# zju3dv/SMAP

Measured on AMD Instinct MI355X. Metric: frames/sec at 3x512x832 (SMAP backbone + depth-aware association + 3D lifting), higher is better.
Workload: dtype f16x3; 1 GPU; batch=8 x 3x512x832 per GPU, full SMAP + depth-aware PAF association + lifting (BASELINE configs[2]; configs[3] when n_gpus=8); records_in_run=4392, resident_batches_in_rotation=4, frames_per_launch=16, ranks_in_gather=1, full=False

## Files before the change

smap_amd/csrc/assoc.hip:

```cpp
#include <hip/hip_runtime.h>
#include <stdint.h>
#include <type_traits>
#include "smap_hip.h"
#include "hip_rc.h"
#include "prep_device.h"

namespace {

constexpr int NJ = SMAP_NJ, NL = SMAP_NL, MAXP = SMAP_MAXP, PSTRIDE = MAXP + 1;

__constant__ int c_pairs[2 * NL] = {0, 1, 0, 2, 0, 9, 9, 10, 10, 11, 0, 3, 3, 4,
                                    4, 5, 2, 12, 12, 13, 13, 14, 2, 6, 6, 7, 7, 8};
__constant__ float c_bone_length[NL] = {
    26.42178982f, 48.36980909f, 14.88291009f, 31.28002332f, 23.915707f,
    14.97674918f, 31.28002549f, 23.91570732f, 12.4644364f,  48.26604433f,
    39.03553194f, 12.4644364f,  48.19076948f, 39.03553252f};

__global__ void scale_hms_kernel(float* __restrict__ hms, int HW4, int total4)
{
    for (int i = blockIdx.x * blockDim.x + threadIdx.x; i < total4; i += gridDim.x * blockDim.x) {
        const int c = (i / HW4) % SMAP_HMS_C;
        const float d = c < NJ ? 255.f : 127.f;
        float4 v = reinterpret_cast<float4*>(hms)[i];
        v.x = v.x / d; v.y = v.y / d; v.z = v.z / d; v.w = v.w / d;
// ... 811 lines not shown
                       root_idx, dist_flag, bodys, counts);
    return hip_rc(hipGetLastError());
}

int smap_lift(const float* bodys, const int32_t* counts, const float* det_d, const float* root_d,
              const double* cams, int B, int H, int W, float* pred_2d, double* pred_3d, double* root_z,
              void* stream)
{
    if (!bodys || !counts || !det_d || !root_d || !cams || !pred_2d || !pred_3d || !root_z || B <= 0)
        return SMAP_E_ARG;
    hipLaunchKernelGGL(lift_kernel<false>, dim3(B), dim3(128), 0, (hipStream_t)stream, bodys, counts, det_d, root_d,
                       cams, H, W, pred_2d, pred_3d, root_z);
    return hip_rc(hipGetLastError());
}

int smap_lift_gt(const float* bodys, const int32_t* counts, const float* det_d, const float* root_d,
                 const double* cams, int B, int H, int W, double* pred_2d, double* pred_3d, double* root_z,
                 void* stream)
{
    if (!bodys || !counts || !det_d || !root_d || !cams || !pred_2d || !pred_3d || !root_z || B <= 0)
        return SMAP_E_ARG;
    hipLaunchKernelGGL(lift_kernel<true>, dim3(B), dim3(128), 0, (hipStream_t)stream, bodys, counts, det_d, root_d,
                       cams, H, W, pred_2d, pred_3d, root_z);
    return hip_rc(hipGetLastError());
}

int smap_lift_gt_bones(const float* bodys, const int32_t* counts, const float* det_d, const float* root_d,
                       const double* cams, int B, int H, int W, double* pred_2d, double* pred_3d, double* root_z,
                       double* depth_v, int32_t* bone_mask, void* stream)
{
    if (!bodys || !counts || !det_d || !root_d || !cams || !pred_2d || !pred_3d || !root_z || !depth_v || !bone_mask || B <= 0)
        return SMAP_E_ARG;
    hipLaunchKernelGGL((lift_kernel<true, true>), dim3(B), dim3(128), 0, (hipStream_t)stream, bodys, counts, det_d, root_d,
                       cams, H, W, pred_2d, pred_3d, root_z, depth_v, bone_mask);
    return hip_rc(hipGetLastError());
}

int smap_register_gt(const float* bodys, const int32_t* counts, const float* gt_roots, const int32_t* gt_counts,
                     int B, int G, float* matched, int32_t* matched_counts, void* stream)
{
    if (!bodys || !counts || !gt_roots || !gt_counts || !matched || !matched_counts || B <= 0 || G <= 0 ||
        G > REG_MAXG)
        return SMAP_E_ARG;
    hipLaunchKernelGGL(register_gt_kernel, dim3(B), dim3(64), 0, (hipStream_t)stream, bodys, counts, gt_roots,
                       gt_counts, G, matched, matched_counts);
    return hip_rc(hipGetLastError());
}

int smap_refine(const float* pred_2d, const double* pred_3d, const int32_t* counts, int B,
                const float* const* wt, const float* const* bs, double* refined, void* stream)
{
    if (!pred_2d || !pred_3d || !counts || !wt || !bs || !refined || B <= 0) return SMAP_E_ARG;
    RefineW w;
    for (int l = 0; l < 5; ++l) {
        if (!wt[l] || !bs[l]) return SMAP_E_ARG;
        w.wt[l] = wt[l];
        w.bs[l] = bs[l];
    }
    hipLaunchKernelGGL(refine_kernel<float>, dim3(MAXP, B), dim3(256), 0, (hipStream_t)stream, pred_2d, pred_3d,
                       counts, w, refined);
    return hip_rc(hipGetLastError());
}

int smap_refine_gt(const double* pred_2d, const double* pred_3d, const int32_t* counts, int B,
                   const float* const* wt, const float* const* bs, double* refined, void* stream)
{
    if (!pred_2d || !pred_3d || !counts || !wt || !bs || !refined || B <= 0) return SMAP_E_ARG;
    RefineW w;
    for (int l = 0; l < 5; ++l) {
        if (!wt[l] || !bs[l]) return SMAP_E_ARG;
        w.wt[l] = wt[l];
        w.bs[l] = bs[l];
    }
    hipLaunchKernelGGL(refine_kernel<double>, dim3(MAXP, B), dim3(256), 0, (hipStream_t)stream, pred_2d, pred_3d,
                       counts, w, refined);
    return hip_rc(hipGetLastError());
}

}

extern "C" int smap_refine_mlp(const float* x, int N, const float* const* wt, const float* const* bs, float* y,
                               void* stream)
{
    if (!wt || !bs || N < 0) return SMAP_E_ARG;
    if (N == 0) return 0;
    if (!x || !y) return SMAP_E_ARG;
    RefineW w;
    for (int l = 0; l < 5; ++l) {
        if (!wt[l] || !bs[l]) return SMAP_E_ARG;
        w.wt[l] = wt[l];
        w.bs[l] = bs[l];
    }
    hipLaunchKernelGGL(refine_mlp_kernel, dim3(N), dim3(256), 0, (hipStream_t)stream, x, w, y);
    return hip_rc(hipGetLastError());
}

extern "C" int smap_flip_merge(float* hms, const float* hms_flip, const int* pair43, int B, int H, int W, void* stream)
{
    if (!hms || !hms_flip || !pair43 || B <= 0 || H <= 0 || W <= 0) return SMAP_E_ARG;
    FlipTab tab;
    for (int c = 0; c < SMAP_HMS_C; ++c) {
        if (pair43[c] < 0 || pair43[c] >= SMAP_HMS_C) return SMAP_E_ARG;
        tab.pair[c] = pair43[c];
    }
    const long long total = (long long)B * SMAP_HMS_C * H * W;
    const int grid = (int)((total + 255) / 256 < 4096 ? (total + 255) / 256 : 4096);
    hipLaunchKernelGGL(flip_merge_kernel, dim3(grid), dim3(256), 0, (hipStream_t)stream, hms, hms_flip, tab, W, H * W,
                       total);
    return hip_rc(hipGetLastError());
}

extern "C" int smap_preprocess(const unsigned char* src, int h, int w, int nh, int nw, int top, int left, float* dst,
                               int net_h, int net_w, const float* mean3, const float* std3, double fx, double fy, void* stream)
{
    if (!src || !dst || !mean3 || !std3 || h <= 0 || w <= 0 || nh <= 0 || nw <= 0 || net_h <= 0 || net_w <= 0 || !(fx > 0) || !(fy > 0))
        return SMAP_E_ARG;
    const PrepFrame f{src, {h, w, nh, nw, top, left, 1.0 / fx, 1.0 / fy}};
    const PrepCanvas cv{net_h, net_w, {mean3[0], mean3[1], mean3[2]}, {std3[0], std3[1], std3[2]}};
    hipLaunchKernelGGL(preprocess_kernel, dim3((net_w + 255) / 256, net_h), dim3(256), 0, (hipStream_t)stream, f, dst, cv);
    return hip_rc(hipGetLastError());
}

extern "C" int smap_sizeof_prep_frame(void) { return (int)sizeof(smap_prep_frame); }

extern "C" int smap_preprocess_batch(const smap_prep_frame* frames, int B, float* dst, int net_h, int net_w, const float* mean3,
                                     const float* std3, void* stream)
{
    if (!frames || !dst || !mean3 || !std3 || B <= 0 || net_h <= 0 || net_w <= 0) return SMAP_E_ARG;
    for (int b = 0; b < B; ++b) {
        const smap_prep_frame& s = frames[b];
        if (!s.src || s.h <= 0 || s.w <= 0 || s.nh <= 0 || s.nw <= 0 || !(s.fx > 0) || !(s.fy > 0)) return SMAP_E_ARG;
    }
    const PrepCanvas cv{net_h, net_w, {mean3[0], mean3[1], mean3[2]}, {std3[0], std3[1], std3[2]}};
    const bool vec = net_w % 4 == 0 && ((uintptr_t)dst & 15) == 0;
    const int px = vec ? 4 : 1;
    const size_t frame_floats = (size_t)3 * net_h * net_w;
    for (int b0 = 0; b0 < B; b0 += SMAP_PREP_MAX_FRAMES) {
        const int n = B - b0 < SMAP_PREP_MAX_FRAMES ? B - b0 : SMAP_PREP_MAX_FRAMES;
        PrepTable t;
        for (int i = 0; i < SMAP_PREP_MAX_FRAMES; ++i) {
            const smap_prep_frame& s = frames[b0 + (i < n ? i : n - 1)];
            t.f[i] = PrepFrame{s.src, {s.h, s.w, s.nh, s.nw, s.top, s.left, 1.0 / s.fx, 1.0 / s.fy}};
        }
        const dim3 grid((net_w + 256 * px - 1) / (256 * px), net_h, n);
        float* out = dst + (size_t)b0 * frame_floats;
        if (vec) hipLaunchKernelGGL(preprocess_batch_kernel<4>, grid, dim3(256), 0, (hipStream_t)stream, t, out, cv);
        else hipLaunchKernelGGL(preprocess_batch_kernel<1>, grid, dim3(256), 0, (hipStream_t)stream, t, out, cv);
        const int rc = hip_rc(hipGetLastError());
        if (rc) return rc;
    }
    return 0;
}

extern "C" const char* smap_version(void) { return "smap_hip gfx950 r6 (assoc + backbone f16|x3 + flip-TTA + persistent conv + whole-Bottleneck launches + plan blob v2 + windowed arena + N segments + split K + lanes + two-input launches + tap-dot head + scaled head sum + two-launch peak search)"; }
```

smap_amd/csrc/conv.hip:

```cpp
#include <hip/hip_runtime.h>
#include <stdint.h>
#include "smap_hip.h"
#include "plan.h"
#include "conv_device.h"

namespace {

#ifndef SMAP_ABLATE
#define SMAP_ABLATE 0
#endif
template <int BM, int BN, int WM, int WN, int STAGES, int BK, bool FULL, bool X3, bool SPLITK = false, bool REGEPI = false, bool DUAL = false, bool TAPDOT = false,
          bool RELUSUM = false>
__global__ __launch_bounds__(WM * WN * 64) void conv_igemm_kernel(const ConvArgs a)
{
    static_assert(!TAPDOT || (!FULL && !SPLITK && !REGEPI && !DUAL), "tap-dot epilogue: plain instance only");
    static_assert(!RELUSUM || DUAL, "relu-sum: a second input");
    static_assert(!REGEPI || (X3 && !FULL && !SPLITK), "register epilogue: split precision, plain epilogue, no split K");
    static_assert(!DUAL || (!FULL && !SPLITK && !REGEPI), "second input: plain epilogue, no split K");
    constexpr int NPL = X3 ? 2 : 1;
    constexpr int NW = WM * WN, NT = NW * 64;
    static_assert(NW == 4 || NW == 8, "4 or 8 waves");
    static_assert(STAGES >= 2 && STAGES <= 4, "2..4 LDS stages");
    static_assert(BK == 32 || BK == 64, "BK = halves per K chunk");
    constexpr int ROWB = BK * 2;
    constexpr int SPR = ROWB / 16;
    constexpr int RPW = 64 / SPR;
    constexpr int RPR = NW * RPW;
    static_assert(BM % RPR == 0 && BN % RPR == 0, "tile must be a multiple of the DMA round");
    constexpr int LA = BM / RPR, LB = BN / RPR;
    constexpr int MI = BM / WM / 32, NI = BN / WN / 32;
    static_assert(MI >= 1 && NI >= 1, "tile too small for the wave grid");
    constexpr int STAGE = NPL * (BM + BN) * ROWB;
    constexpr int LPT = NPL * (LA + LB);
    static_assert((STAGES - 2) * LPT <= 63, "vmcnt is 6 bits");
    constexpr int CSS = TAPDOT ? BN + 8 : BN;
    constexpr int LDS_BYTES = REGEPI ? STAGES * STAGE : (STAGES * STAGE > BM * CSS * 4 ? STAGES * STAGE : BM * CSS * 4) + (SPLITK ? 16 : 0);
    static_assert(LDS_BYTES <= 160 * 1024, "LDS is 160 KiB per CU");
    __shared__ __attribute__((aligned(16))) char smem[LDS_BYTES];

    SMAP_TL_BEGIN
    const int tid = threadIdx.x, lane = tid & 63;
    const int wave = __builtin_amdgcn_readfirstlane(tid >> 6);
#ifdef SMAP_TRACE
    long long tr_t[8]; long long tr_wait = 0;
    tr_t[0] = __builtin_amdgcn_s_memtime();
#define TR(i) tr_t[i] = __builtin_amdgcn_s_memtime()
#else
#define TR(i)
#endif

    const int logical = xcd_logical_block();
    const int S = SPLITK ? a.ksplit : 1;
    const int tile_id = S > 1 ? logical / S : logical, ks = logical - tile_id * S;
    const int m_tile = tile_id / a.n_tiles, n_tile = tile_id - m_tile * a.n_tiles;
    const int m0 = m_tile * BM, n0 = n_tile * BN;
    const int seg = (n0 >= a.seg_n1 ? 1 : 0) + (n0 >= a.seg_n2 ? 1 : 0);
    const int nb = n0 - (seg == 0 ? 0 : seg == 1 ? a.seg_n1 : a.seg_n2);
    void* const o_out = seg == 0 ? a.out : seg == 1 ? a.seg_out1 : a.seg_out2;
    const int o_cout8 = seg == 0 ? a.Cout8 : seg == 1 ? a.seg_cout8_1 : a.seg_cout8_2;
    const int o_stride = seg == 0 ? a.out_stride_c : seg == 1 ? a.seg_stride1 : a.seg_stride2;
    const int o_c_off = seg == 0 ? a.out_c_off : 0;
    const int o_relu = seg == 0 ? a.relu : seg == 1 ? a.seg_relu1 : a.seg_relu2;
    const float o_scale = seg == 0 ? a.acc_scale : seg == 1 ? a.seg_scale1 : a.seg_scale2;
    const int o_lo = o_stride >> 1;
    const _Float16* const o_res = seg == 0 ? a.res : nullptr;
    const _Float16* const o_up = seg == 0 ? a.up : nullptr;
    const _Float16* const o_add1 = seg == 0 ? a.add1 : nullptr;
    const _Float16* const o_add2 = seg == 0 ? a.add2 : nullptr;

    const int lrow = lane / SPR, lslot = lane % SPR;
    const int srow = wave * RPW + lrow;
    const int gch = BK == 64 ? (lslot ^ ((srow >> 1) & 7)) : (lslot ^ ((srow >> 2) & 3));
    const char* __restrict__ arena = reinterpret_cast<const char*>(a.arena);
    const char* __restrict__ wt = reinterpret_cast<const char*>(a.w);
    const int HoWo = a.Ho * a.Wo;

    const bool wpair = BK == 32 && a.w_pairs;
    const int wrow = wpair ? 128 : ROWB;
    const int wblk = NPL * BN * wrow;
    unsigned w_off[NPL * LB];
#pragma unroll
    for (int j = 0; j < NPL * LB; ++j) w_off[j] = (unsigned)((j * RPR + wave * RPW + lrow) * wrow + lslot * 16);
    const char* __restrict__ wt_tile = wt + (long long)n_tile * (wpair ? a.K / 64 : a.K / BK) * wblk;
    auto issue_b = [&](int buf, int it) {
        char* sB = smem + buf * STAGE + NPL * BM * ROWB;
        const char* gB = wpair ? wt_tile + (long long)(it >> 1) * wblk + (it & 1) * 64 : wt_tile + (long long)it * wblk;
#pragma unroll
        for (int j = 0; j < NPL * LB; ++j)
            lds_dma16(gB + w_off[j], sB + (j * RPR + wave * RPW) * ROWB);
    };
    if (!(SMAP_ABLATE & 1) && !SPLITK) issue_b(0, 0);

    unsigned a_off[LA];
    unsigned a_mask[LA];
    {
        int m = m0 + srow;
        int b = m / HoWo, rem = m - b * HoWo;
        int oy = rem / a.Wo, ox = rem - oy * a.Wo;
#pragma unroll
        for (int i = 0; i < LA; ++i) {
            a_off[i] = 0;
            a_mask[i] = 0;
            if (m < a.M) {
                const int iy0 = oy * a.stride - a.pad, ix0 = ox * a.stride - a.pad;
                const long long e = ((long long)(b * a.H + iy0) * a.W + ix0) * a.in_stride_c + a.in_c_off + gch * 8;
                a_off[i] = (unsigned)(a.in_off + e * 2);
                unsigned vx = 0, mk = 0;
#pragma unroll
                for (int kw = 0; kw < 3; ++kw)
                    if (kw < a.ksize && (unsigned)(ix0 + kw) < (unsigned)a.W) vx |= 1u << kw;
#pragma unroll
                for (int kh = 0; kh < 3; ++kh)
                    if (kh < a.ksize && (unsigned)(iy0 + kh) < (unsigned)a.H) mk |= vx << (kh * a.ksize);
                a_mask[i] = mk;
            }
            m += RPR;
            ox += RPR;
            while (ox >= a.Wo) { ox -= a.Wo; ++oy; }
            while (oy >= a.Ho) { oy -= a.Ho; ++b; }
        }
    }
    unsigned a_off2[DUAL ? LA : 1];
    if (DUAL) {
        int m = m0 + srow;
        int b = m / HoWo, rem = m - b * HoWo;
        int oy = rem / a.Wo, ox = rem - oy * a.Wo;
#pragma unroll
        for (int i = 0; i < LA; ++i) {
            a_off2[i] = 0;
            if (m < a.M) {
                const long long e = ((long long)(b * a.H2 + oy * a.stride2) * a.W2 + ox * a.stride2) * a.in2_stride_c + gch * 8;
                a_off2[i] = (unsigned)(a.in2_off + e * 2);
            }
            m += RPR;
            ox += RPR;
            while (ox >= a.Wo) { ox -= a.Wo; ++oy; }
            while (oy >= a.Ho) { oy -= a.Ho; ++b; }
        }
    }
    const int cchunks = a.Cin / BK;
    const int cchunks2 = DUAL ? a.Cin2 / BK : 0;
    const int n_all = a.ksize * a.ksize * cchunks + cchunks2;
    const int it_lo = S > 1 ? ks * n_all / S : 0;
    const int n_iter = (S > 1 ? (ks + 1) * n_all / S : n_all) - it_lo;

    int s_kh = 0, s_kw = 0, s_cc = 0;
    int s_in2 = 0;
    int s_it = it_lo;
    if (S > 1) {
        const int tap = it_lo / cchunks;
        s_cc = it_lo - tap * cchunks;
        s_kh = tap / a.ksize;
        s_kw = tap - s_kh * a.ksize;
    }
    unsigned a_cur[LA];
    auto set_tap = [&]() {
        const unsigned tap_off = (unsigned)((s_kh * a.W + s_kw) * a.in_stride_c * 2);
        const unsigned bit = 1u << (s_kh * a.ksize + s_kw);
#pragma unroll
        for (int i = 0; i < LA; ++i) a_cur[i] = (a_mask[i] & bit) ? a_off[i] + tap_off : 0u;
    };
    set_tap();
    auto issue_a = [&](int buf) {
#pragma unroll
        for (int pl = 0; pl < NPL; ++pl) {
            char* sA = smem + buf * STAGE + pl * BM * ROWB;
            const char* gA = arena + (unsigned)(s_cc * ROWB + (X3 ? pl * ((DUAL && s_in2) ? a.in2_lo : a.in_lo) * 2 : 0));
#pragma unroll
            for (int i = 0; i < LA; ++i)
                lds_dma16(gA + a_cur[i], sA + (i * RPR + wave * RPW) * ROWB);
        }
    };
    auto advance = [&]() {
        ++s_it;
        if (DUAL && s_in2) { ++s_cc; return; }
        if (++s_cc == cchunks) {
            s_cc = 0;
            if (DUAL) {
                s_in2 = 1;
#pragma unroll
                for (int i = 0; i < LA; ++i) a_cur[i] = a_off2[i];
                return;
            }
            if (++s_kw == a.ksize) { s_kw = 0; ++s_kh; }
            set_tap();
        }
    };
    auto stage = [&](int buf) {
        issue_a(buf);
        issue_b(buf, s_it);
        advance();
    };
    if (!(SMAP_ABLATE & 1)) {
        if (SPLITK) issue_b(0, it_lo);
        issue_a(0);
        advance();
    }

    constexpr int CG = BN / 8;
    constexpr int PASSES = REGEPI ? 1 : BM * CG / NT;
    static_assert(BM * CG % NT == 0, "tile/thread mismatch");
    half8 rres[PASSES][NPL];
    auto load_res = [&]() {
#pragma unroll
        for (int p = 0; p < PASSES; ++p) {
            const int idx = p * NT + tid;
            const int row = idx / CG, cg = idx - row * CG;
            const int m = m0 + row, n = nb + cg * 8;
            const unsigned dense = (m < a.M && n < o_cout8) ? (unsigned)m * (unsigned)(NPL * o_cout8) + (unsigned)n : 0u;
#pragma unroll
            for (int pl = 0; pl < NPL; ++pl)
                rres[p][pl] = *reinterpret_cast<const half8*>(o_res + dense + pl * o_cout8);
        }
    };
    if (o_res && !SPLITK && !REGEPI) load_res();

    f32x16 acc[MI][NI];
#pragma unroll
    for (int mi = 0; mi < MI; ++mi)
#pragma unroll
        for (int ni = 0; ni < NI; ++ni)
#pragma unroll
            for (int r = 0; r < 16; ++r) acc[mi][ni][r] = 0.f;

    const int wm = wave / WN, wn = wave - wm * WN;
    const int l31 = lane & 31, lhi = lane >> 5;
    if (REGEPI) {
        const float inv = 1.f / o_scale;
#pragma unroll
        for (int ni = 0; ni < NI; ++ni)
#pragma unroll
            for (int q = 0; q < 4; ++q) {
                const float4 b4 = *reinterpret_cast<const float4*>(a.bias + n0 + wn * (BN / WN) + ni * 32 + 8 * q + 4 * lhi);
#pragma unroll
                for (int mi = 0; mi < MI; ++mi) {
                    acc[mi][ni][4 * q + 0] = b4.x * inv; acc[mi][ni][4 * q + 1] = b4.y * inv;
                    acc[mi][ni][4 * q + 2] = b4.z * inv; acc[mi][ni][4 * q + 3] = b4.w * inv;
                }
            }
    }
    const int rswz = BK == 64 ? ((l31 >> 1) & 7) : ((l31 >> 2) & 3);
    const int a_row0 = wm * (BM / WM) + l31;
    const int b_row0 = wn * (BN / WN) + l31;
    f32x16 park[RELUSUM ? MI : 1][RELUSUM ? NI : 1];
    float bias1[RELUSUM ? NI : 1];
    if (RELUSUM) {
#pragma unroll
        for (int ni = 0; ni < NI; ++ni) bias1[ni] = a.bias[n0 + wn * (BN / WN) + ni * 32 + l31];
    }

    TR(1);
#pragma unroll
    for (int st = 1; st < STAGES - 1; ++st)
        if (st < n_iter && !(SMAP_ABLATE & 1)) stage(st);
    int buf = 0, nbuf = STAGES - 1;
    for (int it = 0; it < n_iter; ++it) {
#ifdef SMAP_TRACE
        const long long tw0 = __builtin_amdgcn_s_memtime();
#endif
        if (it + STAGES - 1 <= n_iter) asm volatile("s_waitcnt vmcnt(%0)" ::"n"((STAGES - 2) * LPT) : "memory");
        else asm volatile("s_waitcnt vmcnt(0)" ::: "memory");
        __builtin_amdgcn_s_barrier();
        asm volatile("" ::: "memory");
#ifdef SMAP_TRACE
        tr_wait += __builtin_amdgcn_s_memtime() - tw0;
        if (it == 0) tr_t[2] = __builtin_amdgcn_s_memtime();
#endif
        if (it + STAGES - 1 < n_iter && !(SMAP_ABLATE & 1)) stage(nbuf);
        if (RELUSUM && it == cchunks) {
#pragma unroll
            for (int mi = 0; mi < MI; ++mi)
#pragma unroll
                for (int ni = 0; ni < NI; ++ni)
#pragma unroll
                    for (int r = 0; r < 16; ++r) {
                        const float v = X3 ? acc[mi][ni][r] * o_scale + bias1[ni] : acc[mi][ni][r] + bias1[ni];
                        park[mi][ni][r] = v < 0.f ? 0.f : v;
                        acc[mi][ni][r] = 0.f;
                    }
        }
        const char* sA = smem + buf * STAGE;
        const char* sB = sA + NPL * BM * ROWB;
#pragma unroll
        for (int kk = 0; kk < ((SMAP_ABLATE & 2) ? 0 : BK / 16); ++kk) {
            const int slot = ((kk * 2 + lhi) ^ rswz) * 16;
            half8 af[NPL][MI], bf[NPL][NI];
#pragma unroll
            for (int pl = 0; pl < NPL; ++pl) {
#pragma unroll
                for (int mi = 0; mi < MI; ++mi)
                    af[pl][mi] = *reinterpret_cast<const half8*>(sA + (pl * BM + a_row0 + mi * 32) * ROWB + slot);
#pragma unroll
                for (int ni = 0; ni < NI; ++ni)
                    bf[pl][ni] = *reinterpret_cast<const half8*>(sB + (pl * BN + b_row0 + ni * 32) * ROWB + slot);
            }
#pragma unroll
            for (int mi = 0; mi < MI; ++mi)
#pragma unroll
                for (int ni = 0; ni < NI; ++ni) {
                    if (REGEPI) {
                        acc[mi][ni] = __builtin_amdgcn_mfma_f32_32x32x16_f16(bf[0][ni], af[NPL - 1][mi], acc[mi][ni], 0, 0, 0);
                        acc[mi][ni] = __builtin_amdgcn_mfma_f32_32x32x16_f16(bf[NPL - 1][ni], af[0][mi], acc[mi][ni], 0, 0, 0);
                        acc[mi][ni] = __builtin_amdgcn_mfma_f32_32x32x16_f16(bf[0][ni], af[0][mi], acc[mi][ni], 0, 0, 0);
                        continue;
                    }
                    if (X3) {
                        acc[mi][ni] = __builtin_amdgcn_mfma_f32_32x32x16_f16(af[NPL - 1][mi], bf[0][ni], acc[mi][ni], 0, 0, 0);
                        acc[mi][ni] = __builtin_amdgcn_mfma_f32_32x32x16_f16(af[0][mi], bf[NPL - 1][ni], acc[mi][ni], 0, 0, 0);
                    }
                    acc[mi][ni] = __builtin_amdgcn_mfma_f32_32x32x16_f16(af[0][mi], bf[0][ni], acc[mi][ni], 0, 0, 0);
                }
        }
        buf = buf + 1 == STAGES ? 0 : buf + 1;
        nbuf = nbuf + 1 == STAGES ? 0 : nbuf + 1;
    }
    TR(3);
    __syncthreads();
    if (SMAP_ABLATE & 8) {
        if (acc[0][0][0] == 12345.678f) reinterpret_cast<float*>(a.out)[tid] = acc[0][0][1];
        return;
    }

    if constexpr (REGEPI) {
        _Float16* const outp = reinterpret_cast<_Float16*>(o_out);
        unsigned m_dense[MI], m_out[MI];
        bool m_ok[MI];
#pragma unroll
        for (int mi = 0; mi < MI; ++mi) {
            const int m = m0 + wm * (BM / WM) + mi * 32 + l31;
            m_ok[mi] = m < a.M;
            const unsigned ms = m_ok[mi] ? (unsigned)m : 0u;
            m_dense[mi] = ms * (unsigned)(NPL * o_cout8);
            m_out[mi] = ms * (unsigned)o_stride + (unsigned)o_c_off;
        }
        auto n_of = [&](int ni) { return nb + wn * (BN / WN) + ni * 32 + 8 * lhi; };
        auto load_rr = [&](int mi, int ni, half8 (&rr)[2][NPL]) {
#pragma unroll
            for (int j = 0; j < 2; ++j) {
                const int n = n_of(ni) + 16 * j;
                const unsigned d = n < o_cout8 ? m_dense[mi] + (unsigned)n : 0u;
#pragma unroll
                for (int pl = 0; pl < NPL; ++pl) rr[j][pl] = *reinterpret_cast<const half8*>(o_res + d + pl * o_cout8);
            }
        };
        half8 rr[2][2][NPL];
        if (o_res) load_rr(0, 0, rr[0]);
#pragma unroll
        for (int mi = 0; mi < MI; ++mi)
#pragma unroll
            for (int ni = 0; ni < NI; ++ni) {
                constexpr int NB = MI * NI;
                const int blk = mi * NI + ni;
                if (o_res && blk + 1 < NB) load_rr((blk + 1) / NI, (blk + 1) % NI, rr[(blk + 1) & 1]);
                f32x16& c = acc[mi][ni];
#pragma unroll
                for (int j = 0; j < 2; ++j)
#pragma unroll
                    for (int e = 0; e < 4; ++e) {
                        const float2 sw = halfwave_swap(c[8 * j + e], c[8 * j + 4 + e]);
                        c[8 * j + e] = o_scale * sw.x;
                        c[8 * j + 4 + e] = o_scale * sw.y;
                    }
                if (o_res) {
#pragma unroll
                    for (int j = 0; j < 2; ++j)
#pragma unroll
                        for (int e = 0; e < 8; ++e) c[8 * j + e] += (float)rr[blk & 1][j][0][e] + (float)rr[blk & 1][j][NPL - 1][e];
                }
                if (o_relu) relu16(c);
#pragma unroll
                for (int j = 0; j < 2; ++j) {
                    const int n = n_of(ni) + 16 * j;
                    if (!m_ok[mi] || n >= o_cout8 || ((SMAP_ABLATE & 4) && a.M != 7)) continue;
                    _Float16* op = outp + (m_out[mi] + (unsigned)n);
                    half8 h, l;
#pragma unroll
                    for (int e = 0; e < 8; ++e) {
                        h[e] = (_Float16)c[8 * j + e];
                        l[e] = (_Float16)(c[8 * j + e] - (float)h[e]);
                    }
                    *reinterpret_cast<half8*>(op) = h;
                    *reinterpret_cast<half8*>(op + o_lo) = l;
                }
            }
        SMAP_TL_END(a)
        return;
    }

    float* Cs = reinterpret_cast<float*>(smem);
#pragma unroll
    for (int ni = 0; ni < NI; ++ni) {
        const int col = wn * (BN / WN) + ni * 32 + l31;
        const float bias = RELUSUM ? a.bias_b[n0 + col] : a.bias[n0 + col];
#pragma unroll
        for (int mi = 0; mi < MI; ++mi)
#pragma unroll
            for (int r = 0; r < 16; ++r) {
                const int row = wm * (BM / WM) + mi * 32 + (r & 3) + 8 * (r >> 2) + 4 * lhi;
                if (RELUSUM) {
                    const float v = X3 ? acc[mi][ni][r] * a.acc_scale_b + bias : acc[mi][ni][r] + bias;
                    Cs[row * CSS + col] = (v < 0.f ? 0.f : v) + park[mi][ni][r];
                    continue;
                }
                Cs[row * CSS + col] = S > 1 ? acc[mi][ni][r] : (X3 ? acc[mi][ni][r] * o_scale + bias : acc[mi][ni][r] + bias);
            }
    }
    __syncthreads();
    if (SPLITK && S == 1 && o_res) load_res();
    if (SPLITK && S > 1) {
#ifndef SMAP_SPLITK_ACQREL
#define SMAP_SPLITK_ACQREL 1
#endif
#if !SMAP_SPLITK_ACQREL && !defined(__gfx942__) && !defined(__gfx950__) && defined(__HIP_DEVICE_COMPILE__)
#error "split K: the fence-free partial-tile hand-off is verified for gfx942 / gfx950 only; build with -DSMAP_SPLITK_ACQREL=1 elsewhere"
#endif
        float* part = a.kpart + (size_t)tile_id * S * (BM * BN);
        for (int i = tid; i < BM * BN; i += NT) __hip_atomic_store(part + (size_t)ks * (BM * BN) + i, Cs[i], __ATOMIC_RELAXED, __HIP_MEMORY_SCOPE_AGENT);
        asm volatile("s_waitcnt vmcnt(0)" ::: "memory");
        __syncthreads();
        volatile int* s_last = reinterpret_cast<volatile int*>(smem + LDS_BYTES - 16);
        if (tid == 0) {
#if SMAP_SPLITK_ACQREL
            const unsigned t = __hip_atomic_fetch_add(a.kcount + tile_id, 1u, __ATOMIC_RELEASE, __HIP_MEMORY_SCOPE_AGENT);
            if (t == (unsigned)(S - 1)) __builtin_amdgcn_fence(__ATOMIC_ACQUIRE, "agent");
#else
            const unsigned t = atomicAdd(a.kcount + tile_id, 1u);
#endif
            *s_last = t == (unsigned)(S - 1);
            if (t == (unsigned)(S - 1)) atomicExch(a.kcount + tile_id, 0u);
        }
        __syncthreads();
        if (!*s_last) return;
        if (o_res) load_res();
        for (int i = tid; i < BM * BN; i += NT) {
            float v = __hip_atomic_load(part + i, __ATOMIC_RELAXED, __HIP_MEMORY_SCOPE_AGENT);
            for (int q = 1; q < S; ++q) v += __hip_atomic_load(part + (size_t)q * (BM * BN) + i, __ATOMIC_RELAXED, __HIP_MEMORY_SCOPE_AGENT);
            const float bias = a.bias[n0 + i % BN];
            Cs[i] = X3 ? v * o_scale + bias : v + bias;
        }
        __syncthreads();
    }

    if constexpr (TAPDOT) {
        static_assert(BM == 128 && BN == 256 && NW == 8, "one 16-row MFMA tile per wave");
                const int prow = wave * 16 + (lane & 15), kq = lane >> 4;
        const half8* __restrict__ wfrag = reinterpret_cast<const half8*>(a.tap_w) + lane;
        f32x4 d = {0.f, 0.f, 0.f, 0.f};
#pragma unroll
        for (int ks = 0; ks < BN / 32; ++ks) {
            const half8 wh = wfrag[(ks * 2 + 0) * 64], wl = wfrag[(ks * 2 + 1) * 64];
            const float4 y0 = *reinterpret_cast<const float4*>(Cs + prow * CSS + ks * 32 + kq * 8);
            const float4 y1 = *reinterpret_cast<const float4*>(Cs + prow * CSS + ks * 32 + kq * 8 + 4);
            float y[8] = {y0.x, y0.y, y0.z, y0.w, y1.x, y1.y, y1.z, y1.w};
            half8 yh, yl;
#pragma unroll
            for (int e = 0; e < 8; ++e) {
                float v = y[e];
                if (o_relu) v = v < 0.f ? 0.f : v;
                yh[e] = (_Float16)v;
                yl[e] = (_Float16)(v - (float)yh[e]);
            }
            d = __builtin_amdgcn_mfma_f32_16x16x32_f16(yl, wh, d, 0, 0, 0);
            d = __builtin_amdgcn_mfma_f32_16x16x32_f16(yh, wl, d, 0, 0, 0);
            d = __builtin_amdgcn_mfma_f32_16x16x32_f16(yh, wh, d, 0, 0, 0);
        }
        float* const tout = reinterpret_cast<float*>(o_out);
#pragma unroll
        for (int i = 0; i < 4; ++i) {
            const int m = m0 + wave * 16 + kq * 4 + i;
            if (m < a.M) tout[(size_t)m * 16 + (lane & 15)] = d[i] * a.tap_scale;
        }
        SMAP_TL_END(a)
        return;
    }

    struct Extra { half8 t00[NPL], t01[NPL], t10[NPL], t11[NPL], a1[NPL], a2[NPL]; float ly0, ly1, lx0, lx1; bool ok; unsigned o; int row, cg; };
    constexpr int TS = NPL;
    auto val = [](const half8 (&h)[NPL], int e) -> float {
        return X3 ? (float)h[0][e] + (float)h[NPL - 1][e] : (float)h[0][e];
    };
    auto load_pass = [&](int p) -> Extra {
        Extra x;
        const int idx = p * NT + tid;
        x.row = idx / CG;
        x.cg = idx - x.row * CG;
        const int m = m0 + x.row, n = nb + x.cg * 8;
        x.ok = m < a.M && n < o_cout8 && !((SMAP_ABLATE & 4) && a.M != 7);
        const int ms = x.ok ? m : 0, ns = x.ok ? n : 0;
        const unsigned dense = (unsigned)ms * (unsigned)(TS * o_cout8) + (unsigned)ns;
        x.o = (unsigned)ms * (unsigned)o_stride + (unsigned)(o_c_off + ns);
        if (FULL && o_up) {
            const int b = (SMAP_ABLATE & 64) ? 0 : ms / HoWo, rem = ms - b * HoWo;
            const int oy = (SMAP_ABLATE & 64) ? (ms & 63) : rem / a.Wo, ox = (SMAP_ABLATE & 64) ? (ms & 127) : rem - oy * a.Wo;
            Lerp ly = lerp_index(oy, a.up_h, a.Ho), lx = lerp_index(ox, a.up_w, a.Wo);
            if (SMAP_ABLATE & 64) { ly.i0 = oy >> 1; ly.i1 = ly.i0; ly.l0 = 0.5f; ly.l1 = 0.5f; lx.i0 = ox >> 1; lx.i1 = lx.i0; lx.l0 = 0.5f; lx.l1 = 0.5f; }
            const int us = TS * o_cout8;
            const unsigned tb0 = (unsigned)b * (unsigned)(a.up_h * a.up_w) * (unsigned)us + (unsigned)ns;
            const _Float16* __restrict__ tb = o_up;
#pragma unroll
            for (int pl = 0; pl < ((SMAP_ABLATE & 32) ? 0 : NPL); ++pl) {
                x.t00[pl] = *reinterpret_cast<const half8*>(tb + (tb0 + (unsigned)(ly.i0 * a.up_w + lx.i0) * (unsigned)us + (unsigned)(pl * o_cout8)));
                x.t01[pl] = *reinterpret_cast<const half8*>(tb + (tb0 + (unsigned)(ly.i0 * a.up_w + lx.i1) * (unsigned)us + (unsigned)(pl * o_cout8)));
                x.t10[pl] = *reinterpret_cast<const half8*>(tb + (tb0 + (unsigned)(ly.i1 * a.up_w + lx.i0) * (unsigned)us + (unsigned)(pl * o_cout8)));
                x.t11[pl] = *reinterpret_cast<const half8*>(tb + (tb0 + (unsigned)(ly.i1 * a.up_w + lx.i1) * (unsigned)us + (unsigned)(pl * o_cout8)));
            }
            x.ly0 = ly.l0; x.ly1 = ly.l1; x.lx0 = lx.l0; x.lx1 = lx.l1;
        }
#pragma unroll
        for (int pl = 0; pl < NPL; ++pl) {
            if (FULL && o_add1) x.a1[pl] = *reinterpret_cast<const half8*>(o_add1 + dense + pl * o_cout8);
            if (FULL && o_add2) x.a2[pl] = *reinterpret_cast<const half8*>(o_add2 + dense + pl * o_cout8);
        }
        return x;
    };
    auto finish_pass = [&](int p, const Extra& x) {
        float v[8];
        {
            const float4 lo = *reinterpret_cast<const float4*>(Cs + x.row * BN + x.cg * 8);
            const float4 hi = *reinterpret_cast<const float4*>(Cs + x.row * BN + x.cg * 8 + 4);
            v[0] = lo.x; v[1] = lo.y; v[2] = lo.z; v[3] = lo.w;
            v[4] = hi.x; v[5] = hi.y; v[6] = hi.z; v[7] = hi.w;
        }
        if (o_res) {
#pragma unroll
            for (int e = 0; e < 8; ++e) v[e] += val(rres[p], e);
        }
        if (FULL && o_up) {
#pragma unroll
            for (int e = 0; e < 8; ++e)
                v[e] += x.ly0 * (x.lx0 * val(x.t00, e) + x.lx1 * val(x.t01, e)) +
                        x.ly1 * (x.lx0 * val(x.t10, e) + x.lx1 * val(x.t11, e));
        }
        if (o_relu) {
#pragma unroll
            for (int e = 0; e < 8; ++e) v[e] = v[e] < 0.f ? 0.f : v[e];
        }
        if (FULL && o_add1) {
#pragma unroll
            for (int e = 0; e < 8; ++e) v[e] += val(x.a1, e);
        }
        if (FULL && o_add2) {
#pragma unroll
            for (int e = 0; e < 8; ++e) v[e] += val(x.a2, e);
        }
        if (!x.ok) return;
        if (a.out_fp32) {
            float* op = reinterpret_cast<float*>(o_out) + x.o;
            *reinterpret_cast<float4*>(op) = make_float4(v[0], v[1], v[2], v[3]);
            *reinterpret_cast<float4*>(op + 4) = make_float4(v[4], v[5], v[6], v[7]);
        } else {
            half8 h;
#pragma unroll
            for (int e = 0; e < 8; ++e) h[e] = (_Float16)v[e];
            *reinterpret_cast<half8*>(reinterpret_cast<_Float16*>(o_out) + x.o) = h;
            if (X3) {
                half8 l;
#pragma unroll
                for (int e = 0; e < 8; ++e) l[e] = (_Float16)(v[e] - (float)h[e]);
                *reinterpret_cast<half8*>(reinterpret_cast<_Float16*>(o_out) + x.o + o_lo) = l;
            }
        }
    };
    TR(4);
#ifndef SMAP_EPI_DEPTH
#define SMAP_EPI_DEPTH 1
#endif
    constexpr int ED = (FULL && PASSES > 2) ? SMAP_EPI_DEPTH : 1;
    Extra ex[ED + 1];
#pragma unroll
    for (int p = 0; p < ED && p < PASSES; ++p) ex[p] = load_pass(p);
#pragma unroll
    for (int p = 0; p < PASSES; ++p) {
        if (p + ED < PASSES) ex[(p + ED) % (ED + 1)] = load_pass(p + ED);
        finish_pass(p, ex[p % (ED + 1)]);
    }
#ifdef SMAP_TRACE
    asm volatile("s_waitcnt vmcnt(0)" ::: "memory");
    TR(5);
    if (a.dbg && tid == 0) {
        long long* d = a.dbg + (long long)blockIdx.x * 8;
        unsigned hwid;
        asm volatile("s_getreg_b32 %0, hwreg(HW_REG_HW_ID)" : "=s"(hwid));
        d[0] = tr_t[0]; d[1] = tr_t[1]; d[2] = tr_t[2]; d[3] = tr_t[3]; d[4] = tr_t[4]; d[5] = tr_t[5]; d[6] = tr_wait; d[7] = hwid;
    }
#endif
    SMAP_TL_END(a)
}

#define SMAP_IGEMM_ROW(cap)                                                                                      \
    constexpr TileRow t = tile_row(TILE);                                                                        \
    static_assert(t.family == TF_IGEMM && tile_has(t, X3, cap),                                                  \
                  "csrc/tiles.h: the row of this tile id does not list this instance");                          \
    constexpr int BM = t.bm, BN = t.bn, BK = tile_bk(t, X3)

template <int TILE, bool X3, int WM, int WN, int STAGES>
hipError_t launch_splitk(const ConvArgs& a, hipStream_t st)
{
    SMAP_IGEMM_ROW(TC_SPLITK);
    const dim3 grid(a.m_tiles * a.n_tiles * a.ksplit);
    if (a.up || a.add1 || a.add2)
        hipLaunchKernelGGL((conv_igemm_kernel<BM, BN, WM, WN, STAGES, BK, true, X3, true>), grid, dim3(WM * WN * 64), 0, st, a);
    else
        hipLaunchKernelGGL((conv_igemm_kernel<BM, BN, WM, WN, STAGES, BK, false, X3, true>), grid, dim3(WM * WN * 64), 0, st, a);
    return hipGetLastError();
}

template <int TILE, bool X3, int WM, int WN, int STAGES>
hipError_t launch(const ConvArgs& a, hipStream_t st)
{
    SMAP_IGEMM_ROW(0);
    static_assert(!(t.caps & TC_REGEPI), "register-epilogue tiles go through launch_regepi");
    if (a.up || a.add1 || a.add2)
        hipLaunchKernelGGL((conv_igemm_kernel<BM, BN, WM, WN, STAGES, BK, true, X3>), dim3(a.m_tiles * a.n_tiles), dim3(WM * WN * 64), 0, st, a);
    else
        hipLaunchKernelGGL((conv_igemm_kernel<BM, BN, WM, WN, STAGES, BK, false, X3>), dim3(a.m_tiles * a.n_tiles), dim3(WM * WN * 64), 0, st, a);
    return hipGetLastError();
}

template <int TILE, bool X3, int WM, int WN, int STAGES>
hipError_t launch_regepi(const ConvArgs& a, hipStream_t st)
{
    SMAP_IGEMM_ROW(TC_REGEPI);
    if (a.up || a.add1 || a.add2 || a.out_fp32 || a.ksplit > 1) return hipErrorInvalidValue;
    hipLaunchKernelGGL((conv_igemm_kernel<BM, BN, WM, WN, STAGES, BK, false, X3, false, true>), dim3(a.m_tiles * a.n_tiles), dim3(WM * WN * 64), 0, st, a);
    return hipGetLastError();
}

template <int TILE, bool X3, int WM, int WN, int STAGES>
hipError_t launch_dual(const ConvArgs& a, hipStream_t st)
{
    SMAP_IGEMM_ROW(TC_DUAL);
    if (a.up || a.add1 || a.add2 || a.ksplit > 1 || a.ksize != 1) return hipErrorInvalidValue;
    hipLaunchKernelGGL((conv_igemm_kernel<BM, BN, WM, WN, STAGES, BK, false, X3, false, false, true>), dim3(a.m_tiles * a.n_tiles), dim3(WM * WN * 64), 0, st, a);
    return hipGetLastError();
}

template <int TILE, bool X3, int WM, int WN, int STAGES>
hipError_t launch_relusum(const ConvArgs& a, hipStream_t st)
{
    SMAP_IGEMM_ROW(TC_DUAL | TC_RELUSUM);
    if (a.up || a.add1 || a.add2 || a.res || a.ksplit > 1 || a.ksize != 1 || a.relu || !a.bias_b) return hipErrorInvalidValue;
    hipLaunchKernelGGL((conv_igemm_kernel<BM, BN, WM, WN, STAGES, BK, false, X3, false, false, true, false, true>), dim3(a.m_tiles * a.n_tiles), dim3(WM * WN * 64), 0, st, a);
    return hipGetLastError();
}

template <int TILE, bool X3, int WM, int WN, int STAGES>
hipError_t launch_tapdot(const ConvArgs& a, hipStream_t st)
{
    SMAP_IGEMM_ROW(TC_TAPDOT);
    if (a.up || a.add1 || a.add2 || a.res || a.ksplit > 1 || a.Cin2 > 0 || a.n_tiles != 1 || a.tap_n != 9 || !a.tap_w) return hipErrorInvalidValue;
    hipLaunchKernelGGL((conv_igemm_kernel<BM, BN, WM, WN, STAGES, BK, false, X3, false, false, false, true>), dim3(a.m_tiles), dim3(WM * WN * 64), 0, st, a);
    return hipGetLastError();
}
#undef SMAP_IGEMM_ROW

#define SMAP_BOTH(HELPER, TILE, ...) (a.x3 ? HELPER<TILE, true, __VA_ARGS__>(a, st) : HELPER<TILE, false, __VA_ARGS__>(a, st))

}

hipError_t smap_launch_conv(const ConvArgs& a, int tile, hipStream_t st)
{
    const TileRow* t = tile_find(tile);
    if (!t || !tile_has(*t, a.x3)) return hipErrorInvalidValue;
    switch (t->family) {
        case TF_HALO: return smap_launch_conv3(a, tile, st);
        case TF_PERSIST: return smap_launch_convp(a, tile, st);
        case TF_TAIL: return smap_launch_convf(a, tile, st);
        case TF_BLOCK: return smap_launch_convb(a, tile, st);
        case TF_IGEMM: break;
    }
    if (a.tap_n > 0) {
        switch (tile) {
            case 54: return SMAP_BOTH(launch_tapdot, 54, 2, 4, 2);
            default: return hipErrorInvalidValue;
        }
    }
    if (a.Cin2 > 0 && a.bias_b) {
        switch (tile) {
            case 50: return SMAP_BOTH(launch_relusum, 50, 2, 4, 2);
            case 51: return SMAP_BOTH(launch_relusum, 51, 4, 2, 2);
            case 53: return SMAP_BOTH(launch_relusum, 53, 4, 2, 2);
            case 54: return SMAP_BOTH(launch_relusum, 54, 2, 4, 2);
            default: return hipErrorInvalidValue;
        }
    }
    if (a.Cin2 > 0) {
        switch (tile) {
            case 20: return SMAP_BOTH(launch_dual, 20, 2, 2, 2);
            case 50: return SMAP_BOTH(launch_dual, 50, 2, 4, 2);
            case 51: return SMAP_BOTH(launch_dual, 51, 4, 2, 2);
            case 53: return SMAP_BOTH(launch_dual, 53, 4, 2, 2);
            case 54: return SMAP_BOTH(launch_dual, 54, 2, 4, 2);
            default: return hipErrorInvalidValue;
        }
    }
    if (a.ksplit > 1) {
        switch (tile) {
            case 2: return SMAP_BOTH(launch_splitk, 2, 2, 2, 2);
            case 22: return SMAP_BOTH(launch_splitk, 22, 2, 2, 2);
            case 7: return SMAP_BOTH(launch_splitk, 7, 2, 2, 4);
            case 20: return SMAP_BOTH(launch_splitk, 20, 2, 2, 2);
            default: return hipErrorInvalidValue;
        }
    }
    if (a.x3) {
        switch (tile) {
            case 0: return launch<0, true, 2, 2, 2>(a, st);
            case 1: return launch<1, true, 2, 2, 2>(a, st);
            case 2: return launch<2, true, 2, 2, 2>(a, st);
            case 4: return launch<4, true, 2, 2, 2>(a, st);
            case 3: return launch<3, true, 4, 1, 2>(a, st);
            case 20: return launch<20, true, 2, 2, 2>(a, st);
            case 21: return launch<21, true, 2, 2, 2>(a, st);
            case 22: return launch<22, true, 2, 2, 2>(a, st);
            case 23: return launch<23, true, 2, 2, 2>(a, st);
            case 24: return launch<24, true, 2, 2, 3>(a, st);
            case 25: return launch<25, true, 2, 2, 3>(a, st);
            case 26: return launch<26, true, 2, 2, 4>(a, st);
            case 7: return launch<7, true, 2, 2, 4>(a, st);
            case 27: return launch<27, true, 2, 2, 3>(a, st);
            case 50: return launch<50, true, 2, 4, 2>(a, st);
            case 51: return launch<51, true, 4, 2, 2>(a, st);
            case 52: return launch<52, true, 2, 4, 2>(a, st);
            case 53: return launch<53, true, 4, 2, 2>(a, st);
            case 54: return launch<54, true, 2, 4, 2>(a, st);
            case 55: return launch<55, true, 2, 4, 4>(a, st);
            case 56: return launch_regepi<56, true, 2, 4, 2>(a, st);
            default: return hipErrorInvalidValue;
        }
    }
    switch (tile) {
        case 20: return launch<20, false, 2, 2, 2>(a, st);
        case 21: return launch<21, false, 2, 2, 2>(a, st);
        case 22: return launch<22, false, 2, 2, 2>(a, st);
        case 23: return launch<23, false, 2, 2, 2>(a, st);
        case 24: return launch<24, false, 2, 2, 4>(a, st);
        case 25: return launch<25, false, 2, 2, 3>(a, st);
        case 26: return launch<26, false, 2, 2, 4>(a, st);
        case 27: return launch<27, false, 2, 2, 3>(a, st);
        case 0: return launch<0, false, 2, 2, 2>(a, st);
        case 1: return launch<1, false, 2, 2, 2>(a, st);
        case 2: return launch<2, false, 2, 2, 2>(a, st);
        case 3: return launch<3, false, 4, 1, 2>(a, st);
        case 4: return launch<4, false, 2, 2, 2>(a, st);
        case 5: return launch<5, false, 2, 2, 4>(a, st);
        case 6: return launch<6, false, 2, 2, 3>(a, st);
        case 7: return launch<7, false, 2, 2, 4>(a, st);
        case 8: return launch<8, false, 4, 1, 3>(a, st);
        case 9: return launch<9, false, 2, 2, 3>(a, st);
        case 50: return launch<50, false, 2, 4, 2>(a, st);
        case 51: return launch<51, false, 4, 2, 2>(a, st);
        case 52: return launch<52, false, 2, 4, 2>(a, st);
        case 53: return launch<53, false, 4, 2, 2>(a, st);
        case 54: return launch<54, false, 2, 4, 2>(a, st);
        case 55: return launch<55, false, 2, 4, 4>(a, st);
        default: return hipErrorInvalidValue;
    }
}
```

smap_amd/csrc/plan.h:

```cpp
#pragma once
#include <hip/hip_runtime.h>
#include <stdint.h>
#include "tiles.h"

struct ConvArgs {
    const void* arena;
    long long in_off;
    const _Float16* w;
    const float* bias;
    void* out;
    const _Float16* res;
    const _Float16* add1;
    const _Float16* add2;
    const _Float16* up;
    int up_h, up_w;
    int H, W, Cin, in_stride_c, in_c_off;
    int Ho, Wo, Cout8;
    int ksize, stride, pad, relu;
    int out_stride_c, out_c_off, out_fp32;
    int M, K, m_tiles, n_tiles;
    int x3;
    int in_lo;
    int out_lo;
    long long w_lo;
    float acc_scale;
    int w_pairs;
    const _Float16* w2;
    const float* bias2;
    int tail_cout8;
    int tail_chunks;
    float tail_acc_scale;
    const _Float16* w0;
    const float* bias0;
    int head_cin;
    float acc_scale0;
    const _Float16* wd;
    float acc_scale_d;
    int ksplit;
    float* kpart;
    unsigned* kcount;
    long long in2_off;
    int H2, W2, Cin2, in2_stride_c, stride2, in2_lo;
    const float* bias_b;
    float acc_scale_b;
    const _Float16* tap_w;
    int tap_n;
    float tap_scale;
    int seg_n1, seg_n2;
    void* seg_out1; void* seg_out2;
    int seg_cout8_1, seg_cout8_2, seg_stride1, seg_stride2, seg_relu1, seg_relu2;
    float seg_scale1, seg_scale2;
#ifdef SMAP_TRACE
    long long* dbg;
#endif
#ifdef SMAP_TIMELINE
    long long* tl;
    long long tl_meta[4];
#endif
};

struct Lerp { int i0, i1; float l0, l1; };
__device__ __forceinline__ Lerp lerp_index(int dst, int in_size, int out_size)
{
    Lerp r;
    if (in_size == out_size) { r.i0 = dst; r.i1 = dst; r.l0 = 1.f; r.l1 = 0.f; return r; }
    const float scale = out_size > 1 ? (float)(in_size - 1) / (float)(out_size - 1) : 0.f;
    const float src = scale * (float)dst;
    r.i0 = (int)src;
    r.i1 = r.i0 + (r.i0 < in_size - 1 ? 1 : 0);
    float l1 = src - (float)r.i0;
    l1 = l1 < 0.f ? 0.f : (l1 > 1.f ? 1.f : l1);
    r.l1 = l1;
    r.l0 = 1.f - l1;
    return r;
}

hipError_t smap_launch_conv(const ConvArgs& a, int tile, hipStream_t st);
hipError_t smap_launch_conv3(const ConvArgs& a, int tile, hipStream_t st);
hipError_t smap_launch_convp(const ConvArgs& a, int tile, hipStream_t st);
hipError_t smap_launch_convf(const ConvArgs& a, int tile, hipStream_t st);
hipError_t smap_launch_convb(const ConvArgs& a, int tile, hipStream_t st);
hipError_t smap_launch_convc(const ConvArgs& a, hipStream_t st);

#ifdef SMAP_TIMELINE
#define SMAP_TL_BEGIN const long long tl_t0 = __builtin_amdgcn_s_memrealtime();
#define SMAP_TL_END(a)                                                                                        \
    if ((a).tl && threadIdx.x == 0) {                                                                         \
        unsigned hw_, xcc_;                                                                                   \
        asm volatile("s_getreg_b32 %0, hwreg(HW_REG_HW_ID)" : "=s"(hw_));                                     \
        asm volatile("s_getreg_b32 %0, hwreg(HW_REG_XCC_ID)" : "=s"(xcc_));                                   \
        long long* d_ = (a).tl + 4 * (1 + (long long)blockIdx.x);                                             \
        d_[0] = tl_t0; d_[1] = __builtin_amdgcn_s_memrealtime(); d_[2] = hw_; d_[3] = xcc_;                   \
        if (blockIdx.x == 0) { (a).tl[0] = (a).tl_meta[0]; (a).tl[1] = (a).tl_meta[1]; (a).tl[2] = (a).tl_meta[2]; (a).tl[3] = (a).tl_meta[3]; } \
    }
#else
#define SMAP_TL_BEGIN
#define SMAP_TL_END(a)
#endif
```

smap_amd/csrc/plan.hip:

```cpp
#include <hip/hip_runtime.h>
#include <stdint.h>
#include <new>
#include <memory>
#include <cstdlib>
#include <cstring>
#include <climits>
#include <vector>
#include <type_traits>
#include "smap_hip.h"
#include "plan.h"
#include "plan_check.h"
#include "conv_device.h"
#include "hip_rc.h"

namespace {

#ifndef SMAP_STEM_STORE16
#define SMAP_STEM_STORE16 1
#endif
constexpr int ST_T = 16, ST_PH = ST_T * 2 + 5, ST_PW = 40;
constexpr int ST_K = SMAP_STEM_K;

struct StemIn {
    const float* p[SMAP_MAX_INPUTS];
// ... 428 lines not shown
    }
    __syncthreads();
    for (int idx = tid; idx < C * HS_PX; idx += 256) {
        const int c = idx / HS_PX, px = idx - c * HS_PX;
        const int x = x0 + px;
        if (x >= Wo) continue;
        float v = tile[c * (HS_PX + 1) + px];
        if (FLIP) {
            const float f = tile2[pair[c] * (HS_PX + 1) + px];
            const bool neg = c >= n_kpt && ((c - n_kpt) & 1) == 0;
            v = v + (neg ? f * -1.f : f);
            if (c >= n_kpt) v = v * 0.5f;
        }
        if (scale) v = v / (c < n_kpt ? 255.f : 127.f);
        out[(((size_t)b * C + c) * Ho + y) * Wo + x] = v;
        if (status && !(fabsf(v) <= 3.4028234e38f)) {
            atomicOr(reinterpret_cast<unsigned*>(status) + b / 31, 1u | (2u << (b % 31)));
            if (b >= 31) atomicOr(reinterpret_cast<unsigned*>(status), 1u);
        }
    }
}

__global__ __launch_bounds__(256) void tapsum_kernel(const float* __restrict__ t, const float* __restrict__ bias, float* __restrict__ out,
                                                     int B, int H, int W, int ts, int* __restrict__ status)
{
    const long long total = (long long)B * H * W;
    const long long i = (long long)blockIdx.x * 256 + threadIdx.x;
    if (i >= total) return;
    const int x = (int)(i % W), y = (int)((i / W) % H), b = (int)(i / ((long long)W * H));
    float v = bias[0];
#pragma unroll
    for (int kh = 0; kh < 3; ++kh)
#pragma unroll
        for (int kw = 0; kw < 3; ++kw) {
            const int yy = y + kh - 1, xx = x + kw - 1;
            if ((unsigned)yy < (unsigned)H && (unsigned)xx < (unsigned)W) v += t[(((size_t)b * H + yy) * W + xx) * ts + kh * 3 + kw];
        }
    out[i] = v;
    if (status && !(fabsf(v) <= 3.4028234e38f)) {
        atomicOr(reinterpret_cast<unsigned*>(status) + b / 31, 1u | (2u << (b % 31)));
        if (b >= 31) atomicOr(reinterpret_cast<unsigned*>(status), 1u);
    }
}

inline int grid_for(long long total, int block)
{
    long long g = (total + block - 1) / block;
    return (int)(g < 1 ? 1 : (g > 8192 ? 8192 : g));
}

}

struct smap_plan : PlanCheck {
    bool lanes_on = false, lanes_ready = false;
    hipStream_t side[SMAP_MAX_LANES] = {};
    std::vector<hipEvent_t> ev;
    hipEvent_t join_ev[SMAP_MAX_LANES] = {};
};

#ifdef SMAP_TIMELINE
constexpr long long TL_SLICE = 4LL * (1 + 16384);
static int tl_next = 0;
static long long* tl_base() { const char* e = getenv("SMAP_TIMELINE_PTR"); return e ? reinterpret_cast<long long*>(strtoull(e, nullptr, 0)) : nullptr; }
static int tl_cap() { const char* e = getenv("SMAP_TIMELINE_CAP"); return e ? atoi(e) : 0; }
extern "C" __attribute__((visibility("default"))) void smap_timeline_reset(void) { tl_next = 0; }
extern "C" __attribute__((visibility("default"))) int smap_timeline_count(void) { return tl_next; }
#endif

extern "C" {

int smap_plan_create(const smap_op* ops, int n_ops, smap_plan** plan)
{
    std::unique_ptr<smap_plan> p(new (std::nothrow) smap_plan());
    if (!plan || !p) return SMAP_E_ARG;
    if (int rc = plan_check(ops, n_ops, p.get())) return rc;
    *plan = p.release();
    return 0;
}

int smap_plan_create_from_blob(const void* blob, size_t blob_bytes, smap_plan** plan, smap_blob_info* info)
{
    std::unique_ptr<smap_plan> p(new (std::nothrow) smap_plan());
    if (!plan || !p) return SMAP_E_ARG;
    if (int rc = plan_check_blob(blob, blob_bytes, p.get(), info)) return rc;
    *plan = p.release();
    return 0;
}

static void lanes_release(smap_plan* p)
{
    for (hipEvent_t& e : p->ev) if (e) { (void)hipEventDestroy(e); e = nullptr; }
    for (int l = 0; l < SMAP_MAX_LANES; ++l) {
        if (p->join_ev[l]) { (void)hipEventDestroy(p->join_ev[l]); p->join_ev[l] = nullptr; }
        if (p->side[l]) { (void)hipStreamDestroy(p->side[l]); p->side[l] = nullptr; }
    }
    p->lanes_ready = false;
}

void smap_plan_destroy(smap_plan* plan)
{
    if (!plan) return;
    lanes_release(plan);
    delete plan;
}

static int lanes_setup(smap_plan* p)
{
    if (p->lanes_ready) return 0;
    hipError_t e = hipSuccess;
    for (int l = 1; l < p->n_lanes && e == hipSuccess; ++l) e = hipStreamCreateWithFlags(&p->side[l], hipStreamNonBlocking);
    for (int l = 0; l < p->n_lanes && e == hipSuccess; ++l) e = hipEventCreateWithFlags(&p->join_ev[l], hipEventDisableTiming);
    p->ev.assign(p->ops.size(), nullptr);
    for (size_t i = 0; i < p->ops.size() && e == hipSuccess; ++i)
        if (p->signalled[i]) e = hipEventCreateWithFlags(&p->ev[i], hipEventDisableTiming);
    if (e != hipSuccess) { lanes_release(p); return hip_rc(e); }
    p->lanes_ready = true;
    return 0;
}

int smap_plan_set_lanes(smap_plan* plan, int on)
{
    if (!plan) return SMAP_E_ARG;
    if (on && plan->n_lanes > 1)
        if (int rc = lanes_setup(plan)) return rc;
    plan->lanes_on = on != 0;
    return 0;
}

static ConvArgs conv_args(const smap_op& o, char* ar, const char* wb)
{
    auto A = [&](int64_t off) -> _Float16* { return off < 0 ? nullptr : reinterpret_cast<_Float16*>(ar + off); };
    const TileRow& t = *tile_find(o.tile);
    ConvArgs a;
    a.arena = ar + window_of(o.in_off);
    a.in_off = o.in_off - window_of(o.in_off);
    a.w = reinterpret_cast<const _Float16*>(wb + o.w_off);
    a.bias = reinterpret_cast<const float*>(wb + o.bias_off);
    a.out = ar + o.out_off;
    a.res = A(o.res_off);
    a.add1 = A(o.add1_off);
    a.add2 = A(o.add2_off);
    a.up = A(o.aux_off[0]);
    a.up_h = o.aux_h[0];
    a.up_w = o.aux_w[0];
    a.H = o.H; a.W = o.W; a.Cin = o.Cin; a.in_stride_c = o.in_stride_c; a.in_c_off = o.in_c_off;
    a.Ho = o.Ho; a.Wo = o.Wo; a.Cout8 = (o.Cout + 7) & ~7;
    a.ksize = o.ksize; a.stride = o.stride; a.pad = o.pad; a.relu = o.relu;
    a.out_stride_c = o.out_stride_c; a.out_c_off = o.out_c_off; a.out_fp32 = o.out_fp32;
    a.M = o.B * o.Ho * o.Wo;
    a.K = o.ksize * o.ksize * o.Cin + (o.in2_C > 0 ? o.in2_C : 0);
    a.Cin2 = o.in2_C > 0 ? o.in2_C : 0;
    a.in2_off = o.in2_C > 0 ? o.in2_off - window_of(o.in_off) : 0;
    a.H2 = o.in2_H; a.W2 = o.in2_W; a.in2_stride_c = o.in2_stride_c; a.stride2 = o.in2_stride; a.in2_lo = o.in2_stride_c / 2;
    a.bias_b = (o.in2_C > 0 && o.in2_mode == 1) ? reinterpret_cast<const float*>(wb + o.in2_bias_off) : nullptr;
    a.acc_scale_b = o.in2_acc_scale;
    a.x3 = o.precision;
    a.in_lo = o.in_stride_c / 2;
    a.out_lo = o.out_stride_c / 2;
    a.w_lo = (long long)o.cout_pad * a.K * 2;
    a.acc_scale = o.acc_scale;
    a.w_pairs = o.w_pairs;
    a.w2 = o.tail_cout > 0 ? reinterpret_cast<const _Float16*>(wb + o.tail_w_off) : nullptr;
    a.bias2 = o.tail_cout > 0 ? reinterpret_cast<const float*>(wb + o.tail_bias_off) : nullptr;
    a.tail_cout8 = o.tail_cout;
    a.tail_chunks = o.tail_cout > 0 ? o.tail_cout_pad / t.tail_bn : 0;
    a.tail_acc_scale = o.tail_acc_scale;
    a.w0 = o.head_cin > 0 ? reinterpret_cast<const _Float16*>(wb + o.head_w_off) : nullptr;
    a.bias0 = o.head_cin > 0 ? reinterpret_cast<const float*>(wb + o.head_bias_off) : nullptr;
    a.head_cin = o.head_cin;
    a.acc_scale0 = o.head_acc_scale;
    a.wd = o.head_cin > 0 && o.short_acc_scale > 0.f ? reinterpret_cast<const _Float16*>(wb + o.short_w_off) : nullptr;
    a.acc_scale_d = o.short_acc_scale;
    a.tap_n = o.tap_n;
    a.tap_w = o.tap_n > 0 ? reinterpret_cast<const _Float16*>(wb + o.tap_w_off) : nullptr;
    a.tap_scale = o.tap_scale;
    a.ksplit = o.ksplit > 1 ? o.ksplit : 1;
    a.kpart = o.ksplit > 1 ? reinterpret_cast<float*>(ar + o.kpart_off) : nullptr;
    a.kcount = o.ksplit > 1 ? reinterpret_cast<unsigned*>(ar + o.kcount_off) : nullptr;
    a.seg_n1 = o.seg_n[0] > 0 ? o.seg_n[0] : INT32_MAX;
    a.seg_n2 = o.seg_n[1] > 0 ? o.seg_n[1] : INT32_MAX;
    a.seg_out1 = o.seg_n[0] > 0 ? ar + o.seg_out_off[0] : nullptr;
    a.seg_out2 = o.seg_n[1] > 0 ? ar + o.seg_out_off[1] : nullptr;
    a.seg_cout8_1 = o.seg_cout[0]; a.seg_cout8_2 = o.seg_cout[1];
    a.seg_stride1 = o.seg_out_stride_c[0]; a.seg_stride2 = o.seg_out_stride_c[1];
    a.seg_relu1 = o.seg_relu[0]; a.seg_relu2 = o.seg_relu[1];
    a.seg_scale1 = o.seg_acc_scale[0]; a.seg_scale2 = o.seg_acc_scale[1];
    a.m_tiles = (a.M + t.bm - 1) / t.bm;
    a.n_tiles = o.cout_pad / t.bn;
    return a;
}

static int run_ops(const smap_plan* plan, int first, int count, const float* const* inputs, int n_inputs, void* arena,
                   const void* weights, float* out, void* stream)
{
    if (!plan || !arena || !weights || first < 0 || count < 0 || first + count > (int)plan->ops.size())
        return SMAP_E_ARG;
    if (n_inputs < 0 || n_inputs > SMAP_MAX_INPUTS || (n_inputs > 0 && !inputs)) return SMAP_E_ARG;
    hipStream_t st = (hipStream_t)stream;
    char* ar = static_cast<char*>(arena);
    const char* wb = static_cast<const char*>(weights);
    auto A = [&](int64_t off) -> _Float16* { return off < 0 ? nullptr : reinterpret_cast<_Float16*>(ar + off); };
    StemIn sin;
    for (int j = 0; j < SMAP_MAX_INPUTS; ++j) sin.p[j] = j < n_inputs ? inputs[j] : nullptr;
    sin.frames_per = 1;
    const bool have_input = n_inputs > 0 && inputs[0];
    for (int64_t w : plan->windows)
        if (hipError_t e = hipMemsetAsync(ar + w, 0, SMAP_ZERO_PAGE, st); e != hipSuccess) return hip_rc(e);
    for (size_t t = 0; t < plan->tickets.size();) {
        if (plan->tickets[t].op < first || plan->tickets[t].op >= first + count) { ++t; continue; }
        int64_t lo = plan->tickets[t].off, hi = lo + plan->tickets[t].bytes;
        size_t u = t + 1;
        while (u < plan->tickets.size() && plan->tickets[u].off == hi && plan->tickets[u].op < first + count) hi += plan->tickets[u++].bytes;
        if (hipError_t e = hipMemsetAsync(ar + lo, 0, (size_t)(hi - lo), st); e != hipSuccess) return hip_rc(e);
        t = u;
    }
    for (int i = first; i < first + count; ++i)
        if ((plan->ops[i].kind == SMAP_OP_HEADSUM || plan->ops[i].kind == SMAP_OP_TAPSUM) && plan->ops[i].status_off > 0 && out) {
            if (hipError_t e = hipMemsetAsync(reinterpret_cast<char*>(out) + plan->ops[i].status_off, 0, 4 * (size_t)SMAP_STATUS_WORDS(plan->ops[i].B), st); e != hipSuccess) return hip_rc(e);
            break;
        }
    const bool lanes = plan->lanes_on && plan->lanes_ready && plan->n_lanes > 1 && first == 0 && count == (int)plan->ops.size();
    hipStream_t const st0 = st;
    auto join = [&]() -> int {
        for (int l = 1; l < plan->n_lanes; ++l) {
            if (hipError_t e = hipEventRecord(plan->join_ev[l], plan->side[l]); e != hipSuccess) return hip_rc(e);
            if (hipError_t e = hipStreamWaitEvent(st0, plan->join_ev[l], 0); e != hipSuccess) return hip_rc(e);
        }
        return 0;
    };
    auto fail = [&](int rc) -> int { if (lanes) (void)join(); return rc; };
    if (lanes) {
        if (hipError_t e = hipEventRecord(plan->join_ev[0], st0); e != hipSuccess) return hip_rc(e);
        for (int l = 1; l < plan->n_lanes; ++l)
            if (hipError_t e = hipStreamWaitEvent(plan->side[l], plan->join_ev[0], 0); e != hipSuccess) return hip_rc(e);
    }
    for (int i = first; i < first + count; ++i) {
        const smap_op& o = plan->ops[i];
        hipError_t e = hipSuccess;
        if (lanes) {
            st = o.lane > 0 ? plan->side[o.lane] : st0;
            for (int k = 0; k < o.n_wait; ++k)
                if (hipError_t e2 = hipStreamWaitEvent(st, plan->ev[o.wait_op[k]], 0); e2 != hipSuccess) return fail(hip_rc(e2));
        }
        switch (o.kind) {
            case SMAP_OP_CONV: {
                ConvArgs a = conv_args(o, ar, wb);
#ifdef SMAP_TIMELINE
                a.tl = nullptr;
                if (tl_base() && tl_next < tl_cap()) {
                    a.tl = tl_base() + (long long)tl_next++ * TL_SLICE;
                    a.tl_meta[0] = i; a.tl_meta[1] = 0; a.tl_meta[2] = (long long)(uintptr_t)stream; a.tl_meta[3] = o.tile;
                }
#endif
#ifdef SMAP_TRACE
                a.dbg = getenv("SMAP_TRACE_PTR") ? reinterpret_cast<long long*>(strtoull(getenv("SMAP_TRACE_PTR"), nullptr, 0)) : nullptr;
#endif
                e = smap_launch_conv(a, o.tile, st);
                break;
            }
            case SMAP_OP_STEM: {
                const int frames = o.flip_from > 0 ? o.flip_from : o.B;
                if (!have_input || frames % n_inputs) return fail(SMAP_E_ARG);
                for (int j = 0; j < n_inputs; ++j) if (!inputs[j]) return fail(SMAP_E_ARG);
                sin.frames_per = frames / n_inputs;
                dim3 grid((o.Wo + ST_T - 1) / ST_T, (o.Ho + ST_T - 1) / ST_T, o.B);
                if (o.precision)
                    hipLaunchKernelGGL(stem_kernel<true>, grid, dim3(256), 0, st, sin,
                                       reinterpret_cast<const _Float16*>(wb + o.w_off),
                                       reinterpret_cast<const float*>(wb + o.bias_off), A(o.out_off), o.H, o.W, o.Ho,
                                       o.Wo, o.acc_scale, o.flip_from);
                else
                    hipLaunchKernelGGL(stem_kernel<false>, grid, dim3(256), 0, st, sin,
                                       reinterpret_cast<const _Float16*>(wb + o.w_off),
                                       reinterpret_cast<const float*>(wb + o.bias_off), A(o.out_off), o.H, o.W, o.Ho,
                                       o.Wo, 1.f, o.flip_from);
                e = hipGetLastError();
                break;
            }
            case SMAP_OP_STEMPOOL: {
                const int frames = o.flip_from > 0 ? o.flip_from : o.B;
                if (!have_input || frames % n_inputs) return fail(SMAP_E_ARG);
                for (int j = 0; j < n_inputs; ++j) if (!inputs[j]) return fail(SMAP_E_ARG);
                sin.frames_per = frames / n_inputs;
                const int hs = (o.H + 6 - 7) / 2 + 1, ws = (o.W + 6 - 7) / 2 + 1;
                dim3 grid((o.Wo + SP_PX - 1) / SP_PX, (o.Ho + SP_PY - 1) / SP_PY, o.B);
                if (o.precision)
                    hipLaunchKernelGGL(stem_pool_kernel<true>, grid, dim3(256), 0, st, sin,
                                       reinterpret_cast<const _Float16*>(wb + o.w_off),
                                       reinterpret_cast<const float*>(wb + o.bias_off), A(o.out_off), o.H, o.W, hs, ws,
                                       o.Ho, o.Wo, o.acc_scale, o.flip_from);
                else
                    hipLaunchKernelGGL(stem_pool_kernel<false>, grid, dim3(256), 0, st, sin,
                                       reinterpret_cast<const _Float16*>(wb + o.w_off),
                                       reinterpret_cast<const float*>(wb + o.bias_off), A(o.out_off), o.H, o.W, hs, ws,
                                       o.Ho, o.Wo, 1.f, o.flip_from);
                e = hipGetLastError();
                break;
            }
            case SMAP_OP_MAXPOOL: {
                const long long total = (long long)o.B * o.Ho * o.Wo * (o.Cin / 8);
                if (o.precision)
                    hipLaunchKernelGGL(maxpool_kernel<true>, dim3(grid_for(total, 256)), dim3(256), 0, st, A(o.in_off),
                                       A(o.out_off), o.B, o.H, o.W, o.Cin, o.Ho, o.Wo);
                else
                    hipLaunchKernelGGL(maxpool_kernel<false>, dim3(grid_for(total, 256)), dim3(256), 0, st, A(o.in_off),
                                       A(o.out_off), o.B, o.H, o.W, o.Cin, o.Ho, o.Wo);
                e = hipGetLastError();
                break;
            }
            case SMAP_OP_UPADD: {
                const long long total = (long long)o.B * o.Ho * o.Wo * (o.Cout / 8);
                hipLaunchKernelGGL(upadd_kernel, dim3(grid_for(total, 256)), dim3(256), 0, st, A(o.in_off),
                                   A(o.aux_off[0]), A(o.out_off), o.B, o.Ho, o.Wo, o.Cout, o.aux_h[0], o.aux_w[0],
                                   o.relu);
                e = hipGetLastError();
                break;
            }
            case SMAP_OP_TAPSUM: {
                if (!out) return fail(SMAP_E_ARG);
                const long long total = (long long)o.B * o.H * o.W;
                int* status = o.status_off > 0 ? reinterpret_cast<int*>(reinterpret_cast<char*>(out) + o.status_off) : nullptr;
                hipLaunchKernelGGL(tapsum_kernel, dim3((unsigned)((total + 255) / 256)), dim3(256), 0, st, reinterpret_cast<const float*>(ar + o.aux_off[0]),
                                   reinterpret_cast<const float*>(wb + o.bias_off), reinterpret_cast<float*>(reinterpret_cast<char*>(out) + o.ext_off),
                                   o.B, o.H, o.W, o.Cin, status);
                e = hipGetLastError();
                break;
            }
            case SMAP_OP_HEADSUM: {
                if (!out) return fail(SMAP_E_ARG);
                HeadSrc s;
                s.n = o.n_aux;
                for (int k = 0; k < 3; ++k) {
                    s.p[k] = k < o.n_aux ? reinterpret_cast<const float*>(ar + o.aux_off[k]) : nullptr;
                    s.h[k] = o.aux_h[k];
                    s.w[k] = o.aux_w[k];
                }
                dim3 grid((o.Wo + HS_PX - 1) / HS_PX, o.Ho, o.B);
                float* dst = reinterpret_cast<float*>(reinterpret_cast<char*>(out) + o.ext_off);
                int* status = o.status_off > 0 ? reinterpret_cast<int*>(reinterpret_cast<char*>(out) + o.status_off) : nullptr;
                if (o.flip_from > 0)
                    hipLaunchKernelGGL(headsum_kernel<true>, grid, dim3(256), 0, st, s, dst, o.Ho, o.Wo, o.Cout, o.Cin,
                                       o.flip_from, reinterpret_cast<const int*>(wb + o.w_off), o.in_c_off, status, o.scale_hms);
                else
                    hipLaunchKernelGGL(headsum_kernel<false>, grid, dim3(256), 0, st, s, dst, o.Ho, o.Wo, o.Cout, o.Cin,
                                       0, nullptr, o.in_c_off, status, o.scale_hms);
                e = hipGetLastError();
                break;
            }
            default:
                return fail(SMAP_E_ARG);
        }
        if (e != hipSuccess) return fail(hip_rc(e));
        if (lanes && plan->signalled[i])
            if (hipError_t e2 = hipEventRecord(plan->ev[i], st); e2 != hipSuccess) return fail(hip_rc(e2));
    }
    if (lanes) return join();
    return 0;
}

int smap_workspace_bytes(const smap_plan* plan, int64_t* arena_bytes, int64_t* out_bytes)
{
    if (!plan) return SMAP_E_ARG;
    plan_workspace_bytes(plan->ops, arena_bytes, out_bytes);
    return 0;
}

int smap_plan_run_range(const smap_plan* plan, int first, int count, const float* input, void* arena,
                        const void* weights, float* out, void* stream)
{
    return run_ops(plan, first, count, &input, input ? 1 : 0, arena, weights, out, stream);
}

int smap_plan_run(const smap_plan* plan, const float* input, void* arena, const void* weights, float* out,
                  void* stream)
{
    if (!plan) return SMAP_E_ARG;
    return run_ops(plan, 0, (int)plan->ops.size(), &input, input ? 1 : 0, arena, weights, out, stream);
}

int smap_plan_run_inputs(const smap_plan* plan, const float* const* inputs, int n_inputs, void* arena, const void* weights,
                         float* out, void* stream)
{
    if (!plan || n_inputs < 1) return SMAP_E_ARG;
    return run_ops(plan, 0, (int)plan->ops.size(), inputs, n_inputs, arena, weights, out, stream);
}

}
```

smap_amd/csrc/plan_check.cpp:

```cpp
#include <algorithm>
#include <climits>
#include <cstring>
#include <initializer_list>
#include "plan_check.h"
#include "tiles.h"

namespace {

bool product(int64_t* r, std::initializer_list<int64_t> factors)
{
    int64_t n = 1;
    for (int64_t x : factors)
        if (x < 0 || __builtin_mul_overflow(n, x, &n)) return false;
    *r = n;
    return true;
}
bool within(int64_t limit, std::initializer_list<int64_t> factors)
{
    int64_t n;
    return product(&n, factors) && n <= limit;
}
inline int64_t cout8(const smap_op& o) { return (o.Cout + 7LL) & ~7LL; }

enum SpanBuf { ARENA, OUTPUT, WEIGHTS };
enum SpanRole { READ, WRITTEN, PARTIALS, TICKETS };
struct Span { SpanBuf buf; SpanRole role; int64_t off, bytes; };

template <class F>
bool for_each_span(const smap_op& o, F&& f)
{
    bool ok = true;
    auto span = [&](SpanBuf buf, SpanRole role, int64_t off, std::initializer_list<int64_t> factors) {
        int64_t bytes;
        if (product(&bytes, factors)) f(Span{buf, role, off, bytes});
        else ok = false;
    };
    const int64_t pl = o.precision == 1 ? 2 : 1;
    int64_t M;
    if (!product(&M, {o.B, o.Ho, o.Wo})) return false;
    auto status = [&] { if (o.status_off > 0) span(OUTPUT, WRITTEN, o.status_off, {SMAP_STATUS_WORDS((int64_t)o.B), 4}); };
    switch (o.kind) {
        case SMAP_OP_CONV: {
            const TileRow* t = tile_find(o.tile);
            int64_t K;
            if (!t || !product(&K, {o.ksize, o.ksize, o.Cin}) || __builtin_add_overflow(K, o.in2_C > 0 ? o.in2_C : 0, &K)) return false;
            const int64_t c8 = o.tail_cout > 0 ? o.tail_cout : cout8(o);
            span(ARENA, READ, o.in_off, {o.B, o.H, o.W, o.in_stride_c, 2});
            if (o.in2_C > 0) span(ARENA, READ, o.in2_off, {o.B, o.in2_H, o.in2_W, o.in2_stride_c, 2});
            span(ARENA, WRITTEN, o.out_off, {M, o.out_stride_c, o.out_fp32 ? 4 : 2});
            for (int64_t off : {o.res_off, o.add1_off, o.add2_off})
                if (off >= 0) span(ARENA, READ, off, {M, c8, 2, pl});
            if (o.aux_off[0] >= 0) span(ARENA, READ, o.aux_off[0], {o.B, o.aux_h[0], o.aux_w[0], c8, 2, pl});
            for (int j = 0; j < 2; ++j)
                if (o.seg_n[j] > 0) span(ARENA, WRITTEN, o.seg_out_off[j], {M, o.seg_out_stride_c[j], 2});
            if (o.ksplit > 1) {
                const int64_t m_tiles = M / t->bm + (M % t->bm != 0), n_tiles = o.cout_pad / t->bn;
                span(ARENA, PARTIALS, o.kpart_off, {m_tiles, n_tiles, o.ksplit, t->bm, t->bn, 4});
                span(ARENA, TICKETS, o.kcount_off, {m_tiles, n_tiles, 4});
            }
            span(WEIGHTS, READ, o.w_off, {o.cout_pad, K, 2, pl});
            span(WEIGHTS, READ, o.bias_off, {o.cout_pad, 4});
            if (o.tail_cout > 0) {
                span(WEIGHTS, READ, o.tail_w_off, {o.tail_cout_pad, o.Cout, 2, pl});
                span(WEIGHTS, READ, o.tail_bias_off, {o.tail_cout_pad, 4});
            }
            if (o.head_cin > 0) {
                span(WEIGHTS, READ, o.head_w_off, {o.head_cin, o.Cin, 2, pl});
                span(WEIGHTS, READ, o.head_bias_off, {o.Cin, 4});
                if (o.short_acc_scale > 0.f) span(WEIGHTS, READ, o.short_w_off, {o.tail_cout, o.head_cin, 2, pl});
            }
            if (o.in2_C > 0 && o.in2_mode == 1) span(WEIGHTS, READ, o.in2_bias_off, {o.cout_pad, 4});
            if (o.tap_n > 0) span(WEIGHTS, READ, o.tap_w_off, {o.cout_pad / 32, 2 * 64 * 8 * 2});
            break;
        }
        case SMAP_OP_STEM: case SMAP_OP_STEMPOOL:
            span(ARENA, WRITTEN, o.out_off, {M, 64, 2, pl});
            span(WEIGHTS, READ, o.w_off, {64, SMAP_STEM_K, 2, pl});
            span(WEIGHTS, READ, o.bias_off, {64, 4});
            break;
        case SMAP_OP_MAXPOOL:
            span(ARENA, READ, o.in_off, {o.B, o.H, o.W, o.Cin, 2, pl});
            span(ARENA, WRITTEN, o.out_off, {M, o.Cout, 2, pl});
            break;
        case SMAP_OP_UPADD:
            span(ARENA, READ, o.in_off, {M, o.Cout, 2});
            span(ARENA, READ, o.aux_off[0], {o.B, o.aux_h[0], o.aux_w[0], o.Cout, 2});
            span(ARENA, WRITTEN, o.out_off, {M, o.Cout, 2});
            break;
        case SMAP_OP_TAPSUM:
            span(ARENA, READ, o.aux_off[0], {M, o.Cin, 4});
            span(WEIGHTS, READ, o.bias_off, {4});
            span(OUTPUT, WRITTEN, o.ext_off, {M, 4});
            status();
            break;
        case SMAP_OP_HEADSUM:
            for (int k = 0; k < o.n_aux && k < 3; ++k)
                span(ARENA, READ, o.aux_off[k], {o.flip_from > 0 ? 2 : 1, o.B, o.aux_h[k], o.aux_w[k], o.Cin, 4});
            if (o.flip_from > 0) span(WEIGHTS, READ, o.w_off, {o.Cout, 4});
            span(OUTPUT, WRITTEN, o.ext_off, {M, o.Cout, 4});
            status();
            break;
        default:
            return false;
    }
    return ok;
}

inline bool clear_of_zero_pages(int64_t off, int64_t bytes)
{
    const int64_t in_window = off & (SMAP_WINDOW - 1);
    return off >= 0 && in_window >= SMAP_ZERO_PAGE && bytes <= SMAP_WINDOW - in_window;
}

inline bool inside(int64_t off, int64_t size, int64_t total) { return off >= 0 && size >= 0 && size <= total && off <= total - size; }

int geometry(const smap_op& o)
{
    if (o.B <= 0 || o.H <= 0 || o.W <= 0 || o.Ho <= 0 || o.Wo <= 0 || o.Cout <= 0) return SMAP_E_ARG;
    if (o.precision != 0 && o.precision != 1) return SMAP_E_ARG;
    if (o.precision == 1 && o.kind == SMAP_OP_UPADD) return SMAP_E_ARG;
    const int64_t pl = 1 + o.precision, i31 = ((int64_t)1 << 31) - 1, i32 = (int64_t)1 << 32;
    switch (o.kind) {
        case SMAP_OP_CONV: {
            const TileRow* t = tile_find(o.tile);
            if (!t || !tile_has(*t, o.precision == 1)) return SMAP_E_ARG;
            const int bn = t->bn;
            if (o.Cin <= 0 || o.Cin % 64 || o.Cin * 2LL + 16 > SMAP_ZERO_PAGE || o.cout_pad % bn || o.cout_pad < o.Cout) return SMAP_E_ARG;
            if (o.precision == 1) {
                if (o.in_stride_c % 16 || (!o.out_fp32 && o.out_stride_c % 16)) return SMAP_E_ARG;
                if (o.Cin * 2LL + o.in_stride_c + 16 > SMAP_ZERO_PAGE || !(o.acc_scale > 0.f)) return SMAP_E_ARG;
                if ((int64_t)o.in_c_off + o.Cin > o.in_stride_c / 2) return SMAP_E_ARG;
            }
            if ((o.ksize != 1 && o.ksize != 3) || o.stride < 1) return SMAP_E_ARG;
            if (o.w_pairs != 0 && o.w_pairs != 1) return SMAP_E_ARG;
            if (t->family == TF_HALO && (o.ksize != 3 || o.stride != 1 || o.pad != 1 || o.res_off >= 0 || o.add1_off >= 0 ||
                                 o.add2_off >= 0 || o.aux_off[0] >= 0))
                return SMAP_E_ARG;
            if ((t->tail_bn > 0) != (o.tail_cout > 0)) return SMAP_E_ARG;
            if ((t->family == TF_BLOCK) != (o.head_cin > 0)) return SMAP_E_ARG;
            if (t->family == TF_BLOCK) {
                const bool first = t->first;
                if (o.ksize != 3 || o.stride != 1 || o.pad != 1 || o.out_fp32 || o.aux_off[0] >= 0) return SMAP_E_ARG;
                const int planes = t->planes;
                if (o.Cin != planes || o.Cout != planes || o.cout_pad != planes || o.head_cin != (first ? planes : 4 * planes) || o.tail_cout != 4 * planes ||
                    o.tail_cout_pad != 4 * planes)
                    return SMAP_E_ARG;
                if (o.in_stride_c != 2 * o.head_cin || o.in_c_off != 0) return SMAP_E_ARG;
                if (first ? (o.res_off >= 0 || o.add1_off >= 0 || o.add2_off >= 0 || !(o.short_acc_scale > 0.f))
                          : (o.res_off != o.in_off || o.short_acc_scale != 0.f))
                    return SMAP_E_ARG;
                if (!(o.head_acc_scale > 0.f) || !(o.tail_acc_scale > 0.f) || o.out_stride_c < o.tail_cout) return SMAP_E_ARG;
                if (!within(i31, {o.B, o.Ho, o.Wo, o.tail_cout, 2})) return SMAP_E_ARG;
            } else if (o.short_acc_scale != 0.f) return SMAP_E_ARG;
            if (t->family == TF_TAIL) {
                const int bn2 = t->tail_bn;
                if (o.ksize != 3 || o.stride != 1 || o.pad != 1 || o.out_fp32 || o.aux_off[0] >= 0 || o.Cout != bn || o.cout_pad != bn)
                    return SMAP_E_ARG;
                if (o.tail_cout % 8 || o.tail_cout_pad % bn2 || o.tail_cout_pad < o.tail_cout) return SMAP_E_ARG;
                if (o.precision == 1 && !(o.tail_acc_scale > 0.f)) return SMAP_E_ARG;
                if (o.out_stride_c < o.tail_cout) return SMAP_E_ARG;
                if (!within(i31, {o.B, o.Ho, o.Wo, o.tail_cout, pl})) return SMAP_E_ARG;
            }
            if ((t->caps & TC_REGEPI) && (o.out_fp32 || o.aux_off[0] >= 0 || o.add1_off >= 0 || o.add2_off >= 0 || o.Cout % 8 || o.ksplit > 1))
                return SMAP_E_ARG;
            if (t->family == TF_PERSIST && (o.out_fp32 || o.aux_off[0] >= 0 || o.Cout % 8 || o.cout_pad > 2048))
                return SMAP_E_ARG;
            if (o.in_stride_c % 8 || o.in_c_off % 8 || o.out_stride_c % 8 || o.out_c_off % 8) return SMAP_E_ARG;
            if (o.out_stride_c < cout8(o) && o.tap_n == 0) return SMAP_E_ARG;
            if ((o.res_off >= 0 || o.add1_off >= 0 || o.add2_off >= 0 || o.aux_off[0] >= 0) && o.Cout % 8) return SMAP_E_ARG;
            if (o.aux_off[0] >= 0 && (o.aux_h[0] <= 0 || o.aux_w[0] <= 0)) return SMAP_E_ARG;
            if (!within(i32, {o.cout_pad, o.ksize, o.ksize, o.Cin, 2, pl})) return SMAP_E_ARG;
            if (o.ksplit < 0 || o.ksplit > 16) return SMAP_E_ARG;
            if (o.ksplit > 1 && (!(t->caps & TC_SPLITK) || o.ksplit > o.ksize * o.ksize * o.Cin / tile_bk(*t, o.precision == 1)))
                return SMAP_E_ARG;
            if (o.tap_n != 0) {
                if (o.tap_n != 9 || !(t->caps & TC_TAPDOT) || o.cout_pad != 256 || o.Cout != 256 || o.ksize != 1 || o.stride != 1 || !o.out_fp32 || o.out_stride_c != 16 ||
                    o.out_c_off != 0 || o.res_off >= 0 || o.add1_off >= 0 || o.add2_off >= 0 || o.aux_off[0] >= 0 || o.seg_n[0] != 0 || o.ksplit > 1 || o.in2_C != 0 ||
                    !(o.tap_scale > 0.f))
                    return SMAP_E_ARG;
            }
            if (o.in2_C < 0) return SMAP_E_ARG;
            if (o.in2_C > 0) {
                if (!(t->caps & TC_DUAL) || o.ksize != 1 || o.stride != 1 || o.pad != 0 || o.ksplit > 1 || o.seg_n[0] != 0 || o.aux_off[0] >= 0 ||
                    o.add1_off >= 0 || o.add2_off >= 0 || o.out_fp32 || o.in_c_off != 0)
                    return SMAP_E_ARG;
                if (o.in2_C % 64 || o.in2_stride < 1 || o.in2_stride > 2 || o.in2_H <= 0 || o.in2_W <= 0) return SMAP_E_ARG;
                if (o.Ho != (o.in2_H - 1) / o.in2_stride + 1 || o.Wo != (o.in2_W - 1) / o.in2_stride + 1) return SMAP_E_ARG;
                if (o.in2_stride_c % 8 || o.in2_stride_c < o.in2_C * pl || (o.precision == 1 && o.in2_stride_c % 16)) return SMAP_E_ARG;
                if (o.in2_C * 2LL + (o.precision ? o.in2_stride_c : 0) + 16 > SMAP_ZERO_PAGE) return SMAP_E_ARG;
                if (window_of(o.in2_off) != window_of(o.in_off)) return SMAP_E_ARG;
                if (!within(i32, {o.cout_pad, (int64_t)o.Cin + o.in2_C, 2, pl})) return SMAP_E_ARG;
                if (o.in2_mode != 0 && o.in2_mode != 1) return SMAP_E_ARG;
                if (o.in2_mode == 1 && (!(t->caps & TC_RELUSUM) || o.in2_stride != 1 || o.res_off >= 0 || o.relu != 0 || (o.precision == 1 && !(o.in2_acc_scale > 0.f))))
                    return SMAP_E_ARG;
            } else if (o.in2_mode != 0) return SMAP_E_ARG;
            if (o.seg_n[0] == 0 && o.seg_n[1] != 0) return SMAP_E_ARG;
            if (o.seg_n[0] != 0) {
                if (t->family != TF_IGEMM || o.ksize != 1 || o.out_fp32 || o.out_c_off != 0) return SMAP_E_ARG;
                int prev = 0;
                for (int j = 0; j < 2 && o.seg_n[j] != 0; ++j) {
                    if (o.seg_n[j] <= prev || o.seg_n[j] % bn || o.seg_n[j] >= o.cout_pad) return SMAP_E_ARG;
                    const int end = (j == 0 && o.seg_n[1] != 0) ? o.seg_n[1] : o.cout_pad;
                    if (o.seg_cout[j] <= 0 || o.seg_cout[j] % 8 || (int64_t)o.seg_n[j] + o.seg_cout[j] > end) return SMAP_E_ARG;
                    if (o.seg_out_stride_c[j] % 8 || (o.precision == 1 && o.seg_out_stride_c[j] % 16)) return SMAP_E_ARG;
                    if (o.seg_out_stride_c[j] < o.seg_cout[j] * pl) return SMAP_E_ARG;
                    if (o.precision == 1 && !(o.seg_acc_scale[j] > 0.f)) return SMAP_E_ARG;
                    if (!within(i31, {o.B, o.Ho, o.Wo, o.seg_out_stride_c[j]})) return SMAP_E_ARG;
                    prev = o.seg_n[j];
                }
                if (cout8(o) > o.seg_n[0]) return SMAP_E_ARG;
            }
            if (!within(i31, {o.B, o.Ho, o.Wo, o.out_stride_c}) || !within(i31, {o.B, o.Ho, o.Wo, cout8(o), pl})) return SMAP_E_ARG;
            if (o.Ho != (o.H + 2LL * o.pad - o.ksize) / o.stride + 1 || o.Wo != (o.W + 2LL * o.pad - o.ksize) / o.stride + 1) return SMAP_E_ARG;
            return 0;
        }
        case SMAP_OP_STEM: case SMAP_OP_STEMPOOL: {
            int64_t h = (o.H + 6LL - 7) / 2 + 1, w = (o.W + 6LL - 7) / 2 + 1;
            if (o.kind == SMAP_OP_STEMPOOL) h = (h + 2 - 3) / 2 + 1, w = (w + 2 - 3) / 2 + 1;
            if (o.Cin != 3 || o.Cout != 64 || o.Ho != h || o.Wo != w) return SMAP_E_ARG;
            if (o.flip_from < 0 || (o.flip_from > 0 && o.B != 2LL * o.flip_from)) return SMAP_E_ARG;
            return 0;
        }
        case SMAP_OP_MAXPOOL:
            if (o.Cin % 8 || o.Cin != o.Cout || o.Ho != (o.H + 2LL - 3) / 2 + 1 || o.Wo != (o.W + 2LL - 3) / 2 + 1)
                return SMAP_E_ARG;
            return 0;
        case SMAP_OP_UPADD:
            if (o.Cout % 8 || o.aux_h[0] <= 0 || o.aux_w[0] <= 0) return SMAP_E_ARG;
            return 0;
        case SMAP_OP_TAPSUM:
            if (o.Cout != 1 || o.Cin < 9 || o.Cin % 4 || o.Ho != o.H || o.Wo != o.W) return SMAP_E_ARG;
            if (o.status_off < 0 || o.status_off % 4) return SMAP_E_ARG;
            return 0;
        case SMAP_OP_HEADSUM:
            if (o.n_aux < 1 || o.n_aux > 3 || o.Cout > 48 || o.Cin < o.Cout || o.Cin % 4) return SMAP_E_ARG;
            for (int k = 0; k < o.n_aux; ++k)
                if (o.aux_h[k] <= 0 || o.aux_w[k] <= 0) return SMAP_E_ARG;
            if (o.flip_from < 0 || (o.flip_from > 0 && (o.in_c_off < 0 || o.in_c_off > o.Cout))) return SMAP_E_ARG;
            if (o.flip_from > 0 && o.flip_from != o.B) return SMAP_E_ARG;
            if (o.status_off < 0 || o.status_off % 4) return SMAP_E_ARG;
            if ((o.scale_hms != 0 && o.scale_hms != 1) || (o.scale_hms && (o.in_c_off < 0 || o.in_c_off > o.Cout))) return SMAP_E_ARG;
            return 0;
        default:
            return SMAP_E_ARG;
    }
}

int validate(const smap_op& o)
{
    if (int rc = geometry(o)) return rc;
    bool bad = false;
    const bool sized = for_each_span(o, [&](const Span& s) {
        if (s.buf == ARENA)
            bad = bad || !clear_of_zero_pages(s.off, s.bytes) || (s.role == PARTIALS && s.off % 16) || (s.role == TICKETS && s.off % 4);
        else
            bad = bad || s.off < 0 || s.off > INT64_MAX - s.bytes;
    });
    return sized && !bad ? 0 : SMAP_E_ARG;
}

}

int plan_check(const smap_op* ops, int n_ops, PlanCheck* out)
{
    if (!ops || !out || n_ops <= 0 || n_ops > 4096) return SMAP_E_ARG;
    for (int i = 0; i < n_ops; ++i)
        if (int rc = validate(ops[i])) return rc;
    *out = PlanCheck();
    out->ops.assign(ops, ops + n_ops);
    out->signalled.assign(n_ops, 0);
    for (int i = 0; i < n_ops; ++i) {
        const smap_op& o = ops[i];
        if (o.lane < 0 || o.lane >= SMAP_MAX_LANES || o.n_wait < 0 || o.n_wait > 4) return SMAP_E_ARG;
        if (o.lane + 1 > out->n_lanes) out->n_lanes = o.lane + 1;
        for (int k = 0; k < o.n_wait; ++k) {
            const int w = o.wait_op[k];
            if (w < 0 || w >= i || ops[w].lane == o.lane) return SMAP_E_ARG;
            out->signalled[w] = 1;
        }
    }
    out->windows.assign(1, 0);
    for (int i = 0; i < n_ops; ++i) {
        const int64_t w = window_of(ops[i].in_off);
        if (ops[i].kind == SMAP_OP_CONV && std::find(out->windows.begin(), out->windows.end(), w) == out->windows.end()) out->windows.push_back(w);
        for_each_span(ops[i], [&](const Span& s) { if (s.role == TICKETS) out->tickets.push_back({s.off, s.bytes, i}); });
    }
    for (int i = 0; i < n_ops; ++i) {
        bool hit = false;
        for_each_span(ops[i], [&](const Span& s) {
            for (const PlanCheck::Ticket& t : out->tickets)
                hit = hit || (s.buf == ARENA && !(s.role == TICKETS && i == t.op) && s.off < t.off + t.bytes && t.off < s.off + s.bytes);
        });
        if (hit) return SMAP_E_ARG;
    }
    return 0;
}

void plan_workspace_bytes(const std::vector<smap_op>& ops, int64_t* arena_bytes, int64_t* out_bytes)
{
    int64_t ar = SMAP_ZERO_PAGE, ob = 0;
    for (const smap_op& o : ops)
        for_each_span(o, [&](const Span& s) {
            int64_t& m = s.buf == ARENA ? ar : ob;
            if (s.buf != WEIGHTS && s.off + s.bytes > m) m = s.off + s.bytes;
        });
    if (arena_bytes) *arena_bytes = ar;
    if (out_bytes) *out_bytes = ob;
}

int plan_check_blob(const void* blob, size_t blob_bytes, PlanCheck* out, smap_blob_info* info)
{
    if (!blob || !out || blob_bytes < sizeof(smap_blob_header)) return SMAP_E_ARG;
    smap_blob_header h;
    memcpy(&h, blob, sizeof(h));
    if (memcmp(h.magic, "SMAPPLN1", 8) || h.version != SMAP_BLOB_VERSION || h.sizeof_op != sizeof(smap_op) || h.header_bytes != sizeof(smap_blob_header))
        return SMAP_E_ARG;
    const int64_t total = (int64_t)blob_bytes;
    if (h.n_ops <= 0 || h.n_ops > 4096 || h.ops_offset < (int64_t)sizeof(h)) return SMAP_E_ARG;
    if (!inside(h.ops_offset, (int64_t)h.n_ops * (int64_t)sizeof(smap_op), total) || !inside(h.weights_offset, h.weights_bytes, total)) return SMAP_E_ARG;
    std::vector<smap_op> ops(h.n_ops);
    memcpy(ops.data(), static_cast<const char*>(blob) + h.ops_offset, (size_t)h.n_ops * sizeof(smap_op));
    if (int rc = plan_check(ops.data(), h.n_ops, out)) return rc;
    bool held = true;
    for (const smap_op& o : ops)
        for_each_span(o, [&](const Span& s) { held = held && (s.buf != WEIGHTS || inside(s.off, s.bytes, h.weights_bytes)); });
    int64_t ar = 0, ob = 0;
    plan_workspace_bytes(ops, &ar, &ob);
    if (!held || ar > h.arena_bytes || ob > h.out_bytes || ar > h.info.arena_bytes || ob > h.info.out_bytes ||
        h.info.weights_offset != h.weights_offset || h.info.weights_bytes != h.weights_bytes)
        return SMAP_E_ARG;
    if (info) *info = h.info;
    return 0;
}

extern "C" {

int smap_sizeof_op(void) { return (int)sizeof(smap_op); }

int smap_conv_tile_dims(int tile, int* bm, int* bn)
{
    const TileRow* t = tile_find(tile);
    if (t) { *bm = t->bm; *bn = t->bn; }
    return t ? 0 : -1;
}
int smap_conv_tile_bk(int tile, int precision) { const TileRow* t = tile_find(tile); return t ? tile_bk(*t, precision != 0) : 0; }
int smap_conv_tile_tail_bn(int tile) { const TileRow* t = tile_find(tile); return t ? t->tail_bn : 0; }

}
```

smap_amd/csrc/tiles.h:

```cpp
#pragma once

enum TileFamily {
    TF_IGEMM,
    TF_HALO,
    TF_PERSIST,
    TF_TAIL,
    TF_BLOCK
};

enum TileCap : unsigned {
    TC_F16 = 1,
    TC_X3 = 2,
    TC_BOTH = TC_F16 | TC_X3,
    TC_SPLITK = 4,
    TC_DUAL = 8,
    TC_RELUSUM = 16,
    TC_REGEPI = 32,
    TC_TAPDOT = 64
};

struct TileRow {
    int id;
    TileFamily family;
    int bm, bn;
    int bk16, bkx3;
    int tail_bn;
    int planes;
    bool first;
    unsigned caps;
};

constexpr TileRow SMAP_TILES[] = {
    {0, TF_IGEMM, 128, 128, 64, 64, 0, 0, false, TC_BOTH},
    {1, TF_IGEMM, 128, 64, 64, 64, 0, 0, false, TC_BOTH},
    {2, TF_IGEMM, 64, 64, 64, 64, 0, 0, false, TC_BOTH | TC_SPLITK},
    {3, TF_IGEMM, 128, 32, 64, 64, 0, 0, false, TC_BOTH},
    {4, TF_IGEMM, 64, 128, 64, 64, 0, 0, false, TC_BOTH},
    {5, TF_IGEMM, 128, 128, 64, 32, 0, 0, false, TC_F16},
    {6, TF_IGEMM, 128, 64, 64, 32, 0, 0, false, TC_F16},
    {7, TF_IGEMM, 64, 64, 64, 64, 0, 0, false, TC_BOTH | TC_SPLITK},
    {8, TF_IGEMM, 128, 32, 64, 32, 0, 0, false, TC_F16},
    {9, TF_IGEMM, 64, 128, 64, 32, 0, 0, false, TC_F16},
    {20, TF_IGEMM, 128, 128, 32, 32, 0, 0, false, TC_BOTH | TC_SPLITK | TC_DUAL},
    {21, TF_IGEMM, 128, 64, 32, 32, 0, 0, false, TC_BOTH},
    {22, TF_IGEMM, 64, 64, 32, 32, 0, 0, false, TC_BOTH | TC_SPLITK},
    {23, TF_IGEMM, 64, 128, 32, 32, 0, 0, false, TC_BOTH},
    {24, TF_IGEMM, 128, 128, 32, 32, 0, 0, false, TC_BOTH},
    {25, TF_IGEMM, 128, 64, 32, 32, 0, 0, false, TC_BOTH},
    {26, TF_IGEMM, 64, 64, 32, 32, 0, 0, false, TC_BOTH},
    {27, TF_IGEMM, 64, 128, 32, 32, 0, 0, false, TC_BOTH},
    {30, TF_HALO, 128, 64, 64, 32, 0, 0, false, TC_BOTH},
    {31, TF_HALO, 128, 128, 64, 32, 0, 0, false, TC_BOTH},
    {32, TF_HALO, 128, 64, 64, 32, 0, 0, false, TC_BOTH},
    {33, TF_HALO, 128, 128, 64, 32, 0, 0, false, TC_BOTH},
    {34, TF_HALO, 128, 64, 64, 32, 0, 0, false, TC_BOTH},
    {35, TF_HALO, 128, 128, 64, 32, 0, 0, false, TC_BOTH},
    {36, TF_HALO, 128, 64, 64, 32, 0, 0, false, TC_BOTH},
    {37, TF_HALO, 128, 128, 64, 32, 0, 0, false, TC_BOTH},
    {38, TF_HALO, 128, 32, 64, 32, 0, 0, false, TC_BOTH},
    {39, TF_HALO, 128, 32, 64, 32, 0, 0, false, TC_BOTH},
    {40, TF_HALO, 128, 128, 64, 32, 0, 0, false, TC_BOTH},
    {41, TF_HALO, 256, 128, 64, 32, 0, 0, false, TC_BOTH},
    {42, TF_HALO, 256, 64, 64, 32, 0, 0, false, TC_BOTH},
    {43, TF_HALO, 256, 128, 64, 32, 0, 0, false, TC_BOTH},
    {44, TF_HALO, 256, 128, 64, 32, 0, 0, false, TC_BOTH},
    {45, TF_HALO, 256, 128, 64, 32, 0, 0, false, TC_BOTH},
    {50, TF_IGEMM, 128, 128, 32, 32, 0, 0, false, TC_BOTH | TC_DUAL | TC_RELUSUM},
    {51, TF_IGEMM, 128, 128, 32, 32, 0, 0, false, TC_BOTH | TC_DUAL | TC_RELUSUM},
    {52, TF_IGEMM, 128, 128, 64, 64, 0, 0, false, TC_BOTH},
    {53, TF_IGEMM, 256, 128, 32, 32, 0, 0, false, TC_BOTH | TC_DUAL | TC_RELUSUM},
    {54, TF_IGEMM, 128, 256, 32, 32, 0, 0, false, TC_BOTH | TC_DUAL | TC_RELUSUM | TC_TAPDOT},
    {55, TF_IGEMM, 128, 128, 32, 32, 0, 0, false, TC_BOTH},
    {56, TF_IGEMM, 256, 256, 64, 32, 0, 0, false, TC_X3 | TC_REGEPI},
    {60, TF_PERSIST, 128, 256, 32, 32, 0, 0, false, TC_BOTH},
    {61, TF_PERSIST, 256, 128, 32, 32, 0, 0, false, TC_BOTH},
    {62, TF_PERSIST, 128, 128, 32, 32, 0, 0, false, TC_BOTH},
    {63, TF_PERSIST, 128, 64, 32, 32, 0, 0, false, TC_BOTH},
    {64, TF_PERSIST, 128, 64, 32, 32, 0, 0, false, TC_BOTH},
    {65, TF_PERSIST, 128, 64, 32, 32, 0, 0, false, TC_BOTH},
    {80, TF_TAIL, 128, 64, 64, 32, 64, 0, false, TC_BOTH},
    {81, TF_TAIL, 128, 64, 64, 32, 128, 0, false, TC_BOTH},
    {82, TF_TAIL, 128, 128, 64, 32, 64, 0, false, TC_BOTH},
    {90, TF_BLOCK, 64, 64, 64, 32, 64, 64, false, TC_X3},
    {91, TF_BLOCK, 128, 64, 64, 32, 64, 64, false, TC_X3},
    {92, TF_BLOCK, 64, 64, 64, 32, 64, 64, true, TC_X3},
    {93, TF_BLOCK, 128, 64, 64, 32, 64, 64, true, TC_X3},
    {94, TF_BLOCK, 128, 128, 64, 32, 128, 128, false, TC_X3},
};

constexpr int SMAP_N_TILES = sizeof(SMAP_TILES) / sizeof(SMAP_TILES[0]);

constexpr const TileRow* tile_find(int id)
{
    for (int i = 0; i < SMAP_N_TILES; ++i)
        if (SMAP_TILES[i].id == id) return &SMAP_TILES[i];
    return nullptr;
}

constexpr TileRow tile_row(int id) { return *tile_find(id); }

constexpr int tile_bk(const TileRow& t, bool x3) { return x3 ? t.bkx3 : t.bk16; }
constexpr bool tile_has(const TileRow& t, bool x3, unsigned caps = 0) { return (t.caps & ((x3 ? TC_X3 : TC_F16) | caps)) == ((x3 ? TC_X3 : TC_F16) | caps); }
```

smap_amd/engine.py:

```python
import ctypes as C
import os
from collections import namedtuple
from dataclasses import dataclass, field, fields

import torch

from . import lib as _L

OP_CONV, OP_STEM, OP_MAXPOOL, OP_UPADD, OP_HEADSUM, OP_STEMPOOL, OP_TAPSUM = range(7)

Tile = namedtuple("Tile", "family bm bn bk16 bkx3 caps tail_bn planes first prec", defaults=("", 0, 0, False, "f16 x3"))
TILE_TABLE = {
    0: Tile("igemm", 128, 128, 64, 64), 1: Tile("igemm", 128, 64, 64, 64), 2: Tile("igemm", 64, 64, 64, 64, "splitk"),
    3: Tile("igemm", 128, 32, 64, 64), 4: Tile("igemm", 64, 128, 64, 64),
    5: Tile("igemm", 128, 128, 64, 32, prec="f16"), 6: Tile("igemm", 128, 64, 64, 32, prec="f16"), 7: Tile("igemm", 64, 64, 64, 64, "splitk"),
    8: Tile("igemm", 128, 32, 64, 32, prec="f16"), 9: Tile("igemm", 64, 128, 64, 32, prec="f16"),
    20: Tile("igemm", 128, 128, 32, 32, "splitk dual"), 21: Tile("igemm", 128, 64, 32, 32), 22: Tile("igemm", 64, 64, 32, 32, "splitk"),
    23: Tile("igemm", 64, 128, 32, 32), 24: Tile("igemm", 128, 128, 32, 32), 25: Tile("igemm", 128, 64, 32, 32),
    26: Tile("igemm", 64, 64, 32, 32), 27: Tile("igemm", 64, 128, 32, 32),
    30: Tile("halo", 128, 64, 64, 32), 31: Tile("halo", 128, 128, 64, 32), 32: Tile("halo", 128, 64, 64, 32), 33: Tile("halo", 128, 128, 64, 32),
    34: Tile("halo", 128, 64, 64, 32), 35: Tile("halo", 128, 128, 64, 32), 36: Tile("halo", 128, 64, 64, 32), 37: Tile("halo", 128, 128, 64, 32),
    38: Tile("halo", 128, 32, 64, 32), 39: Tile("halo", 128, 32, 64, 32),
    40: Tile("halo", 128, 128, 64, 32), 41: Tile("halo", 256, 128, 64, 32), 42: Tile("halo", 256, 64, 64, 32), 43: Tile("halo", 256, 128, 64, 32),
    44: Tile("halo", 256, 128, 64, 32), 45: Tile("halo", 256, 128, 64, 32),
    50: Tile("igemm", 128, 128, 32, 32, "dual relusum"), 51: Tile("igemm", 128, 128, 32, 32, "dual relusum"), 52: Tile("igemm", 128, 128, 64, 64),
    53: Tile("igemm", 256, 128, 32, 32, "dual relusum"), 54: Tile("igemm", 128, 256, 32, 32, "dual relusum tapdot"), 55: Tile("igemm", 128, 128, 32, 32),
    56: Tile("igemm", 256, 256, 64, 32, "regepi", prec="x3"),
    60: Tile("persist", 128, 256, 32, 32), 61: Tile("persist", 256, 128, 32, 32), 62: Tile("persist", 128, 128, 32, 32),
    63: Tile("persist", 128, 64, 32, 32), 64: Tile("persist", 128, 64, 32, 32), 65: Tile("persist", 128, 64, 32, 32),
    80: Tile("tail", 128, 64, 64, 32, tail_bn=64), 81: Tile("tail", 128, 64, 64, 32, tail_bn=128), 82: Tile("tail", 128, 128, 64, 32, tail_bn=64),
    90: Tile("block", 64, 64, 64, 32, tail_bn=64, planes=64, prec="x3"), 91: Tile("block", 128, 64, 64, 32, tail_bn=64, planes=64, prec="x3"),
    92: Tile("block", 64, 64, 64, 32, tail_bn=64, planes=64, first=True, prec="x3"), 93: Tile("block", 128, 64, 64, 32, tail_bn=64, planes=64, first=True, prec="x3"),
    94: Tile("block", 128, 128, 64, 32, tail_bn=128, planes=128, prec="x3")}


def tile_family(tile):
    return TILE_TABLE[tile].family


def tile_bk(tile, x3):
    return TILE_TABLE[tile].bkx3 if x3 else TILE_TABLE[tile].bk16


def tile_has(tile, cap=None, x3=False):
    row = TILE_TABLE.get(tile)
    return row is not None and ("x3" if x3 else "f16") in row.prec.split() and (cap is None or cap in row.caps.split())


def tile_ids(family=None, cap=None, x3=None):
    fams = None if family is None else (family,) if isinstance(family, str) else tuple(family)
    return tuple(t for t, r in sorted(TILE_TABLE.items()) if (fams is None or r.family in fams)
                 and (tile_has(t, cap, x3) if x3 is not None else tile_has(t, cap, False) or tile_has(t, cap, True)))


X3_TILES = tuple(t for t in tile_ids(("igemm", "persist"), x3=True) if TILE_TABLE[t].bn >= 64)
REGEPI_TILES = tile_ids(cap="regepi")
TILES = {t: (r.bm, r.bn) for t, r in TILE_TABLE.items()}
TAIL_BN = {t: r.tail_bn for t, r in TILE_TABLE.items() if r.tail_bn}
HALO_ROWS = ("halo", "tail", "block")
TAIL_DEFAULT = {}
BLOCK_DEFAULT = {64: 91, 128: 94}
BLOCK_FIRST_DEFAULT = {64: 93}


_HERE = os.path.dirname(os.path.abspath(__file__))
_TABLE_FILES = {}


def _load_table(path):
    if not os.path.exists(path):
        return {}
    st = os.stat(path)
    key = (path, st.st_mtime_ns, st.st_size)
    if key not in _TABLE_FILES:
        import json
        _TABLE_FILES[key] = json.load(open(path))
    return _TABLE_FILES[key]


@dataclass(frozen=True)
class SchedulePolicy:
    block: tuple = None
    """SMAP_BLOCK="64:91,128:94": (Bottleneck planes, tile id) of the whole-block launches; () = none; None (unset) = the rule of Graph.block_tile."""
    block_first: tuple = None
    """SMAP_BLOCK_FIRST="64:93": the same for layer1's first block; None (unset) = BLOCK_FIRST_DEFAULT, 92 for 93 in small schedules."""
    tail: tuple = None
    """SMAP_TAIL="64:80,128:82": (planes, tile id) pairs of the fused 3x3 + 1x1 launches (Graph.conv_tail); None (unset) = TAIL_DEFAULT."""
    cat: bool = None
    """SMAP_CAT=0|1: a Bottleneck's last 1x1 and its shortcut conv as one launch (Graph.conv_cat) never / in small schedules too; None = in all but those."""
    skipsum: bool = None
    """SMAP_SKIPSUM=0|1: skip1 + skip2 of an Upsample_unit as one launch and one tensor (Graph.conv_relusum), the same way."""
    taphead: bool = None
    """SMAP_TAPHEAD=0|1: the root-depth head as tap-dot launch + stencil (Graph.conv_tapdot / tapsum), the same way."""
    merge_1x1: int = 1
    """SMAP_MERGE_1X1: shared-input 1x1s of an Upsample_unit as one launch (Graph.conv_seg): 1 = the merges that pay, 2 = all of them, 0 = one launch per conv."""
    splitk: str = ""
    """SMAP_SPLITK: "" (unset or "1") = the measured rule of Graph.split_k, "0" = off, "<n>" = n parts wherever a launch qualifies, "t<n>" = aim at n workgroups."""
    splitk_mink: int = 2048
    """SMAP_SPLITK_MINK: shortest K loop the measured split-K rule shares out (re-measured with the release / acquire ticket: EXPERIMENTS R6.5)."""
    deep_tile: bool = True
    """SMAP_DEEP_TILE=0 switches Graph.deep_pipeline_tile (tile 2 -> 7 for launches of <= 256 workgroups, profiles/r5_v9_*) off."""
    lanes: bool = False
    """SMAP_LANES=1: the independent head chains on forked streams (use_lanes; profiles/r5_v3_ab_b1.log)."""
    wpairs: int = None
    """SMAP_WPAIRS=0|1 forces one layout of the packed 32-half weight tiles; None = pairs in small schedules (use_w_pairs; profiles/r3_ab_wpairs*.log)."""
    x3_tile: int = None
    """SMAP_X3_TILE: one split-precision tile id put before the table's candidates wherever it fits (Graph._pick)."""
    cat_tile: int = None
    """SMAP_CAT_TILE: tile id of every Graph.conv_cat launch."""
    relusum_tile: int = None
    """SMAP_RELUSUM_TILE: tile id of every Graph.conv_relusum launch (profiles/r6_v14_ab_two_input_tiles.log)."""
    halo3: tuple = None
    """SMAP_HALO3="16" | "32" [":64" | ":128"]: (pixel-tile width, BN or None) -- every plain 3x3 with Cout > 32 on that halo tile (csrc/conv3.hip)."""
    halo3_deep: bool = False
    """SMAP_HALO3_DEEP: ... on its variant with the deeper weight pipeline (tile id + 4)."""
    tile_remap: tuple = ()
    """SMAP_TILE_REMAP="0:5,1:6": (tile id, tile id) pairs that swap variants of one tile shape (other pipeline depth) without touching the schedule."""
    tile_policy: str = ""
    """SMAP_TILE_POLICY="traffic[:min blocks]": experiment of pick_tile -- fewest L2 -> LDS bytes subject to a minimum block count (fp16)."""
    stempool: bool = False
    """SMAP_STEMPOOL: ResNet_top as one kernel that writes the pooled tensor only (bit-identical, no faster inside the two-batch pipeline)."""
    no_upadd_fusion: bool = False
    """SMAP_NO_UPADD_FUSION: fp16 with SMAP_MERGE_1X1=0 -- the bilinear add as a launch of its own (SMAP_OP_UPADD) instead of the u_skip conv's epilogue."""
    tile_table: dict = field(default_factory=dict, repr=False)
    """The measured fp16 table (pick_tile): SMAP_TILE_TABLE=<json>, default smap_amd/tile_table.json; {} under SMAP_NO_TILE_TABLE."""
    tile_table_x3: dict = field(default_factory=dict, repr=False)
    """The measured split-precision table (pick_tile_x3): SMAP_TILE_TABLE_X3=<json>, default smap_amd/tile_table_x3.json; {} under SMAP_NO_TILE_TABLE."""

    @classmethod
    def from_env(cls, environ=os.environ):
        get = lambda name, default="": environ.get("SMAP_" + name, default)
        pairs = lambda spec: None if spec is None else tuple((int(a), int(b)) for a, b in (kv.split(":") for kv in spec.split(",") if ":" in kv))
        tri = lambda name: {"0": False, "1": True}.get(get(name))
        num = lambda name: int(get(name)) if get(name) else None
        remap = pairs(get("TILE_REMAP"))
        assert all(TILES[a] == TILES[b] for a, b in remap), "remap must keep the tile shape"
        tw, _, bn = get("HALO3").partition(":")
        table = lambda name, shipped: {} if get("NO_TILE_TABLE") else _load_table(get(name) or os.path.join(_HERE, shipped))
        return cls(block=pairs(get("BLOCK", None)), block_first=pairs(get("BLOCK_FIRST", None)), tail=pairs(get("TAIL", None)),
                   cat=tri("CAT"), skipsum=tri("SKIPSUM"), taphead=tri("TAPHEAD"), merge_1x1={"0": 0, "2": 2}.get(get("MERGE_1X1"), 1),
                   splitk="" if get("SPLITK") == "1" else get("SPLITK"), splitk_mink=int(get("SPLITK_MINK", "2048")),
                   deep_tile=get("DEEP_TILE") != "0", lanes=get("LANES") == "1", wpairs={"0": 0, "1": 1}.get(get("WPAIRS")),
                   x3_tile=num("X3_TILE"), cat_tile=num("CAT_TILE"), relusum_tile=num("RELUSUM_TILE"),
                   halo3=(int(tw), int(bn) if bn else None) if tw else None, halo3_deep=bool(get("HALO3_DEEP")), tile_remap=remap,
                   tile_policy=get("TILE_POLICY"), stempool=bool(get("STEMPOOL")), no_upadd_fusion=bool(get("NO_UPADD_FUSION")),
                   tile_table=table("TILE_TABLE", "tile_table.json"), tile_table_x3=table("TILE_TABLE_X3", "tile_table_x3.json"))

    def cache_token(self):
        import hashlib
        import json
        digest = lambda t: hashlib.blake2b(json.dumps(t, sort_keys=True).encode(), digest_size=16).hexdigest()
        return tuple((f.name, digest(v) if isinstance(v, dict) else v) for f in fields(self) for v in (getattr(self, f.name),))


LAYERS = (3, 4, 6, 3)
PLANES = (64, 128, 256, 512)
ALIGN = 256
ZERO_PAGE = 16384
WINDOW = 1 << 32
PRECISIONS = ("f16", "x3")


def split_f16(w, scaled=True):
    import math
    m = float(w.abs().max())
    s = (13 - math.frexp(m)[1] + 1) if (scaled and m > 0) else 0
    ws = w.double() * (2.0 ** s)
    hi = ws.to(torch.float16)
    lo = (ws - hi.double()).to(torch.float16)
    assert torch.isfinite(hi).all()
    return hi, lo, 2.0 ** -s


def pack_stem_weights(w, x3):
    if x3:
        hi, lo, scale = split_f16(w.permute(0, 2, 1, 3).reshape(64, 21, 7))
        wk = torch.zeros((2, 64, 22, 8), dtype=torch.float16)
        wk[0, :, :21, :7], wk[1, :, :21, :7] = hi, lo
        return wk.reshape(2, 64, 176), scale
    wk = torch.zeros((64, 22, 8), dtype=torch.float16)
    wk[:, :21, :7] = w.permute(0, 2, 1, 3).reshape(64, 21, 7).to(torch.float16)
    return wk.reshape(64, 176), 1.0


def _table_entry(v):
    return [int(t) for t in v] if isinstance(v, (list, tuple)) else [int(v)]


def tile_legal(tile, *, cout, cout_pad=None, plain3=True, up=False, out_fp32=False, adds=False, x3=True):
    fam = tile_family(tile)
    if tile_has(tile, "regepi", True):
        return x3 and not up and not out_fp32 and not adds and cout % 8 == 0
    if fam == "halo":
        return plain3
    if fam in ("tail", "block"):
        return False
    if fam == "persist":
        cp = cout_pad if cout_pad is not None else _rup(cout, TILES[tile][1])
        return not up and not out_fp32 and cout % 8 == 0 and cp <= 2048
    return True


def pick_tile_x3(M, cout, key=None, policy=None):
    table = (policy or SchedulePolicy.from_env()).tile_table_x3
    keys = [key] if isinstance(key, str) else list(key or [])
    tuned = sorted({int(k.split(",")[0]) for k in table})
    if keys and tuned:
        f = int(keys[0].split(",")[0])
        if f not in tuned:
            import math
            near = min(tuned, key=lambda b: abs(math.log(b / f)))
            keys = keys + [",".join([str(near)] + k.split(",")[1:]) for k in keys]
    cands = [t for k in keys if k in table for t in _table_entry(table[k])]
    if cout <= 32:
        return cands + [3]
    best, best_blocks = None, -1
    for t in ((21, 22) if cout <= 64 else (20, 23, 21, 22)):
        bm, bn = TILES[t]
        blocks = -(-M // bm) * (-(-cout // bn))
        if blocks >= 512:
            return cands + [t]
        if blocks > best_blocks:
            best, best_blocks = t, blocks
    return cands + [best]


def use_lanes(frames, H, W, policy=None):
    return int((policy or SchedulePolicy.from_env()).lanes)


def use_w_pairs(small, policy=None):
    forced = (policy or SchedulePolicy.from_env()).wpairs
    return int(small) if forced is None else forced


def pack_conv_weights(w2, tile, x3, ksize, cin, pairs=True):
    planes, cout_pad, K = w2.shape
    assert planes == (2 if x3 else 1) and K == ksize * ksize * cin
    bn = TILES[tile][1]
    nt = cout_pad // bn
    assert nt * bn == cout_pad
    r = torch.arange(bn)
    if tile_family(tile) in HALO_ROWS:
        assert ksize == 3
        return pack_halo_rows(w2, bn, 9, cin, x3)
    bk = tile_bk(tile, x3)
    spr = bk // 8
    kt = K // bk
    assert kt * bk == K
    rows = w2.reshape(planes, nt, bn, kt, spr, 8).permute(1, 3, 0, 2, 4, 5)
    swz = ((r >> 1) & 7) if bk == 64 else ((r >> 2) & 3)
    idx = torch.arange(spr)[None, :] ^ swz[:, None]
    tiles = rows[:, :, :, r[:, None], idx, :]
    if bk == 32 and pairs:
        assert kt % 2 == 0
        tiles = tiles.reshape(nt, kt // 2, 2, planes, bn, spr, 8).permute(0, 1, 3, 4, 2, 5, 6)
    return tiles.contiguous()


def pack_halo_rows(w2, bn, taps, cin, x3):
    planes, cout_pad, K = w2.shape
    assert K == taps * cin and cout_pad % bn == 0
    nt = cout_pad // bn
    ch = 32 if x3 else 64
    cch = cin // ch
    assert cch * ch == cin
    r = torch.arange(bn)
    w = w2.reshape(planes, nt, bn, taps, cch, ch // 8, 8)
    if x3:
        rows = w.permute(1, 4, 3, 2, 0, 5, 6).reshape(nt, cch, taps, bn, 8, 8)
    else:
        rows = w[0].permute(0, 3, 2, 1, 4, 5)
    idx = torch.arange(8)[None, :] ^ ((r[:, None] >> 1) & 7)
    return rows[:, :, :, r[:, None], idx, :].contiguous()


def pack_rows16(w2):
    planes, rows, K = w2.shape
    assert planes == 2 and K % 16 == 0
    w = w2.reshape(2, rows, K // 16, 2, 8).permute(2, 1, 0, 3, 4).reshape(K // 16, rows, 4, 8)
    r = torch.arange(rows)
    idx = torch.arange(4)[None, :] ^ ((r[:, None] >> 2) & 3)
    return w[:, r[:, None], idx, :].contiguous()


def unpack_halo_rows(packed, bn, taps, cin, cout_pad, x3):
    planes, K = (2 if x3 else 1), taps * cin
    perm = pack_halo_rows(torch.arange(planes * cout_pad * K, dtype=torch.int64).reshape(planes, cout_pad, K), bn, taps, cin, x3).reshape(-1)
    out = torch.empty(planes * cout_pad * K, dtype=packed.dtype)
    out[perm] = packed.reshape(-1)
    return out.reshape(planes, cout_pad, K)


# ... 189 lines not shown
        if tiles >= 128 or n_k < 8:
            return 1
        if env.startswith("t"):
            s = min(8, int(env[1:]) // tiles, n_k // 4)
        elif env:
            s = min(int(env), 16, n_k)
        else:
            if K < self.policy.splitk_mink:
                return 1
            s = min(4, 256 // tiles, n_k // 8)
        return s if s >= 2 else 1

    def _split_k_fields(self, name, tile, M, cout_pad, ks):
        if ks <= 1:
            return {}, []
        bm, bn = TILES[tile]
        tiles = -(-M // bm) * (cout_pad // bn)
        part = Tensor(name + ".kpart", 1, 1, 1, tiles * ks * bm * bn, 4, 1)
        self.scratch_tensors.append(part)
        if self.kcount is None:
            self.kcount = Tensor("split_k.tickets", 1, 1, 1, 0, 4, 1)
        first_ticket = self.kcount_tiles
        self.kcount_tiles += tiles
        self.kcount.C = self.kcount_tiles
        return dict(ksplit=ks, kcount_first=first_ticket), [part]

    def _add_w(self, t):
        t = t.contiguous()
        raw = t.view(torch.uint8).reshape(-1) if t.dtype != torch.uint8 else t.reshape(-1)
        off = self.woff
        self.wchunks.append((off, raw))
        self.woff = _rup(off + raw.numel(), ALIGN)
        return off

    @property
    def small(self):
        return self.B * self.H * self.W <= 2 * 512 * 832

    @property
    def one_window(self):
        return self.B * self.H * self.W <= 20 * 512 * 832

    def _weights(self, name, rows, cout_pad=None):
        cout, K = rows.shape
        wk = torch.zeros((2 if self.x3 else 1, cout_pad or cout, K), dtype=torch.float16)
        acc_scale = 1.0
        if self.x3:
            wk[0, :cout], wk[1, :cout], acc_scale = split_f16(rows)
        else:
            wk[0, :cout] = rows.to(torch.float16)
            self._check_fp16(name, wk, rows)
        return wk, acc_scale

    def _check_fp16(self, name, wk, *folded):
        if not torch.isfinite(wk).all():
            raise ValueError(f"{name}: folded weights exceed the fp16 range (max |w| = {max(float(w.abs().max()) for w in folded):.3g})")

    def _bias(self, b, cout_pad=None):
        bk = torch.zeros((cout_pad or b.numel(),), dtype=torch.float32)
        bk[:b.numel()] = b.to(torch.float32)
        return bk

    def _ref(self, **folded):
        return {k + "_ref": v if self.keep_ref else None for k, v in folded.items()}

    def _forced_or_first(self, forced, cands, cap):
        return forced if forced is not None else next(t for t in cands if tile_has(t, cap, self.x3))

    def _pick(self, keys, legal, M, cout, K, *, key16, deep_pad, remap, remap16, x3_tile_fits=lambda t: True, tile=None):
        pol = self.policy
        if tile is not None:
            assert legal(tile), tile
        elif self.x3:
            cands = pick_tile_x3(M, cout, keys, pol)
            if pol.x3_tile is not None and x3_tile_fits(pol.x3_tile):
                cands = [pol.x3_tile] + cands
            tile = next(t for t in cands if legal(t))
            tile = remap.get(tile, tile)
        else:
            tile = pick_tile(M, cout, key16, pol)
            if remap16:
                tile = remap.get(tile, tile)
            if not legal(tile):
                tile = pick_tile_heuristic(M, cout)
        return self.deep_pipeline_tile(tile, M, deep_pad, K)

    def _conv_op(self, out, x, wk, bias, *, flops, alg_bytes, kinds, Cin, Cout, cout_pad, tile, acc_scale, ref, relu=1, ksize=1, stride=1,
                 in_c_off=0, out_fp32=0, frames=None, w_pairs=None, split_k=None, sub=None, **tensors):
        self.flops += flops
        self.alg_bytes += alg_bytes
        skf, scratch = {}, []
        if split_k:
            M, K = split_k
            skf, scratch = self._split_k_fields(out.name, tile, M, cout_pad, self.split_k(tile, M, cout_pad, K))
        p = dict(flops=flops, alg_bytes=alg_bytes, kinds=kinds, **skf,
                 Cin=Cin, in_c_off=in_c_off, Cout=Cout, ksize=ksize, stride=stride, pad=ksize // 2, relu=int(relu),
                 cout_pad=cout_pad, tile=tile, out_fp32=int(out_fp32), w_off=self._add_w(wk), bias_off=self._add_w(bias),
                 acc_scale=acc_scale, frames=self.B if frames is None else frames, w_pairs=self.w_pairs if w_pairs is None else w_pairs)
        p.update(sub() if sub else {}, **ref)
        self.ops.append(Op(OP_CONV, out=out, inp=x, scratch=scratch, p=p, **tensors))
        return out

    def conv(self, name, prefixes, x, ksize=1, stride=1, relu=True, res=None, add1=None, add2=None,
             in_c_off=0, cin=None, out_fp32=False, up=None, frames=None):
        ws, bs = zip(*[self._fold(p) for p in prefixes])
        w, b = torch.cat(ws, 0), torch.cat(bs, 0)
        cout, cin_w = w.shape[0], w.shape[1]
        cin = cin or x.C
        assert cin_w == cin and w.shape[2] == ksize, (name, w.shape, cin, ksize)
        pad = ksize // 2
        Ho = (x.H + 2 * pad - ksize) // stride + 1
        Wo = (x.W + 2 * pad - ksize) // stride + 1
        nfr = self.B if frames is None else frames
        M, K = nfr * Ho * Wo, ksize * ksize * cin
        key = f"{nfr},{x.H},{x.W},{cin},{cout},{ksize},{stride}"
        plain3 = ksize == 3 and stride == 1 and res is None and add1 is None and add2 is None and up is None
        legal = lambda t: tile_legal(t, cout=cout, plain3=plain3, up=up is not None, out_fp32=out_fp32,
                                     adds=add1 is not None or add2 is not None, x3=self.x3)
        tile = self._pick([key + ",up", key] if up is not None else [key], legal, M, cout, K, key16=key, deep_pad=_rup(cout, 64),
                          remap=dict(self.policy.tile_remap), remap16=True, x3_tile_fits=lambda t: cout > 32 and not (cout <= 64 and TILES[t][1] > 64))
        if self.policy.halo3 and plain3 and cout > 32:
            tw, hbn = self.policy.halo3
            hbn = hbn or min(TILES[tile][1], 128 if cout > 64 else 64)
            tile = {(16, 64): 30, (16, 128): 31, (32, 64): 32, (32, 128): 33}[(tw, max(hbn, 64))] + (4 if self.policy.halo3_deep else 0)
        cout_pad = _rup(cout, TILES[tile][1])
        wk, acc_scale = self._weights(name, w.permute(0, 2, 3, 1).reshape(cout, K), cout_pad)
        wk = pack_conv_weights(wk, tile, self.x3, ksize, cin, pairs=self.w_pairs)
        out = self.tensor(name, Ho, Wo, _rup(cout, 8), 4 if out_fp32 else 2)
        by = (nfr * x.H * x.W * cin * 2 * x.planes + nfr * Ho * Wo * out.C * out.esize * out.planes
              + wk.numel() * 2 + sum(t.nbytes * nfr // self.B for t in (res, add1, add2, up) if t is not None))
        return self._conv_op(out, x, wk, self._bias(b, cout_pad), flops=2 * M * cout * K, alg_bytes=by, kinds="1x1" if ksize == 1 else "3x3",
                             Cin=cin, Cout=cout, cout_pad=cout_pad, tile=tile, acc_scale=acc_scale, ref=self._ref(w=w, b=b), relu=relu,
                             ksize=ksize, stride=stride, in_c_off=in_c_off, out_fp32=out_fp32, frames=nfr, split_k=(M, K),
                             res=res, add1=add1, add2=add2, aux=[up] if up is not None else [])

    def conv_relusum(self, name, pre1, x, pre2, x2, tile=None):
        (w1, b1), (w2, b2) = self._fold(pre1), self._fold(pre2)
        cout, c1, c2 = w1.shape[0], w1.shape[1], w2.shape[1]
        assert w2.shape[0] == cout and w1.shape[2] == 1 == w2.shape[2] and c1 == x.C and c2 == x2.C and cout % 8 == 0 and (x.H, x.W) == (x2.H, x2.W)
        M, K = self.B * x.H * x.W, c1 + c2
        if tile is None:
            key = f"{self.B},{x.H},{x.W},{c1}+{c2}relusum,{cout},1,1"
            tile = self._forced_or_first(self.policy.relusum_tile, (pick_tile_x3(M, cout, key, self.policy) if self.x3 else []) + [54, 53, 50, 51], "relusum")
        assert tile_has(tile, "relusum", self.x3), tile
        cout_pad = _rup(cout, TILES[tile][1])
        wk1, sc1 = self._weights(name, w1.reshape(cout, c1), cout_pad)
        wk2, sc2 = self._weights(name, w2.reshape(cout, c2), cout_pad)
        wk = pack_conv_weights(torch.cat([wk1, wk2], 2), tile, self.x3, 1, K, pairs=self.w_pairs)
        out = self.tensor(name, x.H, x.W, cout)
        return self._conv_op(out, x, wk, self._bias(b1, cout_pad), flops=2 * M * cout * K, alg_bytes=x.nbytes + x2.nbytes + out.nbytes + wk.numel() * 2,
                             kinds="1x1", Cin=c1, Cout=cout, cout_pad=cout_pad, tile=tile, acc_scale=sc1, ref=self._ref(w=w1, b=b1), relu=0, aux2=x2,
                             sub=lambda: dict(cat=dict(cin=c2, stride=1, relusum=True, acc_scale=sc2, bias_off=self._add_w(self._bias(b2, cout_pad)),
                                                       **self._ref(w=w2, b=b2))))

    def conv_tapdot(self, name, pre1, pre3, x, frames=None):
        w1, b1 = self._fold(pre1)
        w3, b3 = self._fold(pre3)
        cout, cin = w1.shape[0], w1.shape[1]
        assert cout == 256 == w3.shape[1] and w3.shape[0] == 1 and w3.shape[2] == 3 and cin == x.C and w1.shape[2] == 1
        tile = tile_ids(cap="tapdot", x3=self.x3)[0]
        nfr = self.B if frames is None else frames
        M = nfr * x.H * x.W
        wk, acc_scale = self._weights(name, w1.reshape(cout, cin))
        wk = pack_conv_weights(wk, tile, self.x3, 1, cin, pairs=self.w_pairs)
        tw = torch.zeros((16, cout), dtype=torch.float64)
        tw[:9] = w3[0].permute(1, 2, 0).reshape(9, cout)
        thi, tlo, tap_scale = split_f16(tw)
        lane = torch.arange(64)
        kidx = (torch.arange(cout // 32)[:, None, None] * 32 + (lane // 16)[None, :, None] * 8 + torch.arange(8)[None, None, :])
        tapw = torch.stack([thi[(lane % 16)[None, :, None], kidx], tlo[(lane % 16)[None, :, None], kidx]], 1).contiguous()
        t = Tensor(name, self.B, x.H, x.W, 16, 4, 1)
        self.tensors.append(t)
        by = nfr * x.H * x.W * cin * 2 * x.planes + nfr * x.H * x.W * 16 * 4 + wk.numel() * 2
        self._conv_op(t, x, wk, self._bias(b1), flops=2 * M * cout * cin + 2 * M * 9 * cout, alg_bytes=by, kinds="1x1", Cin=cin, Cout=cout,
                      cout_pad=cout, tile=tile, acc_scale=acc_scale, ref=self._ref(w=w1, b=b1), out_fp32=1, frames=nfr,
                      sub=lambda: dict(tap=dict(w_off=self._add_w(tapw), scale=tap_scale, **self._ref(w=w3))))
        return t, b3

    def tapsum(self, t, b3, ext_off):
        self.ops.append(Op(OP_TAPSUM, aux=[t], p=dict(Cout=1, ext_off=ext_off, bias_off=self._add_w(b3.to(torch.float32).reshape(1)),
                                                       **self._ref(b=b3))))

    def conv_cat(self, name, pre1, x, pre2, x2, stride2, relu=True, tile=None):
        (w1, b1), (w2, b2) = self._fold(pre1), self._fold(pre2)
        cout, c1, c2 = w1.shape[0], w1.shape[1], w2.shape[1]
        assert w2.shape[0] == cout and w1.shape[2] == 1 == w2.shape[2] and c1 == x.C and c2 == x2.C and cout % 8 == 0
        Ho, Wo = x.H, x.W
        assert (x2.H - 1) // stride2 + 1 == Ho and (x2.W - 1) // stride2 + 1 == Wo
        M, K = self.B * Ho * Wo, c1 + c2
        if tile is None:
            key = f"{self.B},{Ho},{Wo},{c1}+{c2}cat,{cout},1,1"
            tile = self._forced_or_first(self.policy.cat_tile, (pick_tile_x3(M, cout, key, self.policy) if self.x3 else []) + [50, 51, 20], "dual")
        assert tile_has(tile, "dual", self.x3), tile
        cout_pad = _rup(cout, TILES[tile][1])
        wk, acc_scale = self._weights(name, torch.cat([w1.reshape(cout, c1), w2.reshape(cout, c2)], 1), cout_pad)
        wk = pack_conv_weights(wk, tile, self.x3, 1, K, pairs=self.w_pairs)
        out = self.tensor(name, Ho, Wo, cout)
        by = x.nbytes + self.B * Ho * Wo * c2 * 2 * x2.planes + out.nbytes + wk.numel() * 2
        return self._conv_op(out, x, wk, self._bias(b1 + b2, cout_pad), flops=2 * M * cout * K, alg_bytes=by, kinds="1x1", Cin=c1, Cout=cout,
                             cout_pad=cout_pad, tile=tile, acc_scale=acc_scale, ref=self._ref(w=w1, b=b1), relu=relu, aux2=x2,
                             sub=lambda: dict(cat=dict(cin=c2, stride=stride2, **self._ref(w=w2, b=b2))))

    def conv_seg(self, segs, x, up=None, tile=None):
        assert 2 <= len(segs) <= 3
        folded = [self._fold(pre) for _, pre, _ in segs]
        cin = x.C
        couts = [w.shape[0] for w, _ in folded]
        assert all(w.shape[1] == cin and w.shape[2] == 1 for w, _ in folded) and all(c % 8 == 0 for c in couts)
        M = self.B * x.H * x.W
        key = f"{self.B},{x.H},{x.W},{cin},{'+'.join(map(str, couts))},1,1"
        wide = f"{self.B},{x.H},{x.W},{cin},{max(couts)},1,1"
        legal = lambda t: (tile_family(t) == "igemm" and tile_has(t, None, self.x3) and TILES[t][1] >= 64
                           and (not tile_has(t, "regepi", True) or (self.x3 and up is None)))
        keys = ([key + ",up"] if up is not None else []) + [key] + ([wide + ",up"] if up is not None else []) + [wide]
        tile = self._pick(keys, legal, M, sum(couts), cin, key16=key, deep_pad=sum(_rup(c, 64) for c in couts),
                          remap={a: b for a, b in self.policy.tile_remap if b}, remap16=False, tile=tile)
        bn = TILES[tile][1]
        starts, n = [], 0
        for c in couts:
            starts.append(n)
            n = _rup(n + c, bn)
        cout_pad = n
        wk = torch.zeros((2 if self.x3 else 1, cout_pad, cin), dtype=torch.float16)
        bk = torch.zeros((cout_pad,), dtype=torch.float32)
        scales = []
        for (w, b), st, c in zip(folded, starts, couts):
            wk[:, st:st + c], sc = self._weights(segs[0][0], w.reshape(c, cin))
            bk[st:st + c] = b.to(torch.float32)
            scales.append(sc)
        self._check_fp16(segs[0][0], wk, *[w for w, _ in folded])
        wk = pack_conv_weights(wk, tile, self.x3, 1, cin, pairs=self.w_pairs)
        outs = [self.tensor(nm, x.H, x.W, c) for (nm, _, _), c in zip(segs, couts)]
        by = x.nbytes + sum(t.nbytes for t in outs) + wk.numel() * 2 + (up.nbytes if up is not None else 0)
        self._conv_op(outs[0], x, wk, bk, flops=2 * M * sum(couts) * cin, alg_bytes=by, kinds="1x1", Cin=cin, Cout=couts[0], cout_pad=cout_pad,
                      tile=tile, acc_scale=scales[0], ref=self._ref(w=folded[0][0], b=folded[0][1]), relu=segs[0][2], split_k=(M, cin),
                      aux=[up] if up is not None else [], outs=outs[1:],
                      sub=lambda: dict(segs=[dict(n0=st, cout=c, relu=int(r), acc_scale=sc, **self._ref(w=w, b=b))
                                             for st, c, (_, _, r), sc, (w, b) in list(zip(starts, couts, segs, scales, folded))[1:]]))
        return outs

    def conv_tail(self, name, pre3, pre1, x, tile, res=None, add1=None, add2=None):
        w3, b3 = self._fold(pre3)
        w1, b1 = self._fold(pre1)
        P, cin = w3.shape[0], w3.shape[1]
        cout = w1.shape[0]
        bn2 = TAIL_BN[tile]
        assert TILES[tile][1] == P == w1.shape[1] and cin == x.C and w3.shape[2] == 3 and w1.shape[2] == 1 and cout % 8 == 0
        cout_pad = _rup(cout, bn2)
        M = self.B * x.H * x.W
        K3 = 9 * cin
        wk3, sc3 = self._weights(name, w3.permute(0, 2, 3, 1).reshape(P, K3))
        wk1, sc1 = self._weights(name, w1.reshape(cout, P), cout_pad)
        wk3 = pack_halo_rows(wk3, P, 9, cin, self.x3)
        wk1 = pack_halo_rows(wk1, bn2, 1, P, self.x3)
        out = self.tensor(name, x.H, x.W, cout)
        by = (x.nbytes + out.nbytes + (wk3.numel() + wk1.numel()) * 2
              + sum(t.nbytes for t in (res, add1, add2) if t is not None))
        return self._conv_op(out, x, wk3, self._bias(b3), flops=2 * M * (P * K3 + cout * P), alg_bytes=by, kinds="3x3+1x1", Cin=cin, Cout=P, cout_pad=P,
                             tile=tile, acc_scale=sc3, ref=self._ref(w=w3, b=b3), ksize=3, w_pairs=0, res=res, add1=add1, add2=add2,
                             sub=lambda: dict(tail=dict(cout=cout, cout_pad=cout_pad, w_off=self._add_w(wk1), bias_off=self._add_w(self._bias(b1, cout_pad)),
                                                        acc_scale=sc1, **self._ref(w=w1, b=b1))))

    def conv_block_first(self, name, pre, x, tile):
        assert self.x3
        w1, b1 = self._fold(pre + ".conv_bn_relu1")
        w3, b3 = self._fold(pre + ".conv_bn_relu2")
        wt, bt = self._fold(pre + ".conv_bn_relu3")
        wd, bd = self._fold(pre + ".downsample")
        P, Cin = w1.shape[0], w1.shape[1]
        C = wt.shape[0]
        assert P == 64 == Cin == x.C and C == 256 and tuple(wd.shape[:2]) == (C, Cin) and wd.shape[2] == 1 and w3.shape[2] == 3
        M = self.B * x.H * x.W
        wk1, sc1 = self._weights(name, w1.reshape(P, Cin))
        wk1 = pack_halo_rows(wk1, P, 1, Cin, True)
        wk3, sc3 = self._weights(name, w3.permute(0, 2, 3, 1).reshape(P, 9 * P))
        wk3 = pack_halo_rows(wk3, P, 9, P, True)
        wkt, sct = self._weights(name, wt.reshape(C, P))
        wkt = pack_halo_rows(wkt, 64, 1, P, True)
        wkd, scd = self._weights(name, wd.reshape(C, Cin))
        wkd = pack_halo_rows(wkd, 64, 1, Cin, True)
        out = self.tensor(name, x.H, x.W, C)
        by = x.nbytes + out.nbytes + (wk1.numel() + wk3.numel() + wkt.numel() + wkd.numel()) * 2
        return self._conv_op(out, x, wk3, self._bias(b3), flops=2 * M * (P * Cin + P * 9 * P + C * P + C * Cin), alg_bytes=by, kinds="block", Cin=P,
                             Cout=P, cout_pad=P, tile=tile, acc_scale=sc3, ref=self._ref(w=w3, b=b3), ksize=3, w_pairs=0,
                             sub=lambda: dict(
                                 head=dict(cin=Cin, w_off=self._add_w(wk1), bias_off=self._add_w(self._bias(b1)), acc_scale=sc1, **self._ref(w=w1, b=b1)),
                                 tail=dict(cout=C, cout_pad=C, w_off=self._add_w(wkt), bias_off=self._add_w(self._bias(bt + bd)), acc_scale=sct,
                                           **self._ref(w=wt, b=bt)),
                                 short=dict(w_off=self._add_w(wkd), acc_scale=scd, **self._ref(w=wd, b=bd))))

    def conv_block(self, name, pre, x, tile, add1=None, add2=None):
        assert self.x3, "the whole-block kernel has a split-precision instance only"
        w1, b1 = self._fold(pre + ".conv_bn_relu1")
        w3, b3 = self._fold(pre + ".conv_bn_relu2")
        wt, bt = self._fold(pre + ".conv_bn_relu3")
        P, C = w1.shape[0], w1.shape[1]
        bn2 = TAIL_BN[tile]
        assert P == TILES[tile][1] and C == 4 * P == x.C == wt.shape[0] and w3.shape[:2] == (P, P) and w3.shape[2] == 3 and wt.shape[1] == P
        assert tile_family(tile) == "block" and not TILE_TABLE[tile].first and P == TILE_TABLE[tile].planes
        M = self.B * x.H * x.W
        wk1, sc1 = self._weights(name, w1.reshape(P, C))
        if P == 64:
            wk1 = pack_rows16(wk1)
        else:
            wk1 = pack_halo_rows(wk1, P, 1, C, True)
        wk3, sc3 = self._weights(name, w3.permute(0, 2, 3, 1).reshape(P, 9 * P))
        wk3 = pack_halo_rows(wk3, P, 9, P, True)
        wkt, sct = self._weights(name, wt.reshape(C, P))
        wkt = pack_halo_rows(wkt, bn2, 1, P, True)
        out = self.tensor(name, x.H, x.W, C)
        by = (x.nbytes + out.nbytes + (wk1.numel() + wk3.numel() + wkt.numel()) * 2
              + sum(t.nbytes for t in (add1, add2) if t is not None))
        return self._conv_op(out, x, wk3, self._bias(b3), flops=2 * M * (P * C + P * 9 * P + C * P), alg_bytes=by, kinds="block", Cin=P, Cout=P,
                             cout_pad=P, tile=tile, acc_scale=sc3, ref=self._ref(w=w3, b=b3), ksize=3, w_pairs=0, res=x, add1=add1, add2=add2,
                             sub=lambda: dict(
                                 head=dict(cin=C, w_off=self._add_w(wk1), bias_off=self._add_w(self._bias(b1)), acc_scale=sc1, **self._ref(w=w1, b=b1)),
                                 tail=dict(cout=C, cout_pad=C, w_off=self._add_w(wkt), bias_off=self._add_w(self._bias(bt)), acc_scale=sct,
                                           **self._ref(w=wt, b=bt))))

    def block_tile(self, planes, stride, has_ds):
        if stride != 1 or has_ds or not self.x3:
            return None
        if self.policy.block is None and self.small:
            return {64: 90}.get(planes)
        return dict(BLOCK_DEFAULT if self.policy.block is None else self.policy.block).get(planes)

    def _build(self):
        B, H, W, sd = self.B, self.H, self.W, self.sd
        w, b = self._fold("top.conv")
        wk, stem_scale = pack_stem_weights(w, self.x3)
        H2, W2 = (H + 6 - 7) // 2 + 1, (W + 6 - 7) // 2 + 1
        H4, W4 = (H2 + 2 - 3) // 2 + 1, (W2 + 2 - 3) // 2 + 1
        self.flops += 2 * B * H2 * W2 * 64 * 147
        stem_p = dict(w_off=self._add_w(wk), bias_off=self._add_w(b.to(torch.float32)), w_ref=w, b_ref=b, acc_scale=stem_scale)
        if not self.policy.stempool:
            t = self.tensor("top.conv", H2, W2, 64)
            self.ops.append(Op(OP_STEM, out=t, p=stem_p))
            x = self.tensor("top.pool", H4, W4, 64)
            self.ops.append(Op(OP_MAXPOOL, out=x, inp=t))
        else:
            x = self.tensor("top.pool", H4, W4, 64)
            self.ops.append(Op(OP_STEMPOOL, out=x, p=stem_p))
        self.out_h, self.out_w = H4, W4
        skip1 = skip2 = None
        for s in range(self.stage_num):
            last = s == self.stage_num - 1
            x, skip1, skip2 = self._stage(s, x, skip1, skip2, gen_skip=not last, heads=last)

    def _bottleneck(self, pre, x, planes, stride, has_ds, add1=None, add2=None):
        blk = self.block_tile(planes, stride, has_ds)
        if blk is not None:
            return self.conv_block(pre + ".c3", pre, x, blk, add1=add1, add2=add2)
        first = dict(BLOCK_FIRST_DEFAULT if self.policy.block_first is None else self.policy.block_first).get(planes)
        if self.policy.block_first is None and first == 93 and self.small:
            first = 92
        if first is not None and self.x3 and has_ds and stride == 1 and x.C == 64 and planes == 64 and add1 is None and add2 is None:
            return self.conv_block_first(pre + ".c3", pre, x, first)
        cat = (has_ds and add1 is None and add2 is None and self.policy.cat is not False and self.tail_tile(planes, stride) is None
               and self.one_window and (self.policy.cat or not self.small))
        idn = x if (not has_ds or cat) else self.conv(pre + ".downsample", [pre + ".downsample"], x, 1, stride, relu=False)
        y = self.conv(pre + ".c1", [pre + ".conv_bn_relu1"], x, 1, 1, relu=True)
        if cat:
            y = self.conv(pre + ".c2", [pre + ".conv_bn_relu2"], y, 3, stride, relu=True)
            return self.conv_cat(pre + ".c3", pre + ".conv_bn_relu3", y, pre + ".downsample", x, stride, relu=True)
        tail = self.tail_tile(planes, stride)
        if tail is not None:
            return self.conv_tail(pre + ".c3", pre + ".conv_bn_relu2", pre + ".conv_bn_relu3", y, tail, res=idn, add1=add1, add2=add2)
        y = self.conv(pre + ".c2", [pre + ".conv_bn_relu2"], y, 3, stride, relu=True)
        return self.conv(pre + ".c3", [pre + ".conv_bn_relu3"], y, 1, 1, relu=True, res=idn, add1=add1, add2=add2)

    def tail_tile(self, planes, stride):
        if stride != 1:
            return None
        return dict(TAIL_DEFAULT if self.policy.tail is None else self.policy.tail).get(planes)

    def _stage(self, s, x, skip1, skip2, gen_skip, heads):
        pre = f"stage{s}."
        feats = []
        inpl = 64
        for li, (planes, nblk) in enumerate(zip(PLANES, LAYERS)):
            stride = 1 if li == 0 else 2
            for j in range(nblk):
                lastb = j == nblk - 1
                a1 = skip1[li] if (skip1 is not None and lastb) else None
                a2 = skip2[li] if (skip2 is not None and lastb) else None
                has_ds = j == 0 and (stride != 1 or inpl != planes * 4)
                x = self._bottleneck(f"{pre}downsample.layer{li + 1}.{j}", x, planes, stride if j == 0 else 1,
                                     has_ds, a1, a2)
                inpl = planes * 4
            feats.append(x)
        x1, x2, x3, x4 = feats
        out, s1, s2, cross = None, [None] * 4, [None] * 4, None
        head_t = {}
        merge_mode = self.policy.merge_1x1
        merge = merge_mode != 0
        tl = None
        for ind, xin in enumerate((x4, x3, x2, x1)):
            u = f"{pre}upsample.up{ind + 1}"
            un = f"{pre}upsample.up{ind + 2}"
            ss = self.policy.skipsum
            skipsum = gen_skip and merge and ss is not False and self.one_window and (ss or not self.small)
            if merge:
                if gen_skip and not skipsum and (tl is None or merge_mode == 2):
                    out, s1[3 - ind] = self.conv_seg([(u + ".out", u + ".u_skip", True), (u + ".skip1", u + ".skip1", True)], xin, up=tl)
                else:
                    out = self.conv(u + ".out", [u + ".u_skip"], xin, relu=True, up=tl)
                    if gen_skip and not skipsum:
                        s1[3 - ind] = self.conv(u + ".skip1", [u + ".skip1"], xin, relu=True)
                if skipsum:
                    s1[3 - ind] = self.conv_relusum(u + ".skipsum", u + ".skip1", xin, u + ".skip2", out)
                sg = []
                if gen_skip:
                    if not skipsum:
                        sg.append((u + ".skip2", u + ".skip2", True))
                    if ind == 3:
                        sg.append((u + ".cross_conv", u + ".cross_conv", True))
                if heads and 1 <= ind < 3:
                    sg.append((u + ".res1", u + ".res_conv1", True))
                if ind < 3:
                    sg.append((un + ".up_conv@low", un + ".up_conv", False))
                got = {}
                if len(sg) >= 2:
                    got = dict(zip([n_ for n_, _, _ in sg], self.conv_seg(sg, out)))
                elif len(sg) == 1:
                    got = {sg[0][0]: self.conv(sg[0][0], [sg[0][1]], out, relu=sg[0][2])}
                tl = got.get(un + ".up_conv@low")
                if gen_skip:
                    s2[3 - ind] = None if skipsum else got[u + ".skip2"]
                    if ind == 3:
                        cross = got[u + ".cross_conv"]
                if heads:
                    if ind == 3:
                        tap = self.chl == 256 and self.policy.taphead is not False and (self.policy.taphead or not self.small)
                        m = self.conv(u + ".heads1x1", [u + ".res_conv1", u + ".res_d_conv1"] + ([] if tap else [u + ".res_rd_conv1"]), out, relu=True)
                        c = self.chl
                        head_t["res4"] = self.conv(u + ".res", [u + ".res_conv2"], m, 3, relu=False, in_c_off=0, cin=c, out_fp32=True)
                        with self.on_lane(1):
                            head_t["res_d"] = self.conv(u + ".res_d", [u + ".res_d_conv2"], m, 3, relu=False, in_c_off=c, cin=c, out_fp32=True,
                                                        frames=self.frames)
                        with self.on_lane(2):
                            if tap:
                                head_t["res_rd_tap"] = self.conv_tapdot(u + ".res_rd_t", u + ".res_rd_conv1", u + ".res_rd_conv2", out, frames=self.frames)
                            else:
                                head_t["res_rd"] = self.conv(u + ".res_rd", [u + ".res_rd_conv2"], m, 3, relu=False, in_c_off=2 * c, cin=c,
                                                             out_fp32=True, frames=self.frames)
                    elif ind >= 1:
                        with self.on_lane(1):
                            head_t[f"res{ind + 1}"] = self.conv(u + ".res", [u + ".res_conv2"], got[u + ".res1"], 3, relu=False, out_fp32=True)
                self._train_heads(s, ind, u, out, head_t if heads else {})
                continue
            if ind == 0:
                out = self.conv(u + ".out", [u + ".u_skip"], xin, relu=True)
            else:
                tl = self.conv(u + ".up_conv@low", [u + ".up_conv"], out, relu=False)
                if self.policy.no_upadd_fusion and not self.x3:
                    a = self.conv(u + ".u_skip", [u + ".u_skip"], xin, relu=False)
                    o = self.tensor(u + ".out", a.H, a.W, a.C)
                    self.ops.append(Op(OP_UPADD, out=o, inp=a, aux=[tl], p=dict(relu=1)))
                    out = o
                else:
                    out = self.conv(u + ".out", [u + ".u_skip"], xin, relu=True, up=tl)
            if gen_skip:
                lvl = 3 - ind
                s1[lvl] = self.conv(u + ".skip1", [u + ".skip1"], xin, relu=True)
                s2[lvl] = self.conv(u + ".skip2", [u + ".skip2"], out, relu=True)
                if ind == 3:
                    cross = self.conv(u + ".cross_conv", [u + ".cross_conv"], out, relu=True)
            if heads:
                if ind == 3:
                    m = self.conv(u + ".heads1x1", [u + ".res_conv1", u + ".res_d_conv1", u + ".res_rd_conv1"],
                                  out, relu=True)
                    c = self.chl
                    head_t["res4"] = self.conv(u + ".res", [u + ".res_conv2"], m, 3, relu=False, in_c_off=0,
                                               cin=c, out_fp32=True)
                    head_t["res_d"] = self.conv(u + ".res_d", [u + ".res_d_conv2"], m, 3, relu=False, in_c_off=c,
                                                cin=c, out_fp32=True, frames=self.frames)
                    head_t["res_rd"] = self.conv(u + ".res_rd", [u + ".res_rd_conv2"], m, 3, relu=False,
                                                 in_c_off=2 * c, cin=c, out_fp32=True, frames=self.frames)
                elif ind >= 1:
                    m = self.conv(u + ".res1", [u + ".res_conv1"], out, relu=True)
                    head_t[f"res{ind + 1}"] = self.conv(u + ".res", [u + ".res_conv2"], m, 3, relu=False,
                                                        out_fp32=True)
            self._train_heads(s, ind, u, out, head_t if heads else {})
        if heads:
            B, h, w = self.frames, self.out_h, self.out_w
            n_hms, n_d = self.kpt_paf, self.paf
            flip_p = {}
            if self.flip_pair is not None:
                flip_p = dict(flip_from=self.frames, n_kpt=n_hms - 2 * n_d,
                              w_off=self._add_w(torch.tensor(self.flip_pair, dtype=torch.int32)))
            self.out_layout = dict(hms=(0, n_hms), det_d=(B * n_hms * h * w * 4, n_d),
                                   root_d=(B * (n_hms + n_d) * h * w * 4, 1))
            self.out_bytes = B * (n_hms + n_d + 1) * h * w * 4
            self.status_off = self.out_bytes
            self.status_words = (B + 30) // 31
            self.ops.append(Op(OP_HEADSUM, aux=[head_t["res4"], head_t["res3"], head_t["res2"]],
                               p={**dict(Cout=n_hms, ext_off=self.out_layout["hms"][0], n_kpt=n_hms - 2 * n_d, scale_hms=int(self.scaled_hms)),
                                  **flip_p}))
            with self.on_lane(1):
                self.ops.append(Op(OP_HEADSUM, aux=[head_t["res_d"]], p=dict(Cout=n_d, ext_off=self.out_layout["det_d"][0])))
            with self.on_lane(2):
                if "res_rd_tap" in head_t:
                    self.tapsum(*head_t["res_rd_tap"], self.out_layout["root_d"][0])
                else:
                    self.ops.append(Op(OP_HEADSUM, aux=[head_t["res_rd"]], p=dict(Cout=1, ext_off=self.out_layout["root_d"][0])))
        return cross, (s1 if gen_skip else None), (s2 if gen_skip else None)

    def _train_heads(self, s, ind, u, out, head_t):
        if not self.all_heads:
            return
        have = {"heatmap_2d": head_t.get(f"res{ind + 1}"), "det_d": head_t.get("res_d") if ind == 3 else None,
                "root_d": head_t.get("res_rd") if ind == 3 else None}
        rd_in_output = ind == 3 and "res_rd_tap" in head_t
        todo = [(key, nm) for key, nm in (("heatmap_2d", "res"), ("det_d", "res_d"), ("root_d", "res_rd"))
                if have[key] is None and not (key == "root_d" and rd_in_output)]
        if todo:
            c = self.chl
            m = self.conv(u + ".heads1x1", [f"{u}.{nm}_conv1" for _, nm in todo], out, relu=True, frames=self.frames)
            for k, (key, nm) in enumerate(todo):
                have[key] = self.conv(f"{u}.{nm}", [f"{u}.{nm}_conv2"], m, 3, relu=False, in_c_off=k * c, cin=c, out_fp32=True,
                                      frames=self.frames)
        self.head_tensors[(s, ind)] = have
        self.keep += [t for t in have.values() if t is not None]

    def allocate(self, reuse=True):
        for i, op in enumerate(self.ops):
            for t in [op.inp, op.res, op.add1, op.add2, op.aux2] + list(op.aux):
                if t is not None:
                    t.last = i
            for t in ([op.out] if op.out is not None else []) + list(op.outs):
                t.first = i
                t.last = max(t.last, i)
            for t in op.scratch:
                t.first = t.last = i
        producer = {}
        for i, op in enumerate(self.ops):
            for t in ([op.out] if op.out is not None else []) + list(op.outs):
                producer[id(t)] = i
        n_last = len(self.ops) - 1
        for i, op in enumerate(self.ops):
            if not op.lane:
                continue
            reads = [t for t in [op.inp, op.res, op.add1, op.add2, op.aux2] + list(op.aux) if t is not None]
            start = 1 + max([producer.get(id(t), -1) for t in reads] + [-1])
            for t in ([op.out] if op.out is not None else []) + list(op.outs) + list(op.scratch):
                t.first = min(t.first, start)
            for t in reads + list(op.scratch):
                t.last = n_last
        if self.kcount is not None:
            self.kcount.first, self.kcount.last = 0, len(self.ops) - 1
        for t in self.keep:
            t.last = n_last
        every = self.tensors + self.scratch_tensors + ([self.kcount] if self.kcount is not None else [])
        for t in every:
            if _rup(t.nbytes, ALIGN) > WINDOW - ZERO_PAGE:
                raise ArenaTooLarge(f"{t.name}: {t.nbytes / 2 ** 30:.2f} GiB ({self.B} frames, precision {self.precision}) does not fit a "
                                    "4 GiB addressing window of the conv kernels -- use a smaller batch (PosePipeline splits by itself)")
        by_first = {}
        for t in every:
            by_first.setdefault(t.first, []).append(t)
        expiring = {}
        for t in every:
            expiring.setdefault(t.last, []).append(t)
        group = {}
        if not reuse:
            for op in self.ops:
                if op.kind == OP_CONV and "cat" in op.p:
                    g = list({id(t): t for t in group.get(id(op.inp), [op.inp]) + group.get(id(op.aux2), [op.aux2])}.values())
                    for t in g:
                        group[id(t)] = g
                        t.off = -1
        free, top = [], ZERO_PAGE
        for i in range(len(self.ops)):
            for t in by_first.get(i, []):
                if t.off >= 0 and id(t) in group:
                    continue
                need = _rup(t.nbytes, ALIGN)
                pick = None
                if reuse:
                    for k, (o, sz) in enumerate(free):
                        if sz >= need and (pick is None or sz < free[pick][1]):
                            pick = k
                if pick is not None:
                    o, sz = free.pop(pick)
                    t.off = o
                    if sz > need:
                        free.append((o + need, sz - need))
                else:
                    members = [m for m in group.get(id(t), [t]) if m is t or m.off < 0]
                    need = sum(_rup(m.nbytes, ALIGN) for m in members)
                    nxt = (top // WINDOW + 1) * WINDOW
                    if top + need > nxt:
                        if reuse and nxt > top:
                            free.append((top, nxt - top))
                        top = nxt + ZERO_PAGE
                    for m in members:
                        m.off = top
                        top += _rup(m.nbytes, ALIGN)
            for t in expiring.get(i, []):
                if reuse and t.off >= 0:
                    free.append((t.off, _rup(t.nbytes, ALIGN)))
                    free.sort()
                    merged = []
                    for o, sz in free:
                        if merged and merged[-1][0] + merged[-1][1] == o:
                            merged[-1] = (merged[-1][0], merged[-1][1] + sz)
                        else:
                            merged.append((o, sz))
                    free = merged
        self.arena_bytes = max(top, ALIGN)
        for t in every:
            if t.off >= 0:
                assert t.off % WINDOW >= ZERO_PAGE and t.off // WINDOW == (t.off + t.nbytes - 1) // WINDOW, t.name
        return self.arena_bytes

    def emit(self):
        arr = (_L.SmapOp * len(self.ops))()
        producer = {}
        for i, op in enumerate(self.ops):
            for t in ([op.out] if op.out is not None else []) + list(op.outs):
                producer[id(t)] = i
        for i, op in enumerate(self.ops):
            o = arr[i]
            C.memset(C.byref(o), 0, C.sizeof(o))
            o.lane = op.lane
            waits = {}
            for t in [op.inp, op.res, op.add1, op.add2, op.aux2] + list(op.aux):
                pi = producer.get(id(t)) if t is not None else None
                if pi is not None and self.ops[pi].lane != op.lane:
                    ln = self.ops[pi].lane
                    waits[ln] = max(waits.get(ln, -1), pi)
            for k in range(4):
                o.wait_op[k] = -1
            for k, pi in enumerate(sorted(waits.values())):
                o.wait_op[k] = pi
            o.n_wait = len(waits)
            o.kind = op.kind
            o.B = self.B
            o.res_off = o.add1_off = o.add2_off = -1
            for k in range(3):
                o.aux_off[k] = -1
            o.in_off = o.out_off = o.w_off = o.bias_off = o.ext_off = -1
            o.precision, o.acc_scale = int(self.x3), 1.0
            p = op.p
            if op.kind == OP_CONV:
                x, y = op.inp, op.out
                o.B = p["frames"]
                o.H, o.W, o.Cin, o.in_stride_c, o.in_c_off = x.H, x.W, p["Cin"], x.C * x.planes, p["in_c_off"]
                o.Ho, o.Wo, o.Cout = y.H, y.W, p["Cout"]
                o.ksize, o.stride, o.pad, o.relu = p["ksize"], p["stride"], p["pad"], p["relu"]
                o.cout_pad, o.out_stride_c, o.out_c_off = p["cout_pad"], y.C * y.planes, 0
                o.acc_scale = p["acc_scale"]
                o.w_pairs = p["w_pairs"]
                o.out_fp32, o.tile = p["out_fp32"], p["tile"]
                if "tail" in p:
                    tl = p["tail"]
                    o.tail_cout, o.tail_cout_pad, o.tail_acc_scale = tl["cout"], tl["cout_pad"], tl["acc_scale"]
                    o.tail_w_off, o.tail_bias_off = tl["w_off"], tl["bias_off"]
                if "head" in p:
                    hd = p["head"]
                    o.head_cin, o.head_acc_scale, o.head_w_off, o.head_bias_off = hd["cin"], hd["acc_scale"], hd["w_off"], hd["bias_off"]
                if "short" in p:
                    o.short_w_off, o.short_acc_scale = p["short"]["w_off"], p["short"]["acc_scale"]
                o.in_off, o.out_off, o.w_off, o.bias_off = x.off, y.off, p["w_off"], p["bias_off"]
                for nm in ("res", "add1", "add2"):
                    t = getattr(op, nm)
                    if t is not None:
                        assert (t.H, t.W, t.C) == (y.H, y.W, y.C) and t.esize == 2, (y.name, nm)
                        setattr(o, nm + "_off", t.off)
                if op.aux:
                    t = op.aux[0]
                    assert t.C == y.C and t.esize == 2
                    o.aux_off[0], o.aux_h[0], o.aux_w[0] = t.off, t.H, t.W
                if "tap" in p:
                    o.tap_n, o.tap_w_off, o.tap_scale = 9, p["tap"]["w_off"], p["tap"]["scale"]
                    o.out_stride_c = 16
                if "cat" in p:
                    t = op.aux2
                    assert t.off // WINDOW == x.off // WINDOW, (y.name, "both inputs of a conv_cat launch must lie in one 4 GiB window")
                    o.in2_off, o.in2_H, o.in2_W, o.in2_C, o.in2_stride_c, o.in2_stride = t.off, t.H, t.W, p["cat"]["cin"], t.C * t.planes, p["cat"]["stride"]
                    if p["cat"].get("relusum"):
                        o.in2_mode, o.in2_acc_scale, o.in2_bias_off = 1, p["cat"]["acc_scale"], p["cat"]["bias_off"]
                if p.get("ksplit", 1) > 1:
                    o.ksplit, o.kpart_off, o.kcount_off = p["ksplit"], op.scratch[0].off, self.kcount.off + 4 * p["kcount_first"]
                for j, (sg, t) in enumerate(zip(p.get("segs", []), op.outs)):
                    assert (t.H, t.W, t.C) == (y.H, y.W, sg["cout"]) and t.esize == 2
                    o.seg_n[j], o.seg_cout[j], o.seg_relu[j], o.seg_acc_scale[j] = sg["n0"], sg["cout"], sg["relu"], sg["acc_scale"]
                    o.seg_out_stride_c[j], o.seg_out_off[j] = t.C * t.planes, t.off
            elif op.kind in (OP_STEM, OP_STEMPOOL):
                y = op.out
                o.H, o.W, o.Cin, o.Ho, o.Wo, o.Cout = self.H, self.W, 3, y.H, y.W, 64
                o.ksize, o.stride, o.pad, o.relu = 7, 2, 3, 1
                o.out_off, o.w_off, o.bias_off = y.off, p["w_off"], p["bias_off"]
                o.acc_scale = p["acc_scale"]
                o.flip_from = self.frames if self.flip_pair is not None else 0
            elif op.kind == OP_MAXPOOL:
                x, y = op.inp, op.out
                o.H, o.W, o.Cin, o.Ho, o.Wo, o.Cout = x.H, x.W, x.C, y.H, y.W, y.C
                o.ksize, o.stride, o.pad = 3, 2, 1
                o.in_off, o.out_off = x.off, y.off
            elif op.kind == OP_UPADD:
                x, y, t = op.inp, op.out, op.aux[0]
                o.H, o.W, o.Cin, o.Ho, o.Wo, o.Cout = x.H, x.W, x.C, y.H, y.W, y.C
                o.relu = p["relu"]
                o.in_off, o.out_off = x.off, y.off
                o.aux_off[0], o.aux_h[0], o.aux_w[0] = t.off, t.H, t.W
            elif op.kind == OP_TAPSUM:
                t = op.aux[0]
                o.H, o.W, o.Cin, o.Ho, o.Wo, o.Cout = t.H, t.W, t.C, self.out_h, self.out_w, 1
                o.aux_off[0], o.aux_h[0], o.aux_w[0] = t.off, t.H, t.W
                o.ext_off, o.bias_off = p["ext_off"], p["bias_off"]
                o.B = self.frames
                o.status_off = self.status_off
            elif op.kind == OP_HEADSUM:
                s0 = op.aux[0]
                assert all(t.C == s0.C and t.esize == 4 for t in op.aux)
                o.H, o.W, o.Cin, o.Ho, o.Wo, o.Cout = s0.H, s0.W, s0.C, self.out_h, self.out_w, p["Cout"]
                o.n_aux = len(op.aux)
                for k, t in enumerate(op.aux):
                    o.aux_off[k], o.aux_h[k], o.aux_w[k] = t.off, t.H, t.W
                o.ext_off = p["ext_off"]
                o.B = self.frames
                o.status_off = self.status_off
                if p.get("flip_from"):
                    o.flip_from, o.in_c_off, o.w_off = p["flip_from"], p["n_kpt"], p["w_off"]
                if p.get("scale_hms"):
                    o.scale_hms, o.in_c_off = 1, p["n_kpt"]
        return arr

    def blob(self):
        ops = self.emit()
        n_ops = len(self.ops)
        hdr = _L.BlobHeader()
        ops_off = _rup(C.sizeof(hdr), ALIGN)
        ops_bytes = C.sizeof(_L.SmapOp) * n_ops
        w_off = _rup(ops_off + ops_bytes, ALIGN)
        wblob = self.weight_blob().numpy().tobytes()
        hdr.magic, hdr.version, hdr.sizeof_op, hdr.header_bytes = b"SMAPPLN1", _L.BLOB_VERSION, C.sizeof(_L.SmapOp), C.sizeof(hdr)
        hdr.n_ops, hdr.ops_offset = n_ops, ops_off
        hdr.weights_offset, hdr.weights_bytes = w_off, len(wblob)
        hdr.arena_bytes, hdr.out_bytes = self.arena_bytes, self.out_bytes + 4 * self.status_words
        i = hdr.info
        i.frames, i.H, i.W, i.out_h, i.out_w = self.frames, self.H, self.W, self.out_h, self.out_w
        i.n_hms, i.n_det, i.n_root, i.precision = self.kpt_paf, self.paf, 1, int(self.x3)
        i.arena_bytes, i.out_bytes, i.weights_offset, i.weights_bytes = hdr.arena_bytes, hdr.out_bytes, w_off, len(wblob)
        i.hms_off, i.det_off, i.root_off = self.out_layout["hms"][0], self.out_layout["det_d"][0], self.out_layout["root_d"][0]
        i.status_off = self.status_off
        out = bytearray(w_off + len(wblob))
        out[:C.sizeof(hdr)] = bytes(hdr)
        out[ops_off:ops_off + ops_bytes] = bytes(ops)
        out[w_off:] = wblob
        return bytes(out)

    def weight_blob(self):
        blob = torch.zeros((max(self.woff, ALIGN),), dtype=torch.uint8)
        for off, raw in self.wchunks:
            blob[off:off + raw.numel()] = raw
        return blob


PLAN_CACHE_KEEP = 6


def plan_cache_dir():
    d = os.environ.get("SMAP_PLAN_CACHE", "")
    return None if d in ("", "0") else os.path.expanduser(d)


def state_hash(sd):
    try:
        import xxhash
        h = xxhash.xxh3_128()
    except ImportError:
        import hashlib
        h = hashlib.blake2b(digest_size=16)
    for k in sorted(sd):
        t = sd[k].detach().cpu().contiguous()
        h.update(f"{k}|{tuple(t.shape)}|{t.dtype}|".encode())
        h.update(t.reshape(-1).view(torch.uint8).numpy().data if t.numel() else b"")
    return h.hexdigest()


BUILDER_SOURCES = ("engine.py",)


def plan_cache_key(sd, B, H, W, stage_num, chl, kpt_paf, paf, precision, flip_pair, scaled_hms, all_heads=False, policy=None):
    import hashlib
    policy = policy or SchedulePolicy.from_env()
    h = hashlib.blake2b(digest_size=16)
    h.update(repr((state_hash(sd), B, H, W, stage_num, chl, kpt_paf, paf, precision, tuple(flip_pair) if flip_pair is not None else None,
                   bool(scaled_hms), _L.BLOB_VERSION, C.sizeof(_L.SmapOp), _L.version(), policy.cache_token(), bool(all_heads))).encode())
    for f in BUILDER_SOURCES:
        h.update(open(os.path.join(_HERE, f), "rb").read())
    return h.hexdigest()


HeadSource = namedtuple("HeadSource", "ptr h w c pix_stride ch_stride frame_stride")
HEAD_KEYS = (("heatmap_2d", "kpt_paf"), ("det_d", "paf"), ("root_d", None))


def graph_head_sources(g, arena_ptr=0, out_ptr=0):
    res = []
    for s in range(g.stage_num):
        for ind in range(4):
            d = {}
            for key, attr in HEAD_KEYS:
                t, c = g.head_tensors[(s, ind)][key], (getattr(g, attr) if attr else 1)
                if t is not None:
                    assert t.esize == 4 and t.off >= 0 and t.C >= c
                    d[key] = HeadSource(arena_ptr + t.off, t.H, t.W, c, t.C, 1, t.H * t.W * t.C)
                else:
                    hw = g.out_h * g.out_w
                    d[key] = HeadSource(out_ptr + g.out_layout[key][0], g.out_h, g.out_w, c, 1, hw, c * hw)
            res.append(d)
    return res


class BackboneEngine:

    def __init__(self, state_dict, B, H, W, device, stage_num=3, chl=256, kpt_paf=43, paf=14, reuse=True,
                 precision="f16", flip_pair=None, scaled_hms=False, all_heads=False):
        self.lib = _L.load()
        self.precision = precision
        self.device = torch.device(device)
        if self.device.type != "cuda":
            raise RuntimeError("BackboneEngine needs a ROCm GPU device (no CPU path in smap_amd)")
        sd = {k: v.detach().cpu() for k, v in state_dict.items()}
        self.policy = SchedulePolicy.from_env()
        self._graph_args = (sd, B, H, W, stage_num, chl, kpt_paf, paf, precision, flip_pair, scaled_hms, reuse, bool(all_heads), self.policy)
        self.all_heads, self.stage_num = bool(all_heads), stage_num
        self._graph = None
        self.B, self.H, self.W = B, H, W
        self.kpt_paf, self.paf = kpt_paf, paf
        self.from_cache = False
        cdir = plan_cache_dir() if reuse else None
# ... 195 lines not shown
```

Before: 880.6 frames/sec.

## Fuse cross_conv 1x1 as a rider into the skip relu-sum launch

The Upsample_unit's cross_conv, a 1x1 conv on the same second input as the skip2 path, is folded into the relu-sum igemm launch as an extra 64-column rider. The kernel reorders its K loop so the second-input chunks run first, reuses the already-staged A fragments for three extra MFMAs per chunk, and writes the rider output from an LDS buffer at the end. This saves one kernel launch and one re-read of the shared activation tensor. In exchange it adds LDS footprint, register pressure and planner and arena complexity for that single tile instance.

```diff
diff --git a/smap_amd/csrc/assoc.hip b/smap_amd/csrc/assoc.hip
--- a/smap_amd/csrc/assoc.hip
+++ b/smap_amd/csrc/assoc.hip
@@ -987,4 +987,4 @@
     return 0;
 }
 
-extern "C" const char* smap_version(void) { return "smap_hip gfx950 r6 (assoc + backbone f16|x3 + flip-TTA + persistent conv + whole-Bottleneck launches + plan blob v2 + windowed arena + N segments + split K + lanes + two-input launches + tap-dot head + scaled head sum + two-launch peak search)"; }
+extern "C" const char* smap_version(void) { return "smap_hip gfx950 r6 (assoc + backbone f16|x3 + flip-TTA + persistent conv + whole-Bottleneck launches + plan blob v2 + windowed arena + N segments + split K + lanes + two-input launches + tap-dot head + scaled head sum + two-launch peak search + relu-sum rider)"; }
diff --git a/smap_amd/csrc/conv.hip b/smap_amd/csrc/conv.hip
--- a/smap_amd/csrc/conv.hip
+++ b/smap_amd/csrc/conv.hip
@@ -10,11 +10,12 @@
 #define SMAP_ABLATE 0
 #endif
 template <int BM, int BN, int WM, int WN, int STAGES, int BK, bool FULL, bool X3, bool SPLITK = false, bool REGEPI = false, bool DUAL = false, bool TAPDOT = false,
-          bool RELUSUM = false>
+          bool RELUSUM = false, bool RIDER = false>
 __global__ __launch_bounds__(WM * WN * 64) void conv_igemm_kernel(const ConvArgs a)
 {
     static_assert(!TAPDOT || (!FULL && !SPLITK && !REGEPI && !DUAL), "tap-dot epilogue: plain instance only");
     static_assert(!RELUSUM || DUAL, "relu-sum: a second input");
+    static_assert(!RIDER || (RELUSUM && X3 && BK == 32 && STAGES == 2 && BM == 128 && BN == 256 && WM == 2 && WN == 4), "rider: the 128 x 256 relu-sum instance");
     static_assert(!REGEPI || (X3 && !FULL && !SPLITK), "register epilogue: split precision, plain epilogue, no split K");
     static_assert(!DUAL || (!FULL && !SPLITK && !REGEPI), "second input: plain epilogue, no split K");
     constexpr int NPL = X3 ? 2 : 1;
@@ -30,11 +31,14 @@
     constexpr int LA = BM / RPR, LB = BN / RPR;
     constexpr int MI = BM / WM / 32, NI = BN / WN / 32;
     static_assert(MI >= 1 && NI >= 1, "tile too small for the wave grid");
-    constexpr int STAGE = NPL * (BM + BN) * ROWB;
+    constexpr int RN = RIDER ? 64 : 0;
+    constexpr int STAGE = NPL * (BM + BN + RN) * ROWB;
+    static_assert(!RIDER || NPL * RN == RPR, "the rider's rows of a K tile are ONE round of the LDS-DMA");
     constexpr int LPT = NPL * (LA + LB);
     static_assert((STAGES - 2) * LPT <= 63, "vmcnt is 6 bits");
     constexpr int CSS = TAPDOT ? BN + 8 : BN;
-    constexpr int LDS_BYTES = REGEPI ? STAGES * STAGE : (STAGES * STAGE > BM * CSS * 4 ? STAGES * STAGE : BM * CSS * 4) + (SPLITK ? 16 : 0);
+    constexpr int EPI_BYTES = STAGES * STAGE > BM * CSS * 4 ? STAGES * STAGE : BM * CSS * 4;
+    constexpr int LDS_BYTES = REGEPI ? STAGES * STAGE : EPI_BYTES + (SPLITK ? 16 : 0) + BM * RN * 4;
     static_assert(LDS_BYTES <= 160 * 1024, "LDS is 160 KiB per CU");
     __shared__ __attribute__((aligned(16))) char smem[LDS_BYTES];
 
@@ -63,7 +67,7 @@
     const int o_relu = seg == 0 ? a.relu : seg == 1 ? a.seg_relu1 : a.seg_relu2;
     const float o_scale = seg == 0 ? a.acc_scale : seg == 1 ? a.seg_scale1 : a.seg_scale2;
     const int o_lo = o_stride >> 1;
-    const _Float16* const o_res = seg == 0 ? a.res : nullptr;
+    const _Float16* const o_res = (seg == 0 && !RIDER) ? a.res : nullptr;
     const _Float16* const o_up = seg == 0 ? a.up : nullptr;
     const _Float16* const o_add1 = seg == 0 ? a.add1 : nullptr;
     const _Float16* const o_add2 = seg == 0 ? a.add2 : nullptr;
@@ -82,7 +86,10 @@
 #pragma unroll
     for (int j = 0; j < NPL * LB; ++j) w_off[j] = (unsigned)((j * RPR + wave * RPW + lrow) * wrow + lslot * 16);
     const char* __restrict__ wt_tile = wt + (long long)n_tile * (wpair ? a.K / 64 : a.K / BK) * wblk;
-    auto issue_b = [&](int buf, int it) {
+    const int cchunks = a.Cin / BK;
+    const int cchunks2 = DUAL ? a.Cin2 / BK : 0;
+    auto issue_b = [&](int buf, int kt) {
+        const int it = RIDER ? (kt < cchunks2 ? cchunks + kt : kt - cchunks2) : kt;
         char* sB = smem + buf * STAGE + NPL * BM * ROWB;
         const char* gB = wpair ? wt_tile + (long long)(it >> 1) * wblk + (it & 1) * 64 : wt_tile + (long long)it * wblk;
 #pragma unroll
@@ -138,8 +145,6 @@
             while (oy >= a.Ho) { oy -= a.Ho; ++b; }
         }
     }
-    const int cchunks = a.Cin / BK;
-    const int cchunks2 = DUAL ? a.Cin2 / BK : 0;
     const int n_all = a.ksize * a.ksize * cchunks + cchunks2;
     const int it_lo = S > 1 ? ks * n_all / S : 0;
     const int n_iter = (S > 1 ? (ks + 1) * n_all / S : n_all) - it_lo;
@@ -161,6 +166,15 @@
         for (int i = 0; i < LA; ++i) a_cur[i] = (a_mask[i] & bit) ? a_off[i] + tap_off : 0u;
     };
     set_tap();
+    if (RIDER) {
+        s_in2 = 1;
+#pragma unroll
+        for (int i = 0; i < LA; ++i) a_cur[i] = a_off2[i];
+    }
+    auto issue_r = [&](int buf, int kt) {
+        lds_dma16(reinterpret_cast<const char*>(a.rider_w) + (long long)kt * (NPL * RN * ROWB) + w_off[0],
+                  smem + buf * STAGE + NPL * (BM + BN) * ROWB + wave * RPW * ROWB);
+    };
     auto issue_a = [&](int buf) {
 #pragma unroll
         for (int pl = 0; pl < NPL; ++pl) {
@@ -173,6 +187,10 @@
     };
     auto advance = [&]() {
         ++s_it;
+        if (RIDER) {
+            if (++s_cc == cchunks2 && s_in2) { s_cc = 0; s_in2 = 0; set_tap(); }
+            return;
+        }
         if (DUAL && s_in2) { ++s_cc; return; }
         if (++s_cc == cchunks) {
             s_cc = 0;
@@ -189,11 +207,13 @@
     auto stage = [&](int buf) {
         issue_a(buf);
         issue_b(buf, s_it);
+        if (RIDER && s_in2) issue_r(buf, s_it);
         advance();
     };
     if (!(SMAP_ABLATE & 1)) {
         if (SPLITK) issue_b(0, it_lo);
         issue_a(0);
+        if (RIDER) issue_r(0, 0);
         advance();
     }
 
@@ -244,9 +264,17 @@
     const int b_row0 = wn * (BN / WN) + l31;
     f32x16 park[RELUSUM ? MI : 1][RELUSUM ? NI : 1];
     float bias1[RELUSUM ? NI : 1];
+    f32x16 racc;
+    if (RIDER) {
+#pragma unroll
+        for (int r = 0; r < 16; ++r) racc[r] = 0.f;
+    }
+    float* const Rs = reinterpret_cast<float*>(smem + (RIDER ? EPI_BYTES : 0));
+    const float rbias = RIDER ? a.rider_bias[(wn & 1) * 32 + l31] : 0.f;
+    const float scale1 = RIDER ? a.acc_scale_b : o_scale;
     if (RELUSUM) {
 #pragma unroll
-        for (int ni = 0; ni < NI; ++ni) bias1[ni] = a.bias[n0 + wn * (BN / WN) + ni * 32 + l31];
+        for (int ni = 0; ni < NI; ++ni) bias1[ni] = (RIDER ? a.bias_b : a.bias)[n0 + wn * (BN / WN) + ni * 32 + l31];
     }
 
     TR(1);
@@ -254,7 +282,10 @@
     for (int st = 1; st < STAGES - 1; ++st)
         if (st < n_iter && !(SMAP_ABLATE & 1)) stage(st);
     int buf = 0, nbuf = STAGES - 1;
-    for (int it = 0; it < n_iter; ++it) {
+    int it = 0;
+#pragma unroll
+    for (int phase = RIDER ? 0 : 1; phase < 2; ++phase)
+    for (const int it_end = (RIDER && phase == 0) ? cchunks2 : n_iter; it < it_end; ++it) {
 #ifdef SMAP_TRACE
         const long long tw0 = __builtin_amdgcn_s_memtime();
 #endif
@@ -267,14 +298,20 @@
         if (it == 0) tr_t[2] = __builtin_amdgcn_s_memtime();
 #endif
         if (it + STAGES - 1 < n_iter && !(SMAP_ABLATE & 1)) stage(nbuf);
-        if (RELUSUM && it == cchunks) {
+        if (RELUSUM && it == (RIDER ? cchunks2 : cchunks)) {
+            if constexpr (RIDER) {
+#pragma unroll
+                for (int r = 0; r < 16; ++r)
+                    Rs[(wm * (BM / WM) + (wn >> 1) * 32 + (r & 3) + 8 * (r >> 2) + 4 * lhi) * RN + (wn & 1) * 32 + l31] = racc[r] * a.rider_scale + rbias;
+                __builtin_amdgcn_sched_barrier(0);
+            }
 #pragma unroll
             for (int mi = 0; mi < MI; ++mi)
 #pragma unroll
                 for (int ni = 0; ni < NI; ++ni)
 #pragma unroll
                     for (int r = 0; r < 16; ++r) {
-                        const float v = X3 ? acc[mi][ni][r] * o_scale + bias1[ni] : acc[mi][ni][r] + bias1[ni];
+                        const float v = X3 ? acc[mi][ni][r] * scale1 + bias1[ni] : acc[mi][ni][r] + bias1[ni];
                         park[mi][ni][r] = v < 0.f ? 0.f : v;
                         acc[mi][ni][r] = 0.f;
                     }
@@ -310,6 +347,17 @@
                     }
                     acc[mi][ni] = __builtin_amdgcn_mfma_f32_32x32x16_f16(af[0][mi], bf[0][ni], acc[mi][ni], 0, 0, 0);
                 }
+            if constexpr (RIDER) {
+                if (phase == 0) {
+                    const char* sR = sB + NPL * BN * ROWB + ((wn & 1) * 32 + l31) * ROWB + slot;
+                    const half8 rh = *reinterpret_cast<const half8*>(sR), rl = *reinterpret_cast<const half8*>(sR + RN * ROWB);
+                    const bool up = (wn >> 1) != 0;
+                    const half8 ah = up ? af[0][1] : af[0][0], al = up ? af[1][1] : af[1][0];
+                    racc = __builtin_amdgcn_mfma_f32_32x32x16_f16(al, rh, racc, 0, 0, 0);
+                    racc = __builtin_amdgcn_mfma_f32_32x32x16_f16(ah, rl, racc, 0, 0, 0);
+                    racc = __builtin_amdgcn_mfma_f32_32x32x16_f16(ah, rh, racc, 0, 0, 0);
+                }
+            }
         }
         buf = buf + 1 == STAGES ? 0 : buf + 1;
         nbuf = nbuf + 1 == STAGES ? 0 : nbuf + 1;
@@ -391,14 +439,14 @@
 #pragma unroll
     for (int ni = 0; ni < NI; ++ni) {
         const int col = wn * (BN / WN) + ni * 32 + l31;
-        const float bias = RELUSUM ? a.bias_b[n0 + col] : a.bias[n0 + col];
+        const float bias = (RELUSUM && !RIDER) ? a.bias_b[n0 + col] : a.bias[n0 + col];
 #pragma unroll
         for (int mi = 0; mi < MI; ++mi)
 #pragma unroll
             for (int r = 0; r < 16; ++r) {
                 const int row = wm * (BM / WM) + mi * 32 + (r & 3) + 8 * (r >> 2) + 4 * lhi;
                 if (RELUSUM) {
-                    const float v = X3 ? acc[mi][ni][r] * a.acc_scale_b + bias : acc[mi][ni][r] + bias;
+                    const float v = X3 ? acc[mi][ni][r] * (RIDER ? o_scale : a.acc_scale_b) + bias : acc[mi][ni][r] + bias;
                     Cs[row * CSS + col] = (v < 0.f ? 0.f : v) + park[mi][ni][r];
                     continue;
                 }
@@ -574,6 +622,30 @@
         if (p + ED < PASSES) ex[(p + ED) % (ED + 1)] = load_pass(p + ED);
         finish_pass(p, ex[p % (ED + 1)]);
     }
+    if constexpr (RIDER) {
+        _Float16* const rout = reinterpret_cast<_Float16*>(a.rider_out);
+        const int r_lo = a.rider_stride >> 1;
+#pragma unroll
+        for (int p = 0; p < BM * (RN / 8) / NT; ++p) {
+            const int idx = p * NT + tid;
+            const int row = idx / (RN / 8), cg = idx - row * (RN / 8);
+            const int m = m0 + row, n = cg * 8;
+            if (m >= a.M || n >= a.rider_cout8) continue;
+            const float4 lo = *reinterpret_cast<const float4*>(Rs + row * RN + n);
+            const float4 hi = *reinterpret_cast<const float4*>(Rs + row * RN + n + 4);
+            float v[8] = {lo.x, lo.y, lo.z, lo.w, hi.x, hi.y, hi.z, hi.w};
+            half8 h, l;
+#pragma unroll
+            for (int e = 0; e < 8; ++e) {
+                if (a.rider_relu) v[e] = v[e] < 0.f ? 0.f : v[e];
+                h[e] = (_Float16)v[e];
+                l[e] = (_Float16)(v[e] - (float)h[e]);
+            }
+            _Float16* op = rout + ((unsigned)m * (unsigned)a.rider_stride + (unsigned)n);
+            *reinterpret_cast<half8*>(op) = h;
+            *reinterpret_cast<half8*>(op + r_lo) = l;
+        }
+    }
 #ifdef SMAP_TRACE
     asm volatile("s_waitcnt vmcnt(0)" ::: "memory");
     TR(5);
@@ -645,6 +717,16 @@
 }
 
 template <int TILE, bool X3, int WM, int WN, int STAGES>
+hipError_t launch_relusum_rider(const ConvArgs& a, hipStream_t st)
+{
+    SMAP_IGEMM_ROW(TC_DUAL | TC_RELUSUM | TC_RIDER);
+    if (a.up || a.add1 || a.add2 || a.res || a.ksplit > 1 || a.ksize != 1 || a.relu || !a.bias_b) return hipErrorInvalidValue;
+    if (!a.rider_bias || !a.rider_out || a.n_tiles != 1 || a.w_pairs || a.rider_cout8 <= 0 || a.rider_cout8 > 64 || a.rider_cout8 % 8) return hipErrorInvalidValue;
+    hipLaunchKernelGGL((conv_igemm_kernel<BM, BN, WM, WN, STAGES, BK, false, X3, false, false, true, false, true, true>), dim3(a.m_tiles), dim3(WM * WN * 64), 0, st, a);
+    return hipGetLastError();
+}
+
+template <int TILE, bool X3, int WM, int WN, int STAGES>
 hipError_t launch_tapdot(const ConvArgs& a, hipStream_t st)
 {
     SMAP_IGEMM_ROW(TC_TAPDOT);
@@ -675,6 +757,8 @@
             default: return hipErrorInvalidValue;
         }
     }
+    if (a.Cin2 > 0 && a.bias_b && a.rider_w)
+        return tile == 54 && a.x3 ? launch_relusum_rider<54, true, 2, 4, 2>(a, st) : hipErrorInvalidValue;
     if (a.Cin2 > 0 && a.bias_b) {
         switch (tile) {
             case 50: return SMAP_BOTH(launch_relusum, 50, 2, 4, 2);
diff --git a/smap_amd/csrc/plan.h b/smap_amd/csrc/plan.h
--- a/smap_amd/csrc/plan.h
+++ b/smap_amd/csrc/plan.h
@@ -50,6 +50,11 @@
     void* seg_out1; void* seg_out2;
     int seg_cout8_1, seg_cout8_2, seg_stride1, seg_stride2, seg_relu1, seg_relu2;
     float seg_scale1, seg_scale2;
+    const _Float16* rider_w;
+    const float* rider_bias;
+    void* rider_out;
+    int rider_cout8, rider_stride, rider_relu;
+    float rider_scale;
 #ifdef SMAP_TRACE
     long long* dbg;
 #endif
diff --git a/smap_amd/csrc/plan.hip b/smap_amd/csrc/plan.hip
--- a/smap_amd/csrc/plan.hip
+++ b/smap_amd/csrc/plan.hip
@@ -604,7 +604,7 @@
     a.Cin2 = o.in2_C > 0 ? o.in2_C : 0;
     a.in2_off = o.in2_C > 0 ? o.in2_off - window_of(o.in_off) : 0;
     a.H2 = o.in2_H; a.W2 = o.in2_W; a.in2_stride_c = o.in2_stride_c; a.stride2 = o.in2_stride; a.in2_lo = o.in2_stride_c / 2;
-    a.bias_b = (o.in2_C > 0 && o.in2_mode == 1) ? reinterpret_cast<const float*>(wb + o.in2_bias_off) : nullptr;
+    a.bias_b = (o.in2_C > 0 && o.in2_mode >= 1) ? reinterpret_cast<const float*>(wb + o.in2_bias_off) : nullptr;
     a.acc_scale_b = o.in2_acc_scale;
     a.x3 = o.precision;
     a.in_lo = o.in_stride_c / 2;
@@ -626,6 +626,9 @@
     a.tap_n = o.tap_n;
     a.tap_w = o.tap_n > 0 ? reinterpret_cast<const _Float16*>(wb + o.tap_w_off) : nullptr;
     a.tap_scale = o.tap_scale;
+    a.rider_w = nullptr; a.rider_bias = nullptr; a.rider_out = nullptr;
+    a.rider_cout8 = a.rider_stride = a.rider_relu = 0;
+    a.rider_scale = 1.f;
     a.ksplit = o.ksplit > 1 ? o.ksplit : 1;
     a.kpart = o.ksplit > 1 ? reinterpret_cast<float*>(ar + o.kpart_off) : nullptr;
     a.kcount = o.ksplit > 1 ? reinterpret_cast<unsigned*>(ar + o.kcount_off) : nullptr;
@@ -640,6 +643,17 @@
     a.m_tiles = (a.M + t.bm - 1) / t.bm;
     a.n_tiles = o.cout_pad / t.bn;
     return a;
+}
+
+static void conv_ride(ConvArgs& a, const smap_op& r, char* ar, const char* wb)
+{
+    a.rider_w = reinterpret_cast<const _Float16*>(wb + r.w_off);
+    a.rider_bias = reinterpret_cast<const float*>(wb + r.bias_off);
+    a.rider_out = ar + r.out_off;
+    a.rider_cout8 = (r.Cout + 7) & ~7;
+    a.rider_stride = r.out_stride_c;
+    a.rider_relu = r.relu;
+    a.rider_scale = r.acc_scale;
 }
 
 static int run_ops(const smap_plan* plan, int first, int count, const float* const* inputs, int n_inputs, void* arena,
@@ -686,9 +700,16 @@
         for (int l = 1; l < plan->n_lanes; ++l)
             if (hipError_t e = hipStreamWaitEvent(plan->side[l], plan->join_ev[0], 0); e != hipSuccess) return hip_rc(e);
     }
+    bool ridden = false;
     for (int i = first; i < first + count; ++i) {
         const smap_op& o = plan->ops[i];
         hipError_t e = hipSuccess;
+        if (ridden) {
+            ridden = false;
+            if (lanes && plan->signalled[i])
+                if (hipError_t e2 = hipEventRecord(plan->ev[i], st); e2 != hipSuccess) return fail(hip_rc(e2));
+            continue;
+        }
         if (lanes) {
             st = o.lane > 0 ? plan->side[o.lane] : st0;
             for (int k = 0; k < o.n_wait; ++k)
@@ -697,6 +718,10 @@
         switch (o.kind) {
             case SMAP_OP_CONV: {
                 ConvArgs a = conv_args(o, ar, wb);
+                if (o.in2_mode == 2 && i + 1 < first + count) {
+                    conv_ride(a, plan->ops[i + 1], ar, wb);
+                    ridden = true;
+                }
 #ifdef SMAP_TIMELINE
                 a.tl = nullptr;
                 if (tl_base() && tl_next < tl_cap()) {
diff --git a/smap_amd/csrc/plan_check.cpp b/smap_amd/csrc/plan_check.cpp
--- a/smap_amd/csrc/plan_check.cpp
+++ b/smap_amd/csrc/plan_check.cpp
@@ -69,7 +69,7 @@
                 span(WEIGHTS, READ, o.head_bias_off, {o.Cin, 4});
                 if (o.short_acc_scale > 0.f) span(WEIGHTS, READ, o.short_w_off, {o.tail_cout, o.head_cin, 2, pl});
             }
-            if (o.in2_C > 0 && o.in2_mode == 1) span(WEIGHTS, READ, o.in2_bias_off, {o.cout_pad, 4});
+            if (o.in2_C > 0 && o.in2_mode >= 1) span(WEIGHTS, READ, o.in2_bias_off, {o.cout_pad, 4});
             if (o.tap_n > 0) span(WEIGHTS, READ, o.tap_w_off, {o.cout_pad / 32, 2 * 64 * 8 * 2});
             break;
         }
@@ -190,8 +190,10 @@
                 if (o.in2_C * 2LL + (o.precision ? o.in2_stride_c : 0) + 16 > SMAP_ZERO_PAGE) return SMAP_E_ARG;
                 if (window_of(o.in2_off) != window_of(o.in_off)) return SMAP_E_ARG;
                 if (!within(i32, {o.cout_pad, (int64_t)o.Cin + o.in2_C, 2, pl})) return SMAP_E_ARG;
-                if (o.in2_mode != 0 && o.in2_mode != 1) return SMAP_E_ARG;
-                if (o.in2_mode == 1 && (!(t->caps & TC_RELUSUM) || o.in2_stride != 1 || o.res_off >= 0 || o.relu != 0 || (o.precision == 1 && !(o.in2_acc_scale > 0.f))))
+                if (o.in2_mode < 0 || o.in2_mode > 2) return SMAP_E_ARG;
+                if (o.in2_mode == 2 && (!(t->caps & TC_RIDER) || o.precision != 1 || o.cout_pad != bn || o.w_pairs != 0))
+                    return SMAP_E_ARG;
+                if (o.in2_mode >= 1 && (!(t->caps & TC_RELUSUM) || o.in2_stride != 1 || o.res_off >= 0 || o.relu != 0 || (o.precision == 1 && !(o.in2_acc_scale > 0.f))))
                     return SMAP_E_ARG;
             } else if (o.in2_mode != 0) return SMAP_E_ARG;
             if (o.seg_n[0] == 0 && o.seg_n[1] != 0) return SMAP_E_ARG;
@@ -259,6 +261,25 @@
     return sized && !bad ? 0 : SMAP_E_ARG;
 }
 
+int rider_pair(const smap_op& s, const smap_op& r)
+{
+    const TileRow* t = tile_find(r.tile);
+    if (r.kind != SMAP_OP_CONV || t->family != TF_IGEMM || t->bn != 64 || tile_bk(*t, true) != 32 || r.precision != 1) return SMAP_E_ARG;
+    if (r.ksize != 1 || r.stride != 1 || r.pad != 0 || r.cout_pad != 64 || r.Cout % 8 || r.w_pairs != 0 || r.out_fp32 || r.out_c_off != 0) return SMAP_E_ARG;
+    if (r.res_off >= 0 || r.add1_off >= 0 || r.add2_off >= 0 || r.aux_off[0] >= 0 || r.seg_n[0] != 0 || r.ksplit > 1 || r.in2_C != 0 || r.tap_n != 0 ||
+        r.tail_cout != 0 || r.head_cin != 0)
+        return SMAP_E_ARG;
+    if (r.in_off != s.in2_off || r.in_stride_c != s.in2_stride_c || r.in_c_off != 0 || r.Cin != s.in2_C || r.B != s.B || r.H != s.in2_H || r.W != s.in2_W ||
+        r.Ho != s.Ho || r.Wo != s.Wo)
+        return SMAP_E_ARG;
+    if (r.lane != s.lane || r.n_wait != 0) return SMAP_E_ARG;
+    int64_t lo = 0, bytes = 0;
+    for_each_span(r, [&](const Span& x) { if (x.buf == ARENA && x.role == WRITTEN) { lo = x.off; bytes = x.bytes; } });
+    bool hit = false;
+    for_each_span(s, [&](const Span& x) { hit = hit || (x.buf == ARENA && x.off < lo + bytes && lo < x.off + x.bytes); });
+    return hit ? SMAP_E_ARG : 0;
+}
+
 }
 
 int plan_check(const smap_op* ops, int n_ops, PlanCheck* out)
@@ -266,6 +287,9 @@
     if (!ops || !out || n_ops <= 0 || n_ops > 4096) return SMAP_E_ARG;
     for (int i = 0; i < n_ops; ++i)
         if (int rc = validate(ops[i])) return rc;
+    for (int i = 0; i < n_ops; ++i)
+        if (ops[i].kind == SMAP_OP_CONV && ops[i].in2_mode == 2)
+            if (i + 1 >= n_ops || rider_pair(ops[i], ops[i + 1])) return SMAP_E_ARG;
     *out = PlanCheck();
     out->ops.assign(ops, ops + n_ops);
     out->signalled.assign(n_ops, 0);
diff --git a/smap_amd/csrc/tiles.h b/smap_amd/csrc/tiles.h
--- a/smap_amd/csrc/tiles.h
+++ b/smap_amd/csrc/tiles.h
@@ -16,7 +16,8 @@
     TC_DUAL = 8,
     TC_RELUSUM = 16,
     TC_REGEPI = 32,
-    TC_TAPDOT = 64
+    TC_TAPDOT = 64,
+    TC_RIDER = 128
 };
 
 struct TileRow {
@@ -69,7 +70,7 @@
     {51, TF_IGEMM, 128, 128, 32, 32, 0, 0, false, TC_BOTH | TC_DUAL | TC_RELUSUM},
     {52, TF_IGEMM, 128, 128, 64, 64, 0, 0, false, TC_BOTH},
     {53, TF_IGEMM, 256, 128, 32, 32, 0, 0, false, TC_BOTH | TC_DUAL | TC_RELUSUM},
-    {54, TF_IGEMM, 128, 256, 32, 32, 0, 0, false, TC_BOTH | TC_DUAL | TC_RELUSUM | TC_TAPDOT},
+    {54, TF_IGEMM, 128, 256, 32, 32, 0, 0, false, TC_BOTH | TC_DUAL | TC_RELUSUM | TC_TAPDOT | TC_RIDER},
     {55, TF_IGEMM, 128, 128, 32, 32, 0, 0, false, TC_BOTH},
     {56, TF_IGEMM, 256, 256, 64, 32, 0, 0, false, TC_X3 | TC_REGEPI},
     {60, TF_PERSIST, 128, 256, 32, 32, 0, 0, false, TC_BOTH},
diff --git a/smap_amd/engine.py b/smap_amd/engine.py
--- a/smap_amd/engine.py
+++ b/smap_amd/engine.py
@@ -24,7 +24,7 @@
     40: Tile("halo", 128, 128, 64, 32), 41: Tile("halo", 256, 128, 64, 32), 42: Tile("halo", 256, 64, 64, 32), 43: Tile("halo", 256, 128, 64, 32),
     44: Tile("halo", 256, 128, 64, 32), 45: Tile("halo", 256, 128, 64, 32),
     50: Tile("igemm", 128, 128, 32, 32, "dual relusum"), 51: Tile("igemm", 128, 128, 32, 32, "dual relusum"), 52: Tile("igemm", 128, 128, 64, 64),
-    53: Tile("igemm", 256, 128, 32, 32, "dual relusum"), 54: Tile("igemm", 128, 256, 32, 32, "dual relusum tapdot"), 55: Tile("igemm", 128, 128, 32, 32),
+    53: Tile("igemm", 256, 128, 32, 32, "dual relusum"), 54: Tile("igemm", 128, 256, 32, 32, "dual relusum tapdot rider"), 55: Tile("igemm", 128, 128, 32, 32),
     56: Tile("igemm", 256, 256, 64, 32, "regepi", prec="x3"),
     60: Tile("persist", 128, 256, 32, 32), 61: Tile("persist", 256, 128, 32, 32), 62: Tile("persist", 128, 128, 32, 32),
     63: Tile("persist", 128, 64, 32, 32), 64: Tile("persist", 128, 64, 32, 32), 65: Tile("persist", 128, 64, 32, 32),
@@ -88,8 +88,10 @@
     """SMAP_TAIL="64:80,128:82": (planes, tile id) pairs of the fused 3x3 + 1x1 launches (Graph.conv_tail); None (unset) = TAIL_DEFAULT."""
     cat: bool = None
     """SMAP_CAT=0|1: a Bottleneck's last 1x1 and its shortcut conv as one launch (Graph.conv_cat) never / in small schedules too; None = in all but those."""
-    skipsum: bool = None
-    """SMAP_SKIPSUM=0|1: skip1 + skip2 of an Upsample_unit as one launch and one tensor (Graph.conv_relusum), the same way."""
+    skipsum: object = None
+    """SMAP_SKIPSUM=0|1: skip1 + skip2 of an Upsample_unit as one launch and one tensor (Graph.conv_relusum), the same way.  That launch also
+    takes the unit's cross_conv along as its RIDER (Graph.ride_next; smap_op.in2_mode = 2) in all but small schedules; SMAP_SKIPSUM=norider:
+    the unset rule without riders (the A/B handle), SMAP_SKIPSUM=rider: both in small schedules too (the tests)."""
     taphead: bool = None
     """SMAP_TAPHEAD=0|1: the root-depth head as tap-dot launch + stencil (Graph.conv_tapdot / tapsum), the same way."""
     merge_1x1: int = 1
@@ -138,7 +140,7 @@
         tw, _, bn = get("HALO3").partition(":")
         table = lambda name, shipped: {} if get("NO_TILE_TABLE") else _load_table(get(name) or os.path.join(_HERE, shipped))
         return cls(block=pairs(get("BLOCK", None)), block_first=pairs(get("BLOCK_FIRST", None)), tail=pairs(get("TAIL", None)),
-                   cat=tri("CAT"), skipsum=tri("SKIPSUM"), taphead=tri("TAPHEAD"), merge_1x1={"0": 0, "2": 2}.get(get("MERGE_1X1"), 1),
+                   cat=tri("CAT"), skipsum=get("SKIPSUM") if get("SKIPSUM") in ("rider", "norider") else tri("SKIPSUM"), taphead=tri("TAPHEAD"), merge_1x1={"0": 0, "2": 2}.get(get("MERGE_1X1"), 1),
                    splitk="" if get("SPLITK") == "1" else get("SPLITK"), splitk_mink=int(get("SPLITK_MINK", "2048")),
                    deep_tile=get("DEEP_TILE") != "0", lanes=get("LANES") == "1", wpairs={"0": 0, "1": 1}.get(get("WPAIRS")),
                    x3_tile=num("X3_TILE"), cat_tile=num("CAT_TILE"), relusum_tile=num("RELUSUM_TILE"),
@@ -634,6 +636,22 @@
                              kinds="1x1", Cin=c1, Cout=cout, cout_pad=cout_pad, tile=tile, acc_scale=sc1, ref=self._ref(w=w1, b=b1), relu=0, aux2=x2,
                              sub=lambda: dict(cat=dict(cin=c2, stride=1, relusum=True, acc_scale=sc2, bias_off=self._add_w(self._bias(b2, cout_pad)),
                                                        **self._ref(w=w2, b=b2))))
+
+    def ride_next(self, i):
+        s, r = self.ops[i], self.ops[i + 1]
+        sp, rp = s.p, r.p
+        ok = (self.x3 and s.kind == OP_CONV == r.kind and sp.get("cat", {}).get("relusum") and tile_has(sp["tile"], "rider", True)
+              and sp["cout_pad"] == TILES[sp["tile"]][1] and not sp["w_pairs"] and r.inp is s.aux2 and rp["ksize"] == 1 and rp["stride"] == 1
+              and tile_family(rp["tile"]) == "igemm" and TILES[rp["tile"]][1] == 64 == rp["cout_pad"] and tile_bk(rp["tile"], True) == 32
+              and not rp["w_pairs"] and not rp["out_fp32"] and rp["in_c_off"] == 0 and rp["Cin"] == sp["cat"]["cin"] and rp["frames"] == sp["frames"]
+              and r.res is None and r.add1 is None and r.add2 is None and not r.aux and not r.outs and r.lane == s.lane
+              and not ({"cat", "tap", "segs", "tail", "head"} & set(rp)) and rp.get("ksplit", 1) <= 1)
+        if ok:
+            sp["cat"]["rider"] = True
+        return bool(ok)
+
+    def launches(self):
+        return len(self.ops) - sum(1 for op in self.ops if op.kind == OP_CONV and op.p.get("cat", {}).get("rider"))
 
     def conv_tapdot(self, name, pre1, pre3, x, frames=None):
         w1, b1 = self._fold(pre1)
@@ -881,7 +899,7 @@
             u = f"{pre}upsample.up{ind + 1}"
             un = f"{pre}upsample.up{ind + 2}"
             ss = self.policy.skipsum
-            skipsum = gen_skip and merge and ss is not False and self.one_window and (ss or not self.small)
+            skipsum = gen_skip and merge and ss is not False and self.one_window and ((ss and ss != "norider") or not self.small)
             if merge:
                 if gen_skip and not skipsum and (tl is None or merge_mode == 2):
                     out, s1[3 - ind] = self.conv_seg([(u + ".out", u + ".u_skip", True), (u + ".skip1", u + ".skip1", True)], xin, up=tl)
@@ -911,6 +929,8 @@
                     s2[3 - ind] = None if skipsum else got[u + ".skip2"]
                     if ind == 3:
                         cross = got[u + ".cross_conv"]
+                        if skipsum and len(sg) == 1 and ss != "norider" and (ss == "rider" or not self.small):
+                            self.ride_next(len(self.ops) - 2)
                 if heads:
                     if ind == 3:
                         tap = self.chl == 256 and self.policy.taphead is not False and (self.policy.taphead or not self.small)
@@ -1015,6 +1035,11 @@
                 t.last = max(t.last, i)
             for t in op.scratch:
                 t.first = t.last = i
+        early = set()
+        for i, op in enumerate(self.ops):
+            if op.kind == OP_CONV and op.p.get("cat", {}).get("rider"):
+                self.ops[i + 1].out.first = i
+                early.add(id(self.ops[i + 1].out))
         producer = {}
         for i, op in enumerate(self.ops):
             for t in ([op.out] if op.out is not None else []) + list(op.outs):
@@ -1081,6 +1106,9 @@
                         top += _rup(m.nbytes, ALIGN)
             for t in expiring.get(i, []):
                 if reuse and t.off >= 0:
+                    if id(t) in early and t.off + _rup(t.nbytes, ALIGN) == top:
+                        top = t.off
+                        continue
                     free.append((t.off, _rup(t.nbytes, ALIGN)))
                     free.sort()
                     merged = []
@@ -1162,7 +1190,7 @@
                     assert t.off // WINDOW == x.off // WINDOW, (y.name, "both inputs of a conv_cat launch must lie in one 4 GiB window")
                     o.in2_off, o.in2_H, o.in2_W, o.in2_C, o.in2_stride_c, o.in2_stride = t.off, t.H, t.W, p["cat"]["cin"], t.C * t.planes, p["cat"]["stride"]
                     if p["cat"].get("relusum"):
-                        o.in2_mode, o.in2_acc_scale, o.in2_bias_off = 1, p["cat"]["acc_scale"], p["cat"]["bias_off"]
+                        o.in2_mode, o.in2_acc_scale, o.in2_bias_off = 2 if p["cat"].get("rider") else 1, p["cat"]["acc_scale"], p["cat"]["bias_off"]
                 if p.get("ksplit", 1) > 1:
                     o.ksplit, o.kpart_off, o.kcount_off = p["ksplit"], op.scratch[0].off, self.kcount.off + 4 * p["kcount_first"]
                 for j, (sg, t) in enumerate(zip(p.get("segs", []), op.outs)):
```

Result: no change. 884.2 frames/sec (median of 6 runs) (+0.4%).
